# google-research/frame-interpolation

Hardware: AMD Instinct MI355X
Metric: interpolated frames/sec @1080p (higher is better)
Workload: dtype f32; 1 GPU; 1080p_2x2: 1920x1080 pair, align 64, block_shape [2, 2] -> 4 tile(s) of 960x576 in one batch, film_net published config, seeded synthetic weights, t=0.5; parallelism=1 independent GPU(s), weights RCCL-broadcast once, exec=direct launches, two lanes, lanes=1

## Files before the change

### frame-interpolation_amd/csrc/conv_igemm.hip

```cpp
#include "conv_buf_impl.h"
#include "conv_wino43_impl.h"
#include "conv_wino2d_impl.h"
#include "conv_fold4_impl.h"
#include "conv_c3_impl.h"
#ifdef FILM_EXTRA_FAMILIES
#include "conv_halo_impl.h"
#include "conv_split_impl.h"
#include "conv_wino_impl.h"
#include "conv_winox3_impl.h"
#include "conv_foldx3_impl.h"
#endif

template <int F>
static hipError_t launch_shape(const ConvParams& p, int shape, hipStream_t s) {
  switch (shape) {
    case TILE_128x128: return conv_buf_launch<128, 128, 2, 2, F>(p, s);
    case TILE_256x64: return conv_buf_launch<256, 64, 4, 1, F>(p, s);
    case TILE_256x32: return conv_buf_launch<256, 32, 4, 1, F>(p, s);
    case TILE_64x64: return conv_buf_launch<64, 64, 2, 2, F>(p, s);
    case TILE_128x32: return conv_buf_launch<128, 32, 4, 1, F>(p, s);
    case TILE_128x64: return conv_buf_launch<128, 64, 2, 2, F>(p, s);
    case TILE_256x128: return conv_buf_launch<256, 128, 4, 2, F>(p, s);
    default: return hipErrorInvalidValue;
  }
}

static hipError_t launch_c3(const ConvParams& p, int shape, hipStream_t s) {
  if (shape != TILE_C3_DIRECT) return hipErrorInvalidValue;
  return p.Cout % 64 == 0 ? conv_c3_launch<64>(p, s) : conv_c3_launch<32>(p, s);
}

#ifdef FILM_EXTRA_FAMILIES
template <int F>
static hipError_t launch_halo(const ConvParams& p, int shape, hipStream_t s) {
  switch (shape) {
    case HALO_8x128: return conv_halo_launch<8, 128, 4, 2, F>(p, s);
    case HALO_8x64: return conv_halo_launch<8, 64, 4, 1, F>(p, s);
    case HALO_8x32: return conv_halo_launch<8, 32, 4, 1, F>(p, s);
    case HALO_4x64: return conv_halo_launch<4, 64, 4, 1, F>(p, s);
    case HALO_4x128: return conv_halo_launch<4, 128, 2, 2, F>(p, s);
    case HALO_4x32: return conv_halo_launch<4, 32, 4, 1, F>(p, s);
    default: return hipErrorInvalidValue;
  }
}

template <int F, int NP>
static hipError_t launch_split(const ConvParams& p, int shape, hipStream_t s) {
  switch (shape) {
    case HALO_8x128: return conv_halo_split_launch<8, 128, 4, 2, NP, F>(p, s);
    case HALO_8x64: return conv_halo_split_launch<8, 64, 4, 1, NP, F>(p, s);
    case HALO_8x32: return conv_halo_split_launch<8, 32, 4, 1, NP, F>(p, s);
    case HALO_4x64: return conv_halo_split_launch<4, 64, 4, 1, NP, F>(p, s);
    case HALO_4x128: return conv_halo_split_launch<4, 128, 2, 2, NP, F>(p, s);
    case HALO_4x32: return conv_halo_split_launch<4, 32, 4, 1, NP, F>(p, s);
    default: return hipErrorInvalidValue;
  }
}

template <int F>
static hipError_t launch_wino(const ConvParams& p, int shape, hipStream_t s) {
  switch (shape) {
    case WINO_4x128: return conv_wino_launch<4, 128, 4, 2, F>(p, s);
    case WINO_4x64: return conv_wino_launch<4, 64, 4, 1, F>(p, s);
    case WINO_4x128_W16: return conv_wino_launch<4, 128, 4, 4, F>(p, s);
    case WINO_4x32: return conv_wino_launch<4, 32, 4, 1, F>(p, s);
    case WINO_8x64_W16: return conv_wino_launch<8, 64, 8, 2, F>(p, s);
    case WINO_8x32_W8: return conv_wino_launch<8, 32, 8, 1, F>(p, s);
    case WINO_2x64: return conv_wino_launch<2, 64, 2, 2, F>(p, s);
    case WINO_4x64_W8: return conv_wino_launch<4, 64, 4, 2, F>(p, s);
    default: return hipErrorInvalidValue;
  }
}

#endif

template <int F>
static hipError_t launch_wino43(const ConvParams& p, int shape, hipStream_t s) {
  switch (shape) {
    case W43_Q16_4x64_T21_P2: return conv_wino43_launch<4, 64, 2, 1, F | W43_F_PF2, 16>(p, s);
    case W43_Q16_4x32_T11_P2: return conv_wino43_launch<4, 32, 1, 1, F | W43_F_PF2, 16>(p, s);
    case W43_Q16_4x64_N1_P2: return conv_wino43_launch<4, 64, 1, 1, F | W43_F_PF2, 16, 1>(p, s);
    case W43_Q8_8x64_T21_P2: return conv_wino43_launch<8, 64, 2, 1, F | W43_F_PF2, 8>(p, s);
    case W43_Q8_8x64_N1_P2: return conv_wino43_launch<8, 64, 1, 1, F | W43_F_PF2, 8, 1>(p, s);
    case W43_Q8_8x32_T11_BG: return conv_wino43_launch<8, 32, 1, 1, F | W43_F_BG, 8>(p, s);
    case W43_Q8_8x32_T11_P2: return conv_wino43_launch<8, 32, 1, 1, F | W43_F_PF2, 8>(p, s);
#ifdef FILM_EXTRA_FAMILIES
    case W43_4x64_T21: return conv_wino43_launch<4, 64, 2, 1, F>(p, s);
    case W43_4x64_T12: return conv_wino43_launch<4, 64, 1, 2, F>(p, s);
    case W43_4x32_T11: return conv_wino43_launch<4, 32, 1, 1, F>(p, s);
    case W43_Q16_4x64_T21: return conv_wino43_launch<4, 64, 2, 1, F, 16>(p, s);
    case W43_Q16_4x64_T12: return conv_wino43_launch<4, 64, 1, 2, F, 16>(p, s);
    case W43_Q16_4x32_T11: return conv_wino43_launch<4, 32, 1, 1, F, 16>(p, s);
    case W43_Q16_4x64_N1: return conv_wino43_launch<4, 64, 1, 1, F, 16, 1>(p, s);
    case W43_Q16_4x64_T12_P2: return conv_wino43_launch<4, 64, 1, 2, F | W43_F_PF2, 16>(p, s);
    case W43_Q16_4x32_T11_BG: return conv_wino43_launch<4, 32, 1, 1, F | W43_F_BG, 16>(p, s);
    case W43_Q8_8x64_T12_P2: return conv_wino43_launch<8, 64, 1, 2, F | W43_F_PF2, 8>(p, s);
#endif
    default: return hipErrorInvalidValue;
  }
}

template <int F>
static hipError_t launch_wino2d(const ConvParams& p, int shape, hipStream_t s) {
  switch (shape) {
    case W2D_8x64: return conv_wino2d_launch_any<64, F>(p, s);
    case W2D_8x32: return conv_wino2d_launch_any<32, F>(p, s);
    case W2D_8x32_S2: return conv_wino2d_launch_any<32, F, 2>(p, s);
    case W2D_16x64: return conv_wino2d_launch_any<64, F | W2D_F_SQ>(p, s);
    case W2D_16x32: return conv_wino2d_launch_any<32, F | W2D_F_SQ>(p, s);
    case W2D_16x32_S2: return conv_wino2d_launch_any<32, F | W2D_F_SQ, 2>(p, s);
    default: return hipErrorInvalidValue;
  }
}

template <int F>
static hipError_t launch_fold4(const ConvParams& p, int shape, hipStream_t s) {
  switch (shape) {
    case F4_4x64: return conv_fold4_launch<2, F>(p, s);
    case F4_4x32: return conv_fold4_launch<1, F>(p, s);
    default: return hipErrorInvalidValue;
  }
}

#ifdef FILM_EXTRA_FAMILIES
template <int F>
static hipError_t launch_winox3(const ConvParams& p, int shape, hipStream_t s) {
  switch (shape) {
    case WX3_4x128_T22: return conv_winox3_launch<4, 128, 2, 2, F>(p, s);
    case WX3_4x64_T12: return conv_winox3_launch<4, 64, 1, 2, F>(p, s);
    case WX3_4x64_T21: return conv_winox3_launch<4, 64, 2, 1, F>(p, s);
    case WX3_4x32_T11: return conv_winox3_launch<4, 32, 1, 1, F>(p, s);
    default: return hipErrorInvalidValue;
  }
}

template <int F>
static hipError_t launch_foldx3(const ConvParams& p, int shape, hipStream_t s) {
  switch (shape) {
    case FX3_4x64: return conv_foldx3_launch<4, 64, 4, 1, F>(p, s);
    case FX3_8x64: return conv_foldx3_launch<8, 64, 8, 1, F>(p, s);
    case FX3_4x128: return conv_foldx3_launch<4, 128, 4, 2, F>(p, s);
    default: return hipErrorInvalidValue;
  }
}
#endif


__global__ __launch_bounds__(256) void conv_splitk_reduce_kernel(const float* __restrict__ part, const float* __restrict__ bias,
                                                                 float* __restrict__ out, int M, int Cout, int ostride,
                                                                 int S, int leaky) {
  const int G = Cout >> 2;
  const unsigned idx = blockIdx.x * 256u + threadIdx.x;
  if (idx >= (unsigned)M * (unsigned)G) return;
  const unsigned m = idx / (unsigned)G, g = idx - m * (unsigned)G;
  const size_t plane = (size_t)M * Cout;
  const float4* src = reinterpret_cast<const float4*>(part + (size_t)m * Cout + g * 4);
  float4 a = *reinterpret_cast<const float4*>(bias + g * 4);
  for (int sidx = 0; sidx < S; ++sidx) {
    const float4 v = src[(size_t)sidx * (plane >> 2)];
    a.x += v.x; a.y += v.y; a.z += v.z; a.w += v.w;
  }
  if (leaky) {
    a.x = a.x > 0.f ? a.x : 0.2f * a.x; a.y = a.y > 0.f ? a.y : 0.2f * a.y;
    a.z = a.z > 0.f ? a.z : 0.2f * a.z; a.w = a.w > 0.f ? a.w : 0.2f * a.w;
  }
  *reinterpret_cast<float4*>(out + (size_t)m * ostride + g * 4) = a;
}

static hipError_t film_launch_conv_main(const ConvParams& p, int fam, int tile, hipStream_t s) {
  const int shape = conv_tile_shape(tile);
  const bool xcd = tile & CONV_TILE_XCD;
  if ((p.pool_out != nullptr || p.pw_out != nullptr) && kConvFamily[fam].fused_shape < 0) return hipErrorInvalidValue;
  switch (fam) {
    case FAM_BUF: return xcd ? launch_shape<CONV_B_XCD_M>(p, shape, s) : launch_shape<0>(p, shape, s);
    case FAM_C3: return launch_c3(p, shape, s);
    case FAM_FOLD4: return xcd ? launch_fold4<CONV_B_XCD_M>(p, shape, s) : launch_fold4<0>(p, shape, s);
    case FAM_W2D:
      if (p.ksize != 3) return hipErrorInvalidValue;
      return xcd ? launch_wino2d<CONV_B_XCD_M>(p, shape, s) : launch_wino2d<0>(p, shape, s);
    case FAM_W43:
      if (p.ksize != 3) return hipErrorInvalidValue;
      if (p.pool_out != nullptr && shape < W43_Q16_4x64_T21) return hipErrorInvalidValue;
      if (p.pw_out != nullptr && ((shape != W43_Q16_4x64_N1 && shape != W43_Q16_4x64_N1_P2 && shape != W43_Q8_8x64_N1_P2) || p.Cout != 64 || p.ksplit > 1 ||
                                  p.pool_out != nullptr || p.pw_cout < 1 || p.pw_cout > 4))
        return hipErrorInvalidValue;
      return xcd ? launch_wino43<CONV_B_XCD_M>(p, shape, s) : launch_wino43<0>(p, shape, s);
#ifdef FILM_EXTRA_FAMILIES
    case FAM_HALO:
      if (p.ksize != 3) return hipErrorInvalidValue;
      return xcd ? launch_halo<CONV_B_XCD_M>(p, shape, s) : launch_halo<0>(p, shape, s);
    case FAM_SPLIT6:
      if (p.ksize != 3) return hipErrorInvalidValue;
      return xcd ? launch_split<CONV_B_XCD_M, 6>(p, shape, s) : launch_split<0, 6>(p, shape, s);
    case FAM_SPLIT3:
      if (p.ksize != 3) return hipErrorInvalidValue;
      return xcd ? launch_split<CONV_B_XCD_M, 3>(p, shape, s) : launch_split<0, 3>(p, shape, s);
    case FAM_WINO:
      if (p.ksize != 3) return hipErrorInvalidValue;
      return xcd ? launch_wino<CONV_B_XCD_M>(p, shape, s) : launch_wino<0>(p, shape, s);
    case FAM_WINOX3:
      if (p.ksize != 3) return hipErrorInvalidValue;
      return xcd ? launch_winox3<CONV_B_XCD_M>(p, shape, s) : launch_winox3<0>(p, shape, s);
    case FAM_FOLDX3:
      if (p.ksize != 2 || p.fold != 2) return hipErrorInvalidValue;
      return xcd ? launch_foldx3<CONV_B_XCD_M>(p, shape, s) : launch_foldx3<0>(p, shape, s);
#endif
    default: return hipErrorNotSupported;
  }
}

hipError_t film_launch_conv(const ConvParams& p, int tile, hipStream_t s) {
  const int fam = conv_family_of(tile);
  if (fam < 0 || (p.ksplit > 1 && !kConvFamily[fam].splitk)) return hipErrorInvalidValue;
  const hipError_t e = film_launch_conv_main(p, fam, tile, s);
  if (e != hipSuccess || p.ksplit <= 1) return e;
  const long long Mout = (long long)p.M * (p.fold == 3 ? 4 : 1);
  if (!p.part || (p.Cout & 3) || Mout * (p.Cout >> 2) >= (1ll << 32)) return hipErrorInvalidValue;
  const unsigned units = (unsigned)Mout * (unsigned)(p.Cout >> 2);
  hipLaunchKernelGGL(conv_splitk_reduce_kernel, dim3((units + 255) / 256), dim3(256), 0, s, p.part, p.bias, p.out, (int)Mout, p.Cout,
                     p.ostride, p.ksplit, p.leaky);
  return hipGetLastError();
}
```

### frame-interpolation_amd/csrc/conv_wino2d_impl.h

```cpp
#pragma once
#include "conv_common.h"

enum { W2D_F_SQ = 128,
       W2D_F_XEPI = 8,
       W2D_DBG_TIME = 8192 };


template <bool SQ> struct W2dSlotTable { unsigned v[24 * 64]; };
template <bool SQ> constexpr W2dSlotTable<SQ> w2d_make_slot_table() {
  constexpr int QW = SQ ? 4 : 8, TH = SQ ? 16 : 8, HR = TH + 2, PW = 4 * QW + 2;
  constexpr int CO4 = (PW + 3) / 4, MO4 = 4 * CO4, RP4 = 4 * MO4 + (SQ ? 2 : 4);
  W2dSlotTable<SQ> t{};
  for (int sl = 0; sl < 24 * 64; ++sl) {
    const int r = sl / RP4, rem = sl % RP4, m = rem / MO4, rr = rem % MO4, c = rr / CO4, k = rr % CO4, px = 4 * k + m;
    const bool ok = r < HR && rem < 4 * MO4 && px < PW;
    t.v[sl] = ok ? ((unsigned)r << 24 | (unsigned)px << 8 | (unsigned)c << 4) : 0xFFFFFFFFu;
  }
  return t;
}
template <bool SQ> __device__ const W2dSlotTable<SQ> w2d_slot_table = w2d_make_slot_table<SQ>();

template <int BN, int FLAGS, int NS_ = 3>
__global__ __launch_bounds__(4 * (BN / 32) * 64, (BN == 32) ? 2 : 1) void conv_wino2d_kernel(ConvParams p) {
  constexpr bool SQ = (FLAGS & W2D_F_SQ) != 0;
  constexpr int QW = SQ ? 4 : 8, TH = SQ ? 16 : 8, HR = TH + 2, PXW = 4 * QW, PW = PXW + 2;
  static_assert(QW * (TH / 2) == 32, "32 units per tile");
  constexpr int NG = BN / 32, NW = 4 * NG;
  constexpr int CO4 = (PW + 3) / 4, MO4 = 4 * CO4, RP4 = 4 * MO4 + (SQ ? 2 : 4);
  constexpr int NREQ = 24;
  constexpr int STAGE4 = NREQ * 64;
  constexpr int NS = NS_;
  static_assert(NS == 2 || NS == 3, "stages");
  constexpr int IPW = NREQ / NW;
  static_assert(NREQ % NW == 0, "requests per wave");
  static_assert(HR * RP4 <= STAGE4, "stage size");
  constexpr bool XE = (FLAGS & W2D_F_XEPI) != 0;
  constexpr unsigned OOB = 0xFFFFFFFFu;

  extern __shared__ __attribute__((aligned(1024))) float smem[];

  const int t = threadIdx.x;
  const int lane = t & 63;
  const int wv = __builtin_amdgcn_readfirstlane(t >> 6);
  const int l31 = lane & 31, half = lane >> 5;
  const int mu = wv & 3, ng = wv >> 2;

  unsigned long long tm0 = 0, tm1 = 0, tm2 = 0, tmA = 0, tmB = 0, tmC = 0, tmW = 0, tmE1 = 0, tmE2 = 0, tmE3 = 0;
  unsigned long long rt0 = 0;
  if constexpr ((FLAGS & W2D_DBG_TIME) != 0) { rt0 = __builtin_amdgcn_s_memrealtime(); tm0 = __builtin_readcyclecounter(); }

  int aH = p.H, aW = p.W, aNB = p.NB, aCtot = p.Ctot, aKsplit = p.ksplit, aNseg = p.nseg, aUnused = p.unused_chain;
  unsigned a_tpi = p.mg_tpi, a_ntx = p.mg_ntx, a_nby = p.mg_nby;
  int ntx_ = p.tl_ntx, tpi_ = p.tl_tpi;
  int aGx = (int)gridDim.x, aGy = (int)gridDim.y;
  const float* aS0ptr = p.seg[0].ptr;
  int aS0stride = p.seg[0].stride, aS0C = p.seg[0].C, aS0boff = p.seg[0].boff, aS0bmod = p.seg[0].bmod;
  const float* aWptr = p.w;
  unsigned rtab[(24 / (4 * (BN / 32)))];
#pragma unroll
  for (int n = 0; n < 24 / NW; ++n) rtab[n] = w2d_slot_table<SQ>.v[t + 64 * NW * n];
  {
    unsigned long long q0 = (unsigned long long)(uintptr_t)aS0ptr, q1 = (unsigned long long)(uintptr_t)aWptr;
    asm volatile("" : "+s"(aH), "+s"(aW), "+s"(aNB), "+s"(aCtot), "+s"(aKsplit), "+s"(aNseg), "+s"(aUnused), "+s"(a_tpi), "+s"(a_ntx), "+s"(a_nby), "+s"(ntx_), "+s"(tpi_),
                      "+s"(aGx), "+s"(aGy), "+s"(q0), "+s"(q1), "+s"(aS0stride), "+s"(aS0C), "+s"(aS0boff), "+s"(aS0bmod));
    aS0ptr = reinterpret_cast<const float*>((uintptr_t)q0);
    aWptr = reinterpret_cast<const float*>((uintptr_t)q1);
  }
  unsigned long long tmK = 0, tmT = 0;
  if constexpr ((FLAGS & W2D_DBG_TIME) != 0) tmK = __builtin_readcyclecounter();
  int bx = blockIdx.x, by = blockIdx.y;
  if constexpr ((FLAGS & CONV_B_XCD_M) != 0) {
    const int nbx = aGx, nby = aGy;
    const int nwg = nbx * nby;
    const int lin = by * nbx + bx;
    const int xcd = lin & 7, idx = lin >> 3;
    const int q = nwg >> 3, r = nwg & 7;
    const int base = xcd < r ? xcd * (q + 1) : r * (q + 1) + (xcd - r) * q;
    const int nl = base + idx;
    bx = (int)conv_udiv((unsigned)nl, a_nby);
    by = nl - bx * nby;
  }
  const int ntx = ntx_, tpi = tpi_;
  const int img = (int)conv_udiv((unsigned)bx, a_tpi);
  const int trow0 = (int)conv_udiv((unsigned)(bx - img * tpi), a_ntx);
  const int y0 = trow0 * TH, x0 = (bx - img * tpi - trow0 * ntx) * PXW;
  const int n0 = by * BN;

  unsigned rvoff[IPW];
  int rsg = 0, rc0 = 0, rsegC = 0;
  conv_rsrc_t rrsrc = conv_make_rsrc(conv_uniform_ptr(aS0ptr));
  const unsigned lds0 = (unsigned)(size_t)(__attribute__((address_space(3))) float*)smem;
  unsigned rpk[IPW];
  auto set_rpk = [&]() {
    const int H = aH, W = aW;
    const bool inside = y0 >= 1 && y0 + TH + 1 <= H && x0 >= 1 && x0 + PXW + 1 <= W;
    if (inside) {
#pragma unroll
      for (int n = 0; n < IPW; ++n) rpk[n] = rtab[n];
    } else {
#pragma unroll
      for (int n = 0; n < IPW; ++n) {
        const unsigned tv = rtab[n];
        const unsigned y = (unsigned)(y0 - 1) + (tv >> 24), x = (unsigned)(x0 - 1) + ((tv >> 8) & 255u);
        rpk[n] = ((y < (unsigned)H) & (x < (unsigned)W)) ? tv : OOB;
      }
    }
  };
  set_rpk();
#pragma unroll
  for (int n = 0; n < IPW; ++n) asm volatile("" : "+v"(rpk[n]));
  if constexpr ((FLAGS & W2D_DBG_TIME) != 0) tmT = __builtin_readcyclecounter();
  auto raw_setup_seg_of = [&](const float* sptr, int sstride, int sC, int sboff, int sbmod) {
    rsegC = __builtin_amdgcn_readfirstlane(sC);
    int be = img + sboff;
    if (sbmod && be >= sbmod) be -= sbmod;
    const int spix = (be * aH + (y0 - 1)) * aW + (x0 - 1);
    rrsrc = conv_make_rsrc(conv_uniform_ptr(sptr + (long long)spix * sstride));
    const unsigned st4 = (unsigned)sstride * 4u;
    const unsigned wst4 = (unsigned)aW * st4;
#pragma unroll
    for (int n = 0; n < IPW; ++n) {
      const unsigned tv = rpk[n];
      unsigned off, tmp;
      asm("v_and_b32 %0, 48, %2\n\tv_bfe_u32 %1, %2, 8, 8\n\tv_mad_u32_u24 %0, %1, %3, %0\n\tv_lshrrev_b32 %1, 24, %2\n\tv_mad_u32_u24 %0, %1, %4, %0"
          : "=&v"(off), "=&v"(tmp) : "v"(tv), "s"(st4), "s"(wst4));
      rvoff[n] = tv == OOB ? OOB : off;
    }
  };
  auto raw_setup_seg = [&]() {
    const ConvSeg& s = p.seg[rsg];
    raw_setup_seg_of(s.ptr, s.stride, s.C, s.boff, s.bmod);
  };
  auto dma_piece = [&](int n, int stage) {
    const unsigned so = (unsigned)rc0 * 4u;
    const unsigned base = lds0 + (unsigned)stage * (STAGE4 * 16u) + (unsigned)(wv + NW * n) * 1024u;
    asm volatile("s_mov_b32 m0, %0\n\ts_nop 0\n\tbuffer_load_dwordx4 %1, %2, %3 offen lds" ::"s"(base), "v"(rvoff[n]), "s"(rrsrc), "s"(so)
                 : "memory");
  };
  auto dma_advance = [&]() {
    rc0 += 16;
    if (rc0 >= rsegC) {
      if (rsg + 1 < aNseg) { rc0 = 0; ++rsg; raw_setup_seg(); }
    }
  };
  const int ksp = XE && aKsplit > 1 ? aKsplit : 1;
  const int nsc_all = aCtot >> 4;
  int sc0 = 0, sc1 = nsc_all;
  if (ksp > 1) {
    sc0 = (int)((unsigned)nsc_all * blockIdx.z / (unsigned)ksp);
    sc1 = (int)((unsigned)nsc_all * (blockIdx.z + 1u) / (unsigned)ksp);
    int c = sc0 * 16;
    while (rsg + 1 < aNseg && c >= p.seg[rsg].C) { c -= p.seg[rsg].C; ++rsg; }
    rc0 = c;
  }
  auto raw_issue = [&](int stage) {
#pragma unroll
    for (int n = 0; n < IPW; ++n) dma_piece(n, stage);
    dma_advance();
  };

  const int nkc = aCtot / 8, nsc = sc1 - sc0, kc0 = 2 * sc0, kc1 = 2 * sc1;
  const conv_rsrc_t brsrc = conv_make_rsrc(conv_uniform_ptr(aWptr));
  const unsigned bvoff = (unsigned)((half * 32 + l31) * 16);
  const int ct = n0 / 32 + ng;
  auto slab = [&](int kc) { return (unsigned)(((ct * nkc + (kc < nkc ? kc : nkc - 1)) * 4 + mu) * 6) * 1024u; };
  bf4 fbg[2][6];

  f32x16 acc[6];

  const bf4* const smem4 = reinterpret_cast<const bf4*>(smem);
  const int ur = l31 / QW, lq = l31 % QW;
  const int ra = mu == 0 ? 0 : mu == 2 ? 2 : 1, rb = mu == 0 ? 2 : mu == 1 ? 2 : mu == 2 ? 1 : 3;
  const float sgn = mu == 1 ? 1.f : -1.f;
  const int ix_a = (2 * ur + ra) * RP4 + half * CO4 + lq, ix_b = (2 * ur + rb) * RP4 + half * CO4 + lq;
  typedef float f2 __attribute__((ext_vector_type(2)));
  f2 A[2][6][2];
  bf4 d[6];
  bf4 d2[6];

  using C0 = std::integral_constant<int, 0>;
  using C1 = std::integral_constant<int, 1>;
  auto read_row = [&](bf4 (&dst)[6], int ix, int stage, auto h_c) {
    constexpr int IMM = decltype(h_c)::value * 2 * CO4;
    const int ixs = ix + stage * STAGE4;
#pragma unroll
    for (int j = 0; j < 6; ++j) dst[j] = smem4[ixs + IMM + (j & 3) * MO4 + (j >> 2)];
  };
  auto pair_of = [](const bf4& v, int q) -> f2 { return q ? f2{v[2], v[3]} : f2{v[0], v[1]}; };
  auto set_pair = [](bf4& v, int q, f2 x) { if (q) { v[2] = x[0]; v[3] = x[1]; } else { v[0] = x[0]; v[1] = x[1]; } };
  auto fma2 = [](float k, f2 x, f2 y) -> f2 {
    f2 r;
    const f2 kk = {k, k};
    asm("v_pk_fma_f32 %0, %1, %2, %3" : "=v"(r) : "s"(kk), "v"(x), "v"(y));
    return r;
  };
  auto add2 = [](f2 x, f2 y) -> f2 { f2 r; asm("v_pk_add_f32 %0, %1, %2" : "=v"(r) : "v"(x), "v"(y)); return r; };
  auto mul2 = [](float k, f2 x) -> f2 {
    f2 r;
    const f2 kk = {k, k};
    asm("v_pk_mul_f32 %0, %1, %2" : "=v"(r) : "s"(kk), "v"(x));
    return r;
  };
  auto max1 = [](float x, float y) -> float { float r; asm("v_max_f32 %0, %1, %2" : "=v"(r) : "v"(x), "v"(y)); return r; };
  auto sub2 = [](f2 x, f2 y) -> f2 { f2 r; asm("v_pk_add_f32 %0, %1, %2 neg_lo:[0,1] neg_hi:[0,1]" : "=v"(r) : "v"(x), "v"(y)); return r; };
  f2 xt[4];
  auto xf_t = [&](int q) {
    const f2 d1 = pair_of(d[1], q), d2v = pair_of(d[2], q), d3 = pair_of(d[3], q), d4 = pair_of(d[4], q);
    xt[0] = fma2(-4.f, d2v, d4);
    xt[1] = fma2(-4.f, d1, d3);
    xt[2] = sub2(d4, d2v);
    xt[3] = sub2(d3, d1);
  };
  auto xf_v = [&](int q, int nu) -> f2 {
    switch (nu) {
      case 0: return fma2(4.f, pair_of(d[0], q), fma2(-5.f, pair_of(d[2], q), pair_of(d[4], q)));
      case 1: return add2(xt[0], xt[1]);
      case 2: return sub2(xt[0], xt[1]);
      case 3: return fma2(2.f, xt[3], xt[2]);
      case 4: return fma2(-2.f, xt[3], xt[2]);
      default: return fma2(4.f, pair_of(d[1], q), fma2(-5.f, pair_of(d[3], q), pair_of(d[5], q)));
    }
  };
  auto pin = [](f2& v) { asm volatile("" : "+v"(v)); };
  auto prepare = [&](f2 (&An)[6][2], int stage, auto h_c) {
    read_row(d, ix_a, stage, h_c);
    read_row(d2, ix_b, stage, h_c);
#pragma unroll
    for (int j = 0; j < 6; ++j)
#pragma unroll
      for (int q = 0; q < 2; ++q) set_pair(d[j], q, fma2(sgn, pair_of(d2[j], q), pair_of(d[j], q)));
#pragma unroll
    for (int q = 0; q < 2; ++q) {
      xf_t(q);
#pragma unroll
      for (int nu = 0; nu < 6; ++nu) An[nu][q] = xf_v(q, nu);
    }
  };

  if (ksp > 1) raw_setup_seg();
  else raw_setup_seg_of(aS0ptr, aS0stride, aS0C, aS0boff, aS0bmod);
  raw_issue(0);
  if constexpr ((FLAGS & W2D_DBG_TIME) != 0) tmA = __builtin_readcyclecounter();
#pragma unroll
  for (int j = 0; j < 6; ++j) fbg[0][j] = conv_buf_load(brsrc, bvoff, slab(kc0) + (unsigned)j * 1024u);
  __builtin_amdgcn_sched_barrier(0);
  asm volatile("s_waitcnt vmcnt(6)" ::: "memory");
  if constexpr ((FLAGS & W2D_DBG_TIME) != 0) tmB = __builtin_readcyclecounter();
  __syncthreads();
  if constexpr ((FLAGS & W2D_DBG_TIME) != 0) tmC = __builtin_readcyclecounter();
#pragma unroll
  for (int j = 0; j < 6; ++j) fbg[1][j] = conv_buf_load(brsrc, bvoff, slab(kc0 + 1) + (unsigned)j * 1024u);
  __builtin_amdgcn_sched_barrier(0);
  if (nsc > 1) raw_issue(1);
  if constexpr (NS > 2) { if (nsc > 2) raw_issue(2); }
  prepare(A[0], 0, C0{});

  int st_s = 0, st_n = 1;
  int st_dma = 0;
  bool dma_on = false;
  int gs = 0;
  constexpr int P1 = NS == 2 ? IPW : (IPW + 1) / 2, P0 = IPW - P1;
  auto dma_slot = [](int g, int cnt) constexpr -> int {
    if (cnt <= 0) return -1;
    if (cnt == 6) return g == 2 ? 0 : (g >= 5 && (g - 5) % 4 == 0) ? 1 + (g - 5) / 4 : -1;
    const int step = 24 / cnt, at = cnt == 1 ? 13 : 5;
    return (g % step == at && g / step < cnt) ? g / step : -1;
  };
  auto chunk = [&](int kc, auto h_c, auto first_c, auto last_c) {
    constexpr int H = decltype(h_c)::value;
    constexpr bool FIRST = decltype(first_c)::value != 0;
    constexpr bool LAST = decltype(last_c)::value != 0;
    constexpr bool PREP = !(LAST && H == 1);
    using RH = std::integral_constant<int, 1 - H>;
    const int rs = H == 0 ? st_s : st_n;
    f2(&Ac)[6][2] = A[H];
    f2(&An)[6][2] = A[1 - H];
    if constexpr (H == 1 && !LAST) {
      unsigned long long tw0 = 0;
      if constexpr ((FLAGS & W2D_DBG_TIME) != 0) tw0 = __builtin_readcyclecounter();
      if (NS == 2 || gs == 0) asm volatile("s_waitcnt vmcnt(6)" ::: "memory");
      else asm volatile("s_waitcnt vmcnt(12)" ::: "memory");
      __syncthreads();
      if constexpr ((FLAGS & W2D_DBG_TIME) != 0) tmW += __builtin_readcyclecounter() - tw0;
      dma_on = (kc >> 1) + NS < sc1;
      st_dma = st_s;
    }
    const unsigned so2 = LAST ? 0u : slab(kc + 2);
    __builtin_amdgcn_sched_barrier(0);
    auto gap = [&](auto g_c) {
      constexpr int g = decltype(g_c)::value;
      constexpr int jp = g >> 3, i8 = g & 7, k = i8 >> 1, j = 2 * jp + (i8 & 1);
      if constexpr (FIRST && k == 0) {
        const f32x16 zero = {0.f, 0.f, 0.f, 0.f, 0.f, 0.f, 0.f, 0.f, 0.f, 0.f, 0.f, 0.f, 0.f, 0.f, 0.f, 0.f};
        acc[j] = __builtin_amdgcn_mfma_f32_32x32x2f32(fbg[H][j][k], Ac[j][k >> 1][k & 1], zero, 0, 0, 0);
      } else {
        acc[j] = __builtin_amdgcn_mfma_f32_32x32x2f32(fbg[H][j][k], Ac[j][k >> 1][k & 1], acc[j], 0, 0, 0);
      }
      if constexpr (!LAST) {
        if constexpr (k == 3) fbg[H][j] = conv_buf_load(brsrc, bvoff, so2 + (unsigned)j * 1024u);
      }
      if constexpr (PREP) {
        if constexpr (g == 0) read_row(d, ix_a, rs, RH{});
        if constexpr (g == 1) read_row(d2, ix_b, rs, RH{});
        if constexpr (g >= 4 && g < 10) {
          constexpr int jj = g - 4;
#pragma unroll
          for (int q = 0; q < 2; ++q) { f2 v = fma2(sgn, pair_of(d2[jj], q), pair_of(d[jj], q)); pin(v); set_pair(d[jj], q, v); }
        }
        if constexpr (g >= 10 && g < 16) {
          constexpr int q = (g - 10) / 3, part = (g - 10) % 3;
          if constexpr (part == 0) {
            xf_t(q);
            pin(xt[0]); pin(xt[1]); pin(xt[2]); pin(xt[3]);
          } else if constexpr (part == 1) {
            An[0][q] = xf_v(q, 0);
            An[5][q] = xf_v(q, 5);
            pin(An[0][q]); pin(An[5][q]);
          } else {
#pragma unroll
            for (int nu = 1; nu < 5; ++nu) { An[nu][q] = xf_v(q, nu); pin(An[nu][q]); }
          }
        }
      }
      if constexpr (!LAST) {
        constexpr int CNT = H == 1 ? P1 : P0, N0 = H == 1 ? 0 : P1;
        constexpr int idx = dma_slot(g, CNT);
        if constexpr (idx >= 0) {
          if (dma_on) {
            dma_piece(N0 + idx, st_dma);
            if constexpr (N0 + idx == IPW - 1) dma_advance();
          }
        }
      }
      __builtin_amdgcn_sched_barrier(0);
    };
    conv_for_each(gap, std::make_integer_sequence<int, 24>{});
    if constexpr (H == 1) {
      st_s = st_n;
      st_n = st_n + 1 == NS ? 0 : st_n + 1;
      ++gs;
    }
  };

  auto epilogue = [&]() {
    const int t = threadIdx.x, lane = t & 63, l31 = lane & 31, half = lane >> 5;
    __syncthreads();
    if constexpr ((FLAGS & W2D_DBG_TIME) != 0) tmE1 = __builtin_readcyclecounter();
    float o[4][16];
  #pragma unroll
    for (int r = 0; r < 16; ++r) {
      const float m0 = acc[0][r], m1 = acc[1][r], m2 = acc[2][r], m3 = acc[3][r], m4 = acc[4][r], m5 = acc[5][r];
      const float s34 = m3 + m4, d34 = m3 - m4, d12 = m1 - m2, s12 = m1 + m2;
      o[0][r] = ((m0 + m1) + m2) + s34;
      o[1][r] = __builtin_fmaf(2.f, d34, d12);
      o[2][r] = __builtin_fmaf(4.f, s34, s12);
      o[3][r] = d12 + __builtin_fmaf(8.f, d34, m5);
    }
    bf4* const xb = reinterpret_cast<bf4*>(smem);
    constexpr int XB4 = NG * 4 * 256;
    static_assert(2 * XB4 <= NS * STAGE4, "exchange buffers");
    const int widx = (ng * 4 + mu) * 256 + l31 * 8;
    const int rng = t >> 8, run = (t >> 3) & 31, rcg = t & 7;
    const int ridx = rng * 1024 + run * 8 + (rcg ^ (run & 7));
    const int nrd = n0 + rng * 32 + rcg * 4;
    const bool rawsum = XE && ksp > 1;
    const bool has_pw = XE && p.pw_out != nullptr;
    float b0 = 0.f, b1 = 0.f, b2 = 0.f, b3 = 0.f;
    if (!rawsum) { const float* const bp = p.bias + nrd; b0 = bp[0]; b1 = bp[1]; b2 = bp[2]; b3 = bp[3]; }
    const int oy = y0 + 2 * (run / QW), ox = x0 + 4 * (run % QW);
    const int ostr = rawsum ? p.Cout : p.ostride;
    const float slope = (p.leaky && !rawsum) ? 0.2f : 1.f;
    const int dyo = 2 * (run / QW), dxo = 4 * (run % QW), nth = rng * 32 + rcg * 4;
    const int cpix = (img * p.H + y0) * p.W + x0;
    float* obase = p.out;
    if (rawsum) { asm volatile(""); obase = p.part + (size_t)blockIdx.z * p.M * p.Cout; }
    float* const ocorner = obase + ((long long)cpix * ostr + n0);
    float* const orow = ocorner + (__umul24(__umul24(dyo, p.W) + dxo, ostr) + nth);
    float* pool_base = nullptr;
    if (XE && p.pool_out) {
      asm volatile("");
      const int ppix = (img * (p.H >> 1) + (y0 >> 1)) * (p.W >> 1) + (x0 >> 1);
      pool_base = p.pool_out + ((long long)ppix * p.pool_ostride + n0) + (__umul24(__umul24(dyo >> 1, p.W >> 1) + (dxo >> 1), p.pool_ostride) + nth);
    }
    constexpr int PWS = 68;
    float* const pwt = smem + 2 * XB4 * 4;
    float* const pww = pwt + TH * PXW * PWS;
    if (has_pw && t < 256) pww[t] = (t & 3) < p.pw_cout ? p.pw_w[(t >> 2) * p.pw_cout + (t & 3)] : 0.f;
    bf4 k0 = {0.f, 0.f, 0.f, 0.f}, k1 = {0.f, 0.f, 0.f, 0.f};
    auto write_round = [&](int jx, bf4* xw) {
  #pragma unroll
      for (int g = 0; g < 4; ++g) {
        bf4 v;
        v[0] = o[jx][4 * g]; v[1] = o[jx][4 * g + 1]; v[2] = o[jx][4 * g + 2]; v[3] = o[jx][4 * g + 3];
        xw[widx + ((2 * g + half) ^ (l31 & 7))] = v;
      }
    };
  #pragma unroll
    for (int jx = 0; jx < 4; ++jx) {
      bf4* const xw = xb + (jx & 1) * XB4;
      write_round(jx, xw);
      __syncthreads();
      if constexpr ((FLAGS & W2D_DBG_TIME) != 0) { if (jx == 0) tmE2 = __builtin_readcyclecounter(); if (jx == 3) tmE3 = __builtin_readcyclecounter(); }
      const bf4 m0 = xw[ridx], m1 = xw[ridx + 256], m2 = xw[ridx + 512], m3 = xw[ridx + 768];
      bf4 r0, r1;
  #pragma unroll
      for (int q = 0; q < 2; ++q) {
        const f2 bq = q ? f2{b2, b3} : f2{b0, b1};
        const f2 v0 = add2(add2(add2(pair_of(m0, q), pair_of(m1, q)), pair_of(m2, q)), bq);
        const f2 v1 = add2(sub2(sub2(pair_of(m1, q), pair_of(m2, q)), pair_of(m3, q)), bq);
        const f2 s0 = mul2(slope, v0), s1 = mul2(slope, v1);
        set_pair(r0, q, f2{max1(v0[0], s0[0]), max1(v0[1], s0[1])});
        set_pair(r1, q, f2{max1(v1[0], s1[0]), max1(v1[1], s1[1])});
      }
      if (!has_pw) {
        if (ox + jx < p.W) {
          float* const o0 = orow + (size_t)jx * ostr;
          if (oy < p.H) *reinterpret_cast<bf4*>(o0) = r0;
          if (oy + 1 < p.H) *reinterpret_cast<bf4*>(o0 + (size_t)p.W * ostr) = r1;
        }
        if (XE && pool_base != nullptr) {
          if (jx & 1) {
            bf4 pv;
  #pragma unroll
            for (int c = 0; c < 4; ++c) pv[c] = (((k0[c] + r0[c]) + k1[c]) + r1[c]) * 0.25f;
            if (oy < p.H && ox + jx < p.W) *reinterpret_cast<bf4*>(pool_base + (size_t)(jx >> 1) * p.pool_ostride) = pv;
          } else {
            k0 = r0; k1 = r1;
          }
        }
      } else {
        float* const tr = pwt + ((2 * (run / QW)) * PXW + 4 * (run % QW) + jx) * PWS + rng * 32 + rcg * 4;
        *reinterpret_cast<bf4*>(tr) = r0;
        *reinterpret_cast<bf4*>(tr + PXW * PWS) = r1;
      }
    }
    if (has_pw) {
      __syncthreads();
      if (t < TH * PXW) {
        const int y = y0 + t / PXW, x = x0 + (t % PXW);
        float a[4] = {0.f, 0.f, 0.f, 0.f};
        const bf4* row = reinterpret_cast<const bf4*>(pwt + t * PWS);
        const bf4* wq = reinterpret_cast<const bf4*>(pww);
  #pragma unroll 4
        for (int c4 = 0; c4 < 16; ++c4) {
          const bf4 v = row[c4];
  #pragma unroll
          for (int k = 0; k < 4; ++k) {
            const bf4 w = wq[c4 * 4 + k];
  #pragma unroll
            for (int j = 0; j < 4; ++j) a[j] = __builtin_fmaf(v[k], w[j], a[j]);
          }
        }
        if (y < p.H && x < p.W) {
          float* dd = p.pw_out + (((size_t)img * p.H + y) * p.W + x) * p.pw_ostride;
  #pragma unroll
          for (int j = 0; j < 4; ++j)
            if (j < p.pw_cout) dd[j] = a[j] + p.pw_bias[j];
        }
      }
    }
  };
  if constexpr ((FLAGS & W2D_DBG_TIME) != 0) tm1 = __builtin_readcyclecounter();
  for (int tile = 0; tile < 1; ++tile) {
    chunk(kc0, C0{}, C1{}, C0{});
    chunk(kc0 + 1, C1{}, C0{}, C0{});
    for (int kc = kc0 + 2; kc < kc1 - 2; kc += 2) {
      chunk(kc, C0{}, C0{}, C0{});
      chunk(kc + 1, C1{}, C0{}, C0{});
    }
    if (nsc > 1) {
      chunk(kc1 - 2, C0{}, C0{}, C1{});
      chunk(kc1 - 1, C1{}, C0{}, C1{});
    }
    if constexpr ((FLAGS & W2D_DBG_TIME) != 0) tm2 = __builtin_readcyclecounter();
    epilogue();
  }
  if constexpr ((FLAGS & W2D_DBG_TIME) != 0) {
    const unsigned long long tm3 = __builtin_readcyclecounter();
    if (t == 0) {
      unsigned long long* o8 = reinterpret_cast<unsigned long long*>(p.part) + (size_t)(blockIdx.y * gridDim.x + blockIdx.x) * 16;
      o8[0] = tm0; o8[1] = tm1; o8[2] = tm2; o8[3] = tm3; o8[4] = tmA; o8[5] = tmB; o8[6] = tmC; o8[7] = tmW;
      o8[8] = rt0; o8[9] = __builtin_amdgcn_s_memrealtime();
      o8[10] = (unsigned long long)__builtin_amdgcn_s_getreg((31 << 11) | 4) | ((unsigned long long)__builtin_amdgcn_s_getreg((31 << 11) | 20) << 32);
      o8[11] = tmE1; o8[12] = tmE2; o8[13] = tmE3; o8[14] = tmK; o8[15] = tmT;
    }
  }
}

template <int BN, int FLAGS, int NS = 3>
hipError_t conv_wino2d_launch(const ConvParams& p, hipStream_t s) {
  if (!(FLAGS & W2D_F_XEPI) && (p.ksplit > 1 || p.pool_out || p.pw_out)) return hipErrorInvalidValue;
  const size_t lds = p.pw_out ? (size_t)2 * (BN / 32) * 16 * 1024 + 256 * 68 * 4 + 1024 : (size_t)NS * 24 * 1024;
  constexpr int NT = 4 * (BN / 32) * 64;
  if (p.ksize != 3 || p.Ctot % 16 || p.Cout % BN) return hipErrorInvalidValue;
  if (p.ksplit > 1 && (!p.part || (reinterpret_cast<uintptr_t>(p.part) & 15) || p.Cout % 4 || p.pool_out || p.pw_out || p.ksplit > p.Ctot / 16)) return hipErrorInvalidValue;
  if (p.pw_out) {
    if (BN != 64 || p.Cout != 64 || p.pool_out || p.pw_cout < 1 || p.pw_cout > 4) return hipErrorInvalidValue;
  } else if (p.ostride % 4 || (reinterpret_cast<uintptr_t>(p.out) & 15)) return hipErrorInvalidValue;
  if (p.pool_out && ((p.H | p.W) & 1 || p.pool_ostride % 4 || (reinterpret_cast<uintptr_t>(p.pool_out) & 15))) return hipErrorInvalidValue;
  {
    long long nimg = p.NB;
    for (int i = 0; i < p.nseg; ++i) nimg = std::max<long long>(nimg, (long long)p.seg[i].bmod);
    if ((nimg + 1) * p.H * p.W >= (1ll << 31)) return hipErrorInvalidValue;
  }
  if (p.W <= 0 || p.H <= 0 || p.W >= (1 << 20) || p.ostride >= (1 << 22) || p.pool_ostride >= (1 << 22) || p.Cout >= (1 << 22) ||
      (long long)8 * p.W * (p.ostride > p.Cout ? p.ostride : p.Cout) >= (1ll << 31)) return hipErrorInvalidValue;
  for (int i = 0; i < p.nseg; ++i)
    if ((long long)p.W * p.seg[i].stride * 4 >= (1ll << 24) || p.seg[i].C % 16 || p.seg[i].stride % 4 || p.seg[i].stride <= 0 || p.seg[i].stride >= (1 << 22) || p.seg[i].up || (reinterpret_cast<uintptr_t>(p.seg[i].ptr) & 15)) return hipErrorInvalidValue;
  constexpr bool SQ = (FLAGS & W2D_F_SQ) != 0;
  const int ntx = SQ ? (p.W + 15) / 16 : (p.W + 31) / 32, nty = SQ ? (p.H + 15) / 16 : (p.H + 7) / 8;
  const int ntiles = p.NB * ntx * nty;
  dim3 grid((unsigned)ntiles, p.Cout / BN, (unsigned)(p.ksplit > 1 ? p.ksplit : 1));
  ConvParams q = p;
  bool exact = true;
  q.mg_nby = conv_magic(grid.y, (unsigned long long)grid.x * grid.y, exact);
  q.mg_tpi = conv_magic((unsigned long long)ntx * nty, (unsigned long long)ntiles + 1, exact);
  q.mg_ntx = conv_magic(ntx, (unsigned long long)ntx * nty, exact);
  q.tl_ntx = ntx; q.tl_tpi = ntx * nty;
  if (!exact) return hipErrorInvalidValue;
  return conv_launch<conv_wino2d_kernel<BN, FLAGS, NS>>(grid, dim3(NT), lds, s, q, 144 * 1024);
}

template <int BN, int FLAGS, int NS = 3>
hipError_t conv_wino2d_launch_any(const ConvParams& p, hipStream_t s) {
  if (p.ksplit > 1 || p.pool_out || p.pw_out) return conv_wino2d_launch<BN, FLAGS | W2D_F_XEPI, NS>(p, s);
  return conv_wino2d_launch<BN, FLAGS, NS>(p, s);
}
```

### frame-interpolation_amd/csrc/film_engine.cpp

```cpp
#include "film_internal.h"

namespace film_internal {

thread_local std::string g_create_error;

int fail(film_t* h, int code, const char* fmt, ...) {
  char buf[1024];
  va_list ap;
  va_start(ap, fmt);
  vsnprintf(buf, sizeof buf, fmt, ap);
  va_end(ap);
  if (h) h->err = buf; else g_create_error = buf;
  return code;
}

int copy_out_string(film_t* h, const std::string& s, char* buf, int64_t cap, int64_t* needed) {
  if (needed) *needed = (int64_t)s.size() + 1;
  if (!buf || cap < (int64_t)s.size() + 1) {
    if (!buf && needed) return FILM_OK;
    return fail(h, FILM_ERR_INVALID, "buffer too small: need %lld bytes", (long long)s.size() + 1);
  }
  memcpy(buf, s.c_str(), s.size() + 1);
  return FILM_OK;
}

}

using namespace film_internal;

namespace {

enum OptNorm { AS_IS, BOOL, NONNEG, LOW5 };
struct OptionRow {
  const char* key;
  int film_t::*field;
  OptNorm norm;
  bool drops_plans;
  int64_t lo = 0, hi = 0;
  const char* refusal = nullptr;
  ConvFamily family = FAM_BUF;
  int need_lo = 0, need_hi = 0;
  const char* family_refusal = nullptr;
};
constexpr OptionRow kOptions[] = {
    {"graph", &film_t::opt_graph, AS_IS, false, 0, 2, "graph: 0 (one stream, eager), 1 (hipGraph replay) or 2 (two lanes, eager: the default)"},
    {"profile", &film_t::opt_profile, BOOL, false},
    {"autotune", &film_t::opt_autotune, BOOL, false},
    {"max_batch", &film_t::opt_max_batch, NONNEG, false},
    {"host_overlap", &film_t::opt_host_overlap, BOOL, false},
    {"block_overlap_h", &film_t::opt_block_overlap_h, AS_IS, false, -1, 65535, "block_overlap_h: -1 (what the align padding of a tile holds) or 0 .. 65535 rows"},
    {"block_overlap_w", &film_t::opt_block_overlap_w, AS_IS, false, -1, 65535, "block_overlap_w: -1 (what the align padding of a tile holds) or 0 .. 65535 columns"},
    {"tune_ms", &film_t::opt_tune_ms, NONNEG, false},
    {"splitk", &film_t::opt_splitk, BOOL, true},
    {"pack_groups", nullptr, AS_IS, false, 1, 4, "pack_groups: 1 .. 4"},
    {"fuse", &film_t::opt_fuse, LOW5, true},
    {"fold2x2", &film_t::opt_fold2x2, AS_IS, true, 0, 2, "fold2x2: 0, 1 or 2"},
    {"planar", &film_t::opt_planar, BOOL, true},
    {"winograd", &film_t::opt_wino, AS_IS, true, 0, 3, "winograd: 0, 1, 2 or 3", FAM_WINO, 2, 2,
     "winograd = 2 (F(2,3) kernel on every level) needs a library built with FILM_EXTRA_FAMILIES=1"},
    {"halo_all", &film_t::opt_halo_all, BOOL, true, 0, 0, nullptr, FAM_HALO, 1, 1, "halo_all needs a library built with FILM_EXTRA_FAMILIES=1"},
    {"lanes", &film_t::opt_lanes, AS_IS, true, 0, 3, "lanes: 0, 1, 2 or 3"},
    {"wino2d", &film_t::opt_wino2d, AS_IS, true, 0, 2, "wino2d: 0, 1 or 2"},
    {"w2d_small_px", &film_t::opt_w2d_small_px, AS_IS, true, 0, 1 << 30, "w2d_small_px: pixels per image, 0 = never"},
    {"w2d_min_px", &film_t::opt_w2d_min_px, AS_IS, true, 1, 1 << 30, "w2d_min_px: pixels per image"},
    {"w2d_splitk", &film_t::opt_w2d_splitk, AS_IS, true, 0, 16, "w2d_splitk: 0 (off), 1 (default rule) or 2..16 (A/B: the cap on levels of <= 1024 pixels)"},
    {"w2d_shape", &film_t::opt_w2d_shape, AS_IS, true, -1, W2D_SHAPES - 1, "w2d_shape: -1 (autotuned) or a Wino2dTile shape index"},
    {"fold4_shape", &film_t::opt_fold4_shape, AS_IS, true, -1, F4_4x32, "fold4_shape: -1 (autotuned) or a Fold4Tile shape index"},
    {"w43_shape", &film_t::opt_w43_shape, AS_IS, true, -1, 31, "w43_shape: -1 (autotuned) or a Wino43Tile shape index"},
    {"precision", &film_t::opt_precision, AS_IS, true, 0, 2, "precision: 0 (f32), 1 (bf16x6) or 2 (bf16x3)", FAM_SPLIT6, 1, 2,
     "precision %d (bf16 split modes) needs a library built with FILM_EXTRA_FAMILIES=1; this build runs fp32 MFMA only"},
};
constexpr bool option_rows_complete() {
  for (const OptionRow& o : kOptions)
    if ((o.lo < o.hi) != (o.refusal != nullptr) || ((o.family != FAM_BUF) != (o.family_refusal != nullptr))) return false;
  return true;
}
static_assert(option_rows_complete(), "a row with a range (a family) carries its refusal message, a row without leaves lo = hi (family = FAM_BUF)");

int tile_geometry(film_t* h, int H, int W, int block_h, int block_w, int align, TileMapParams* tp) {
  const int bh = block_h > 0 ? block_h : 1, bw = block_w > 0 ? block_w : 1;
  if (H % bh) return fail(h, FILM_ERR_INVALID, "block_height=%d should evenly divide height=%d.", bh, H);
  if (W % bw) return fail(h, FILM_ERR_INVALID, "block_width=%d should evenly divide width=%d.", bw, W);
  tp->H = H; tp->W = W; tp->bh = bh; tp->bw = bw; tp->ph = H / bh; tp->pw = W / bw;
  struct Axis { const char* key; int nb, p, want; int *ov, *e, *T, *off; };
  const Axis axes[2] = {{"block_overlap_h", bh, tp->ph, h->opt_block_overlap_h, &tp->ovy, &tp->eh, &tp->TH, &tp->oy},
                        {"block_overlap_w", bw, tp->pw, h->opt_block_overlap_w, &tp->ovx, &tp->ew, &tp->TW, &tp->ox}};
  for (const Axis& a : axes) {
    const int pad0 = (align > 0 && a.p % align) ? align - a.p % align : 0;
    const int o = a.nb == 1 ? 0 : a.want < 0 ? std::min(pad0 / 2, a.p / 2) : a.want;
    if (2 * (int64_t)o > a.p)
      return fail(h, FILM_ERR_INVALID, "%s: twice the overlap (%d) must not exceed the patch size %d", a.key, o, a.p);
    const int e = a.p + 2 * o;
    const int pad = (align > 0 && e % align) ? align - e % align : 0;
    *a.ov = o; *a.e = e; *a.T = e + pad; *a.off = pad / 2;
  }
  return FILM_OK;
}
hipError_t cut_tiles(const TileMapParams& tp, hipStream_t s) {
  return (tp.ovy | tp.ovx) ? film_launch_frame_to_tiles_overlap(tp, s) : film_launch_frame_to_tiles(tp, s);
}
hipError_t join_tiles(const TileMapParams& tp, hipStream_t s) {
  return (tp.ovy | tp.ovx) ? film_launch_blend_tiles(tp, s) : film_launch_tiles_to_frame(tp, s);
}
hipError_t cut_tiles_pix(const TileMapParams& tp, int pix, hipStream_t s) {
  if (pix != FILM_PIX_U8) return cut_tiles(tp, s);
  const uint8_t* src = reinterpret_cast<const uint8_t*>(tp.src);
  return (tp.ovy | tp.ovx) ? film_launch_frame_to_tiles_overlap_u8(tp, src, s) : film_launch_frame_to_tiles_u8(tp, src, s);
}
int ensure_stage(film_t* h, size_t bytes, hipStream_t s) {
  if (h->stage_bytes >= bytes) return FILM_OK;
  if (h->stage) { HIPCHK(h, hipStreamSynchronize(s)); HIPCHK(h, hipFree(h->stage)); h->stage = nullptr; h->stage_bytes = 0; }
  hipError_t e = hipMalloc(&h->stage, bytes);
  if (e != hipSuccess) return fail(h, FILM_ERR_NOMEM, "frame staging hipMalloc of %.1f MB failed", bytes * 1e-6);
  h->stage_bytes = bytes;
  return FILM_OK;
}
int balanced_chunk(int n, int maxc) {
  if (n <= maxc) return n;
  for (int c = maxc; 2 * c > maxc; --c)
    if (n % c == 0) return c;
  return maxc;
}
void sequence_chunk(int n, int T, int cap, int* k, int* nt) {
  int bk = 0, bt = 1;
  for (int t = std::min(T, cap); t >= 1; --t) {
    const int kk = std::min(n, cap / t);
    if (kk > bk) { bk = kk; bt = t; }
  }
  *k = balanced_chunk(n, std::max(bk, 1));
  *nt = balanced_chunk(T, bt);
}
int need_device(film_t* h, const char* fn) {
  if (h->plan_only) return fail(h, FILM_ERR_NO_DEVICE, "plan-only handle: %s needs a HIP device (no CPU fallback)", fn);
  if (!h->finalized) return fail(h, FILM_ERR_STATE, "film_finalize has not been called");
  return FILM_OK;
}
bool halve_on_nomem(int rc, int* chunk) {
  if (rc != FILM_ERR_NOMEM || *chunk <= 1) return false;
  *chunk = (*chunk + 1) / 2;
  return true;
}
struct FrameStage {
  film_t* h; hipStream_t s; bool host;
  float* result; size_t out_floats;
  float* out = nullptr;
  size_t used = 0;
  int open(size_t in_floats) {
    out = result;
    if (!host) return FILM_OK;
    int rc = ensure_stage(h, (in_floats + out_floats) * sizeof(float), s);
    if (rc == FILM_OK) out = (float*)h->stage + in_floats;
    return rc;
  }
  int upload(const float* src, size_t floats, const float** dev) {
    *dev = src;
    if (!host) return FILM_OK;
    HIPCHK(h, hipMemcpyAsync((float*)h->stage + used, src, floats * sizeof(float), hipMemcpyHostToDevice, s));
    *dev = (float*)h->stage + used;
    used += floats;
    return FILM_OK;
  }
  int finish() {
    if (!host) return FILM_OK;
    HIPCHK(h, hipMemcpyAsync(result, out, out_floats * sizeof(float), hipMemcpyDeviceToHost, s));
    HIPCHK(h, hipStreamSynchronize(s));
    return FILM_OK;
  }
};
template <class T> struct TileCopy { T* frames; int tile0, ntiles; int64_t slot; };
using Cut = TileCopy<const float>;
using Join = TileCopy<float>;
int run_chunk(film_t* h, Plan* P, TileMapParams tp, const std::vector<Cut>& cuts, const std::vector<Join>& joins, hipStream_t s) {
  const int64_t tile_floats = (int64_t)tp.TH * tp.TW * 3;
  for (const Cut& c : cuts) {
    tp.tile0 = c.tile0; tp.ntiles = c.ntiles; tp.src = c.frames; tp.dst = P->at("img0") + c.slot * tile_floats;
    HIPCHK(h, cut_tiles(tp, s));
  }
  int rc = run_plan(h, P, s);
  if (rc) return rc;
  for (const Join& j : joins) {
    tp.tile0 = j.tile0; tp.ntiles = j.ntiles; tp.src = P->at("out") + j.slot * tile_floats; tp.dst = j.frames;
    HIPCHK(h, join_tiles(tp, s));
  }
  return FILM_OK;
}

hipStream_t pick_stream(film_t* h, int mem_kind, void* stream) {
  return stream ? (hipStream_t)stream : (mem_kind == FILM_MEM_DEVICE ? (hipStream_t) nullptr : h->stream);
}

int forward_chunk(film_t* h, const float* x0, const float* x1, int B, int H, int W, float* out, int mem_kind, void* stream) {
  HIPCHK(h, hipSetDevice(h->device));
  Plan* P = nullptr;
  int rc = get_plan(h, B, H, W, true, &P);
  if (rc) return rc;
  hipStream_t s = pick_stream(h, mem_kind, stream);
  const size_t in_bytes = (size_t)B * H * W * 3 * sizeof(float);
  const hipMemcpyKind kin = mem_kind == FILM_MEM_HOST ? hipMemcpyHostToDevice : hipMemcpyDeviceToDevice;
  const hipMemcpyKind kout = mem_kind == FILM_MEM_HOST ? hipMemcpyDeviceToHost : hipMemcpyDeviceToDevice;
  HIPCHK(h, hipMemcpyAsync(P->at("img0"), x0, in_bytes, kin, s));
  HIPCHK(h, hipMemcpyAsync(P->at("img0") + (int64_t)B * H * W * 3, x1, in_bytes, kin, s));
  rc = run_plan(h, P, s);
  if (rc) return rc;
  HIPCHK(h, hipMemcpyAsync(out, P->at("out"), in_bytes, kout, s));
  if (mem_kind == FILM_MEM_HOST) HIPCHK(h, hipStreamSynchronize(s));
  return FILM_OK;
}

int interpolate_host_pipeline(film_t* h, Plan* P, TileMapParams tp, const float* x0, const float* x1, float* out, float* st, size_t frame_bytes, hipStream_t s) {
  const int nt = P->B;
  const size_t nf = frame_bytes / sizeof(float);
  for (hipEvent_t& e : h->pipe_ev)
    if (!e) HIPCHK(h, hipEventCreateWithFlags(&e, hipEventDisableTiming));
  LanePipe lp;
  for (size_t i = 0; i < P->ops.size() && lp.head.size() < 2; ++i) {
    const OpDesc& op = P->ops[i];
    if (op.lane == 1) continue;
    if (!batch_splittable(op, 2) || !op.xdeps.empty() || op.NB != 2 * nt) break;
    lp.head.push_back(i);
  }
  const OpDesc& last = P->ops.back();
  lp.tail = tp.B == 1 && tp.bh % 2 == 0 && last.lane == 0 && last.pw_out.buf >= 0 && last.NB == nt && batch_splittable(last, 2) && P->ops.size() > lp.head.size() + 1 &&
            std::find(lp.head.begin(), lp.head.end(), P->ops.size() - 1) == lp.head.end();
  tp.tile0 = 0;
  lp.mid_tail = [&]() -> hipError_t {
    TileMapParams t2 = tp;
    t2.ntiles = nt / 2; t2.src = P->at("out"); t2.dst = st + 2 * nf;
    hipError_t e = film_launch_tiles_to_frame(t2, s);
    if (e == hipSuccess) e = hipEventRecord(h->pipe_ev[1], s);
    return e;
  };
  struct Drain {
    film_t* h; hipStream_t s; bool armed;
    ~Drain() { if (armed) { (void)hipStreamSynchronize(h->stream2); (void)hipStreamSynchronize(s); } }
  } drain{h, s, true};
  HIPCHK(h, hipMemcpyAsync(st, x0, frame_bytes, hipMemcpyHostToDevice, s));
  tp.ntiles = nt; tp.src = st; tp.dst = P->at("img0");
  HIPCHK(h, film_launch_frame_to_tiles(tp, s));
  HIPCHK(h, hipEventRecord(h->pipe_ev[0], s));
  HIPCHK(h, hipStreamWaitEvent(h->stream2, h->pipe_ev[0], 0));
  for (size_t i : lp.head) HIPCHK(h, launch_op(batch_part(P->ops[i], 0, 2), P->arena, h->packed_dev, s));
  HIPCHK(h, hipMemcpyAsync(st + nf, x1, frame_bytes, hipMemcpyHostToDevice, h->stream2));
  tp.src = st + nf; tp.dst = P->at("img0") + (int64_t)nt * tp.TH * tp.TW * 3;
  HIPCHK(h, film_launch_frame_to_tiles(tp, h->stream2));
  HIPCHK(h, hipEventRecord(h->pipe_ev[0], h->stream2));
  HIPCHK(h, hipStreamWaitEvent(s, h->pipe_ev[0], 0));
  const hipError_t le = issue_lanes(h, P, s, false, &lp);
  if (le != hipSuccess) return fail(h, FILM_ERR_HIP, "kernel launch failed: %s", hipGetErrorString(le));
  h->last_plan = P;
  const int64_t tile_floats = (int64_t)tp.TH * tp.TW * 3;
  if (lp.tail) {
    TileMapParams t2 = tp;
    t2.tile0 = nt / 2; t2.ntiles = nt - nt / 2; t2.src = P->at("out") + (int64_t)(nt / 2) * tile_floats; t2.dst = st + 2 * nf;
    HIPCHK(h, film_launch_tiles_to_frame(t2, s));
    const size_t half = frame_bytes / 2;
    HIPCHK(h, hipStreamWaitEvent(h->stream2, h->pipe_ev[1], 0));
    HIPCHK(h, hipMemcpyAsync(out, st + 2 * nf, half, hipMemcpyDeviceToHost, h->stream2));
    HIPCHK(h, hipMemcpyAsync((char*)out + half, (const char*)(st + 2 * nf) + half, frame_bytes - half, hipMemcpyDeviceToHost, s));
    HIPCHK(h, hipStreamSynchronize(h->stream2));
  } else {
    tp.tile0 = 0; tp.ntiles = nt; tp.src = P->at("out"); tp.dst = st + 2 * nf;
    HIPCHK(h, film_launch_tiles_to_frame(tp, s));
    HIPCHK(h, hipMemcpyAsync(out, st + 2 * nf, frame_bytes, hipMemcpyDeviceToHost, s));
  }
  HIPCHK(h, hipStreamSynchronize(s));
  drain.armed = false;
  return FILM_OK;
}

size_t pix_bytes(int pix) { return pix == FILM_PIX_U8 ? 1 : sizeof(float); }
void stream_free(film_t* h) {
  FilmStream& fs = h->fs;
  for (void* p : {fs.keep, (void*)fs.result, (void*)fs.result8})
    if (p) (void)hipFree(p);
  fs = FilmStream{};
}
bool same_geometry(const TileMapParams& a, const TileMapParams& b) {
  const int va[] = {a.H, a.W, a.bh, a.bw, a.ph, a.pw, a.TH, a.TW, a.oy, a.ox, a.ovy, a.ovx, a.eh, a.ew};
  const int vb[] = {b.H, b.W, b.bh, b.bw, b.ph, b.pw, b.TH, b.TW, b.oy, b.ox, b.ovy, b.ovx, b.eh, b.ew};
  return std::equal(std::begin(va), std::end(va), std::begin(vb));
}
hipError_t stream_cut(const FilmStream& fs, TileMapParams tp, const Plan* P, int slot, hipStream_t s) {
  tp.tile0 = 0; tp.ntiles = tp.bh * tp.bw;
  tp.src = (const float*)fs.keep;
  tp.dst = P->at("img0") + (int64_t)slot * tp.ntiles * tp.TH * tp.TW * 3;
  return cut_tiles_pix(tp, fs.pix, s);
}

int debug_plan(film_t* h, int B, int H, int W, int tiles, Plan** P) {
  if (h->plan_only) return fail(h, FILM_ERR_NO_DEVICE, "plan-only handle has no device");
  if (!h->finalized) return fail(h, FILM_ERR_STATE, "weights are not finalized");
  if (tiles < 0 || (tiles > 0 && B % tiles)) return fail(h, FILM_ERR_INVALID, "tiles must be 0 (pair plan) or divide B (sequence plan)");
  HIPCHK(h, hipSetDevice(h->device));
  return get_plan(h, B, H, W, true, P, tiles);
}

}

extern "C" {

int film_to_uint8(const float* src, unsigned char* dst, int64_t n, void* stream) {
  if (n < 0 || (n > 0 && (!src || !dst))) return FILM_ERR_INVALID;
  return film_launch_to_uint8(src, dst, n, (hipStream_t)stream) == hipSuccess ? FILM_OK : FILM_ERR_HIP;
}

#ifndef FILM_SRC_ID
#define FILM_SRC_ID "unknown"
#endif
#ifdef FILM_EXTRA_FAMILIES
#define FILM_FLAVOUR "+extra"
#else
#define FILM_FLAVOUR ""
#endif
const char* film_version(void) { return "gfx950;film_hip r6;src=" FILM_SRC_ID FILM_FLAVOUR; }

int film_default_config(film_config* cfg) {
  if (!cfg) return FILM_ERR_INVALID;
  memset(cfg, 0, sizeof *cfg);
  cfg->pyramid_levels = 7; cfg->fusion_pyramid_levels = 5; cfg->specialized_levels = 3; cfg->sub_levels = 4;
  cfg->filters = 64;
  const int fcv[4] = {3, 3, 3, 3}, ffl[4] = {32, 64, 128, 256};
  for (int i = 0; i < 4; ++i) { cfg->flow_convs[i] = fcv[i]; cfg->flow_filters[i] = ffl[i]; }
  return FILM_OK;
}

int film_create(film_t** out, int device, const film_config* cfg) {
  if (!out) return fail(nullptr, FILM_ERR_INVALID, "out is NULL");
  *out = nullptr;
  std::unique_ptr<film_handle> h(new film_handle);
  if (cfg) h->cfg = *cfg; else film_default_config(&h->cfg);
  int rc = validate_config(h.get(), h->cfg);
  if (rc) { g_create_error = h->err; return rc; }
  h->device = device;
  h->plan_only = device < 0;
  if (!h->plan_only) {
    int ndev = 0;
    hipError_t e = hipGetDeviceCount(&ndev);
    if (e != hipSuccess || ndev <= 0)
      return fail(nullptr, FILM_ERR_NO_DEVICE, "no HIP device available (%s); libfilm_hip has no CPU fallback",
                  e != hipSuccess ? hipGetErrorString(e) : "device count 0");
    if (device >= ndev) return fail(nullptr, FILM_ERR_INVALID, "device %d out of range (%d devices)", device, ndev);
    if (hipSetDevice(device) != hipSuccess) return fail(nullptr, FILM_ERR_HIP, "hipSetDevice(%d) failed", device);
    hipDeviceProp_t prop;
    if (hipGetDeviceProperties(&prop, device) == hipSuccess && strncmp(prop.gcnArchName, "gfx950", 6) != 0)
      return fail(nullptr, FILM_ERR_NO_DEVICE, "device %d is %s; this library is built for gfx950 only", device, prop.gcnArchName);
    if (hipStreamCreateWithFlags(&h->stream, hipStreamNonBlocking) != hipSuccess ||
        hipStreamCreateWithFlags(&h->stream2, hipStreamNonBlocking) != hipSuccess)
      return fail(nullptr, FILM_ERR_HIP, "hipStreamCreate failed");
  }
  build_layers(h.get());
  *out = h.release();
  return FILM_OK;
}

void film_destroy(film_t* h) {
  if (!h) return;
  drop_plans(h);
  stream_free(h);
  if (h->packed_dev) (void)hipFree(h->packed_dev);
  if (h->stage) (void)hipFree(h->stage);
  if (h->metrics_buf) (void)hipFree(h->metrics_buf);
  if (h->stream) (void)hipStreamDestroy(h->stream);
  for (hipEvent_t& e : h->pipe_ev) if (e) { (void)hipEventDestroy(e); e = nullptr; }
  if (h->stream2) (void)hipStreamDestroy(h->stream2);
  delete h;
}

const char* film_last_error(const film_t* h) { return h ? h->err.c_str() : g_create_error.c_str(); }

int film_set_option(film_t* h, const char* key, int64_t value) {
  if (!h || !key) return FILM_ERR_INVALID;
  for (const OptionRow& o : kOptions) {
    if (strcmp(key, o.key)) continue;
    if (o.refusal && (value < o.lo || value > o.hi)) return fail(h, FILM_ERR_INVALID, "%s", o.refusal);
    const int v = o.norm == BOOL ? value != 0 : o.norm == NONNEG ? (value > 0 ? (int)value : 0) : o.norm == LOW5 ? (int)(value & 31) : (int)value;
    if (o.family_refusal && v >= o.need_lo && v <= o.need_hi && !conv_family_built(o.family)) return fail(h, FILM_ERR_INVALID, o.family_refusal, v);
    if (!o.field) return h->finalized ? film_ensure_groups_(h, v) : FILM_OK;
    if (h->*o.field == v) return FILM_OK;
    if (o.drops_plans) drop_plans(h);
    h->*o.field = v;
    return FILM_OK;
  }
  return fail(h, FILM_ERR_NOTFOUND, "unknown option '%s'", key);
}

int film_plan_json(film_t* h, int B, int H, int W, char* buf, int64_t cap, int64_t* needed) {
  if (!h) return FILM_ERR_INVALID;
  Plan* P = nullptr;
  int rc = get_plan(h, B, H, W, false, &P);
  if (rc) return rc;
  return copy_out_string(h, plan_json(h, *P), buf, cap, needed);
}

int film_sequence_plan_json(film_t* h, int n_pairs, int tiles_per_frame, int H, int W, char* buf, int64_t cap, int64_t* needed) {
  if (!h) return FILM_ERR_INVALID;
  if (n_pairs < 1 || tiles_per_frame < 1) return fail(h, FILM_ERR_INVALID, "n_pairs and tiles_per_frame must be positive");
  if ((int64_t)n_pairs * tiles_per_frame >= (int64_t)1 << 30) return fail(h, FILM_ERR_INVALID, "batch too large (2*B*H*W must fit int32)");
  Plan* P = nullptr;
  int rc = get_plan(h, n_pairs * tiles_per_frame, H, W, false, &P, tiles_per_frame);
  if (rc) return rc;
  return copy_out_string(h, plan_json(h, *P), buf, cap, needed);
}

int film_profile_json(film_t* h, char* buf, int64_t cap, int64_t* needed) {
  if (!h) return FILM_ERR_INVALID;
  if (h->profile_json.empty()) return fail(h, FILM_ERR_STATE, "no profiled forward yet (film_set_option(\"profile\", 1))");
  return copy_out_string(h, h->profile_json, buf, cap, needed);
}

int film_forward(film_t* h, const float* x0, const float* x1, int B, int H, int W, float* out, int mem_kind, void* stream) {
  if (!h || !x0 || !x1 || !out) return fail(h, FILM_ERR_INVALID, "NULL argument");
  int rc = need_device(h, "film_forward");
  if (rc) return rc;
  if (mem_kind != FILM_MEM_HOST && mem_kind != FILM_MEM_DEVICE) return fail(h, FILM_ERR_INVALID, "bad mem_kind");
  if (B < 1) return fail(h, FILM_ERR_INVALID, "B, H, W must be positive");
  int bmax = 1;
  rc = max_units(h, H, W, "frame", "tile the frame (Interpolator block_shape)", &bmax);
  if (rc) return rc;
  const size_t frame = (size_t)H * W * 3;
  int chunk = balanced_chunk(B, bmax);
  for (int b0 = 0; b0 < B;) {
    chunk = std::min(chunk, B - b0);
    rc = forward_chunk(h, x0 + b0 * frame, x1 + b0 * frame, chunk, H, W, out + b0 * frame, mem_kind, stream);
    if (halve_on_nomem(rc, &chunk)) continue;
    if (rc) return rc;
    b0 += chunk;
  }
  return FILM_OK;
}

int film_interpolate(film_t* h, const float* x0, const float* x1, int B, int H, int W, int align, int block_h,
                     int block_w, float* out, int mem_kind, void* stream) {
  if (!h || !x0 || !x1 || !out) return fail(h, FILM_ERR_INVALID, "NULL argument");
  int rc = need_device(h, "film_interpolate");
  if (rc) return rc;
  if (mem_kind != FILM_MEM_HOST && mem_kind != FILM_MEM_DEVICE) return fail(h, FILM_ERR_INVALID, "bad mem_kind");
  if (B < 1 || H < 1 || W < 1) return fail(h, FILM_ERR_INVALID, "B, H, W must be positive");
  TileMapParams tp{};
  tp.B = B;
  rc = tile_geometry(h, H, W, block_h, block_w, align, &tp);
  if (rc) return rc;
  HIPCHK(h, hipSetDevice(h->device));
  int tmax = 1;
  rc = max_units(h, tp.TH, tp.TW, "tile", "use a finer block_shape", &tmax);
  if (rc) return rc;
  const int ntiles = B * tp.bh * tp.bw;
  hipStream_t s = pick_stream(h, mem_kind, stream);
  const size_t nf = (size_t)B * H * W * 3;
  FrameStage st{h, s, mem_kind == FILM_MEM_HOST, out, nf};
  rc = st.open(2 * nf);
  if (rc) return rc;
  if (st.host && h->opt_host_overlap && !(tp.ovy | tp.ovx) && !h->opt_profile && h->opt_graph == 2 && h->opt_lanes != 0 && ntiles <= tmax && h->stream2) {
    Plan* P = nullptr;
    rc = get_plan(h, ntiles, tp.TH, tp.TW, true, &P);
    if (rc == FILM_OK) return interpolate_host_pipeline(h, P, tp, x0, x1, out, (float*)h->stage, nf * sizeof(float), s);
    if (rc != FILM_ERR_NOMEM) return rc;
  }
  const float *d0 = nullptr, *d1 = nullptr;
  if ((rc = st.upload(x0, nf, &d0)) || (rc = st.upload(x1, nf, &d1))) return rc;
  int chunk = balanced_chunk(ntiles, tmax);
  for (int t0 = 0; t0 < ntiles;) {
    chunk = std::min(chunk, ntiles - t0);
    Plan* P = nullptr;
    rc = get_plan(h, chunk, tp.TH, tp.TW, true, &P);
    if (halve_on_nomem(rc, &chunk)) continue;
    if (rc == FILM_OK) rc = run_chunk(h, P, tp, {{d0, t0, chunk, 0}, {d1, t0, chunk, chunk}}, {{st.out, t0, chunk, 0}}, s);
    if (rc) return rc;
    t0 += chunk;
  }
  return st.finish();
}

int film_tiling_json(film_t* h, int H, int W, int align, int block_h, int block_w, char* buf, int64_t cap, int64_t* needed) {
  if (!h) return FILM_ERR_INVALID;
  if (H < 1 || W < 1) return fail(h, FILM_ERR_INVALID, "B, H, W must be positive");
  TileMapParams tp{};
  int rc = tile_geometry(h, H, W, block_h, block_w, align, &tp);
  if (rc) return rc;
  std::ostringstream o;
  o << "{\"overlap_h\":" << tp.ovy << ",\"overlap_w\":" << tp.ovx << ",\"tile_h\":" << tp.eh << ",\"tile_w\":" << tp.ew
    << ",\"padded_h\":" << tp.TH << ",\"padded_w\":" << tp.TW << ",\"pad_y\":" << tp.oy << ",\"pad_x\":" << tp.ox << ",\"origins_y\":[";
  for (int i = 0; i < tp.bh; ++i) o << (i ? "," : "") << film_tile_origin(i, tp.ph, tp.ovy, tp.H, tp.eh);
  o << "],\"origins_x\":[";
  for (int j = 0; j < tp.bw; ++j) o << (j ? "," : "") << film_tile_origin(j, tp.pw, tp.ovx, tp.W, tp.ew);
  o << "]}";
  return copy_out_string(h, o.str(), buf, cap, needed);
}

int film_interpolate_sequence(film_t* h, const float* frames, int F, int H, int W, int align, int block_h, int block_w, float* out,
                              int mem_kind, void* stream) {
  if (!h || !frames || !out) return fail(h, FILM_ERR_INVALID, "NULL argument");
  if (mem_kind != FILM_MEM_HOST && mem_kind != FILM_MEM_DEVICE) return fail(h, FILM_ERR_INVALID, "bad mem_kind");
  if (F < 2) return fail(h, FILM_ERR_INVALID, "a sequence needs at least 2 frames, got %d", F);
  if (H < 1 || W < 1) return fail(h, FILM_ERR_INVALID, "B, H, W must be positive");
  TileMapParams tp{};
  tp.B = 1;
  int rc = tile_geometry(h, H, W, block_h, block_w, align, &tp);
  if (rc == FILM_OK) rc = need_device(h, "film_interpolate_sequence");
  if (rc) return rc;
  HIPCHK(h, hipSetDevice(h->device));
  int tmax = 1;
  rc = max_units(h, tp.TH, tp.TW, "tile", "use a finer block_shape", &tmax);
  if (rc) return rc;
  const int n = F - 1, T = tp.bh * tp.bw;
  int k = 1, nt = 1;
  sequence_chunk(n, T, tmax, &k, &nt);
  hipStream_t s = pick_stream(h, mem_kind, stream);
  const size_t frame = (size_t)H * W * 3;
  FrameStage st{h, s, mem_kind == FILM_MEM_HOST, out, n * frame};
  const float* dfr = nullptr;
  if ((rc = st.open(F * frame)) || (rc = st.upload(frames, F * frame, &dfr))) return rc;
  for (int j0 = 0; j0 < n; j0 += k) {
    k = std::min(k, n - j0);
    for (int t0 = 0; t0 < T;) {
      const int nn = std::min(nt, T - t0);
      Plan* P = nullptr;
      rc = get_plan(h, k * nn, tp.TH, tp.TW, true, &P, nn);
      if (k * nn > 1 && (halve_on_nomem(rc, &k) || halve_on_nomem(rc, &nt))) { t0 = 0; continue; }
      if (rc) return rc;
      std::vector<Cut> cuts;
      std::vector<Join> joins;
      if (nn == T) {
        cuts = {{dfr + j0 * frame, 0, (k + 1) * T, 0}};
        joins = {{st.out + j0 * frame, 0, k * T, 0}};
      } else {
        for (int f = 0; f <= k; ++f) cuts.push_back({dfr + (j0 + f) * frame, t0, nn, (int64_t)f * nn});
        for (int j = 0; j < k; ++j) joins.push_back({st.out + (j0 + j) * frame, t0, nn, (int64_t)j * nn});
      }
      rc = run_chunk(h, P, tp, cuts, joins, s);
      if (rc) return rc;
      t0 += nn;
    }
  }
  return st.finish();
}

int film_stream_plan_json(film_t* h, int tiles, int H, int W, int slot, char* buf, int64_t cap, int64_t* needed) {
  if (!h) return FILM_ERR_INVALID;
  if (tiles < 1) return fail(h, FILM_ERR_INVALID, "tiles must be positive");
  if (slot != 0 && slot != 1) return fail(h, FILM_ERR_INVALID, "slot must be 0 or 1 (the half of the frame buffers the pushed frame fills)");
  if (tiles >= 1 << 30) return fail(h, FILM_ERR_INVALID, "batch too large (2*B*H*W must fit int32)");
  Plan* P = nullptr;
  int rc = get_plan(h, tiles, H, W, false, &P, tiles, true);
  if (rc) return rc;
  return copy_out_string(h, plan_json(h, *P->orientation(slot)), buf, cap, needed);
}

int film_stream_open(film_t* h, int H, int W, int align, int block_h, int block_w, int pix) {
  if (!h) return FILM_ERR_INVALID;
  if (h->fs.open) return fail(h, FILM_ERR_STATE, "a stream is already open on this handle (one per handle: close it, or create another handle)");
  if (pix != FILM_PIX_F32 && pix != FILM_PIX_U8) return fail(h, FILM_ERR_INVALID, "bad pix: FILM_PIX_F32 (0) or FILM_PIX_U8 (1)");
  if (H < 1 || W < 1) return fail(h, FILM_ERR_INVALID, "B, H, W must be positive");
  TileMapParams tp{};
  tp.B = 1;
  int rc = tile_geometry(h, H, W, block_h, block_w, align, &tp);
  if (rc == FILM_OK) rc = need_device(h, "film_stream_open");
  if (rc) return rc;
  HIPCHK(h, hipSetDevice(h->device));
  int tmax = 1;
  rc = max_units(h, tp.TH, tp.TW, "tile", "use a finer block_shape", &tmax);
  if (rc) return rc;
  const int T = tp.bh * tp.bw;
  if (T > tmax)
    return fail(h, FILM_ERR_INVALID, "a stream runs the whole frame in one model invocation: its %d tiles of %d x %d exceed the %d tiles one invocation "
                "may take (64 GiB / 60 %% of the free HBM of workspace, 4 GiB per 32-bit addressed buffer, \"max_batch\") - use a finer block_shape", T, tp.TH, tp.TW, tmax);
  Plan* P = nullptr;
  rc = get_plan(h, T, tp.TH, tp.TW, true, &P, T, true);
  if (rc) return rc;
  FilmStream& fs = h->fs;
  const size_t nv = (size_t)H * W * 3;
  hipError_t e = hipMalloc(&fs.keep, (nv * pix_bytes(pix) + 3) & ~(size_t)3);
  if (e == hipSuccess) e = hipMalloc((void**)&fs.result, nv * sizeof(float));
  if (e == hipSuccess && pix == FILM_PIX_U8) e = hipMalloc((void**)&fs.result8, nv);
  if (e != hipSuccess) {
    (void)hipGetLastError();
    stream_free(h);
    return fail(h, FILM_ERR_NOMEM, "hipMalloc of the stream's frame buffers (%.1f MB) failed", nv * (pix_bytes(pix) + 5) * 1e-6);
  }
  fs.open = true;
  fs.H = H; fs.W = W; fs.align = align; fs.block_h = block_h; fs.block_w = block_w; fs.pix = pix;
  return FILM_OK;
}

int film_stream_reset(film_t* h) {
  if (!h) return FILM_ERR_INVALID;
  if (!h->fs.open) return fail(h, FILM_ERR_STATE, "no open stream (film_stream_open)");
  h->fs.primed = false;
  return FILM_OK;
}

int film_stream_close(film_t* h) {
  if (!h) return FILM_ERR_INVALID;
  if (!h->fs.open) return fail(h, FILM_ERR_STATE, "no open stream (film_stream_open)");
  (void)hipSetDevice(h->device);
  (void)hipDeviceSynchronize();
  stream_free(h);
  return FILM_OK;
}

int film_stream_push(film_t* h, const void* frame, void* mid, int* produced, int mem_kind, void* stream) {
  if (!h) return FILM_ERR_INVALID;
  FilmStream& fs = h->fs;
  if (!fs.open) return fail(h, FILM_ERR_STATE, "no open stream (film_stream_open)");
  hipStream_t s = pick_stream(h, mem_kind == FILM_MEM_DEVICE ? FILM_MEM_DEVICE : FILM_MEM_HOST, stream);
  struct Unprime {
    film_t* h; hipStream_t s; bool armed;
    ~Unprime() {
      if (!armed) return;
      h->fs.primed = false;
      (void)hipStreamSynchronize(h->stream2);
      (void)hipStreamSynchronize(s);
    }
  } unprime{h, s, true};
  if (produced) *produced = 0;
  if (!frame || !produced || (fs.primed && !mid)) return fail(h, FILM_ERR_INVALID, "NULL argument");
  if (mem_kind != FILM_MEM_HOST && mem_kind != FILM_MEM_DEVICE) return fail(h, FILM_ERR_INVALID, "bad mem_kind");
  HIPCHK(h, hipSetDevice(h->device));
  TileMapParams tp{};
  tp.B = 1;
  int rc = tile_geometry(h, fs.H, fs.W, fs.block_h, fs.block_w, fs.align, &tp);
  if (rc) return rc;
  const int T = tp.bh * tp.bw;
  Plan* P0 = nullptr;
  rc = get_plan(h, T, tp.TH, tp.TW, true, &P0, T, true);
  if (rc) return rc;
  const bool host = mem_kind == FILM_MEM_HOST;
  const size_t nv = (size_t)fs.H * fs.W * 3;
  if (fs.primed && (fs.plan_id != P0->id || !same_geometry(fs.geo, tp))) {
    Plan* R = P0->orientation(fs.slot);
    HIPCHK(h, stream_cut(fs, tp, R, fs.slot, s));
    if ((rc = run_plan(h, R, s, R->n_extract))) return rc;
  }
  const int slot = fs.primed ? 1 - fs.slot : 0;
  Plan* P = P0->orientation(slot);
  HIPCHK(h, hipMemcpyAsync(fs.keep, frame, nv * pix_bytes(fs.pix), host ? hipMemcpyHostToDevice : hipMemcpyDeviceToDevice, s));
  HIPCHK(h, stream_cut(fs, tp, P, slot, s));
  if (!fs.primed) {
    if ((rc = run_plan(h, P, s, P->n_extract))) return rc;
  } else {
    if ((rc = run_plan(h, P, s))) return rc;
    float* joined = (fs.pix == FILM_PIX_F32 && !host) ? (float*)mid : fs.result;
    TileMapParams j = tp;
    j.tile0 = 0; j.ntiles = T; j.src = P->at("out"); j.dst = joined;
    HIPCHK(h, join_tiles(j, s));
    if (fs.pix == FILM_PIX_U8) {
      uint8_t* q = host ? fs.result8 : (uint8_t*)mid;
      HIPCHK(h, film_launch_to_uint8(joined, q, (int64_t)nv, s));
      if (host) HIPCHK(h, hipMemcpyAsync(mid, q, nv, hipMemcpyDeviceToHost, s));
    } else if (host) {
      HIPCHK(h, hipMemcpyAsync(mid, joined, nv * sizeof(float), hipMemcpyDeviceToHost, s));
    }
  }
  if (host) HIPCHK(h, hipStreamSynchronize(s));
  *produced = fs.primed ? 1 : 0;
  fs.primed = true; fs.slot = slot; fs.plan_id = P0->id; fs.geo = tp;
  unprime.armed = false;
  return FILM_OK;
}

int film_get_tap(film_t* h, const char* name, float* dst, int64_t cap, int64_t dims[4]) {
  if (!h || !name) return FILM_ERR_INVALID;
  if (h->plan_only) return fail(h, FILM_ERR_NO_DEVICE, "plan-only handle has no device");
  Plan* P = h->last_plan;
  if (!P || !P->arena) return fail(h, FILM_ERR_STATE, "no forward has run yet");
  const int bi = P->find(name);
  if (bi < 0) return fail(h, FILM_ERR_NOTFOUND, "unknown tap '%s'", name);
  const Buffer& b = P->bufs[bi];
  for (const OpDesc& op : P->ops)
    if (op.kind == OP_CONV && op.pw_out.buf >= 0 && op.out.buf == bi)
      return fail(h, FILM_ERR_STATE, "tap '%s' is not materialised: the RGB head is fused into the layer that produces it "
                  "(film_set_option \"fuse\" without bit 16 keeps it)", name);
  if (dims) { dims[0] = b.N; dims[1] = b.H; dims[2] = b.W; dims[3] = b.C; }
  if (!dst) return FILM_OK;
  if (cap < b.size()) return fail(h, FILM_ERR_INVALID, "capacity %lld < %lld floats", (long long)cap, (long long)b.size());
  HIPCHK(h, hipSetDevice(h->device));
  HIPCHK(h, hipDeviceSynchronize());
  if (!b.planar) {
    HIPCHK(h, hipMemcpy(dst, P->arena + b.off, (size_t)b.size() * sizeof(float), hipMemcpyDeviceToHost));
    return FILM_OK;
  }
  std::vector<float> raw((size_t)b.size());
  HIPCHK(h, hipMemcpy(raw.data(), P->arena + b.off, raw.size() * sizeof(float), hipMemcpyDeviceToHost));
  const int64_t npix = (int64_t)b.N * b.H * b.W;
  const int pc[3] = {b.planar, b.planar, b.C - 2 * b.planar};
  int64_t base = 0;
  int coff = 0;
  for (int part = 0; part < 3; ++part) {
    for (int64_t i = 0; i < npix; ++i) std::memcpy(dst + i * b.C + coff, raw.data() + base + i * pc[part], (size_t)pc[part] * sizeof(float));
    base += npix * pc[part];
    coff += pc[part];
  }
  return FILM_OK;
}

int film_debug_arena(film_t* h, int B, int H, int W, int tiles, int64_t offset, int64_t count, float* data, int write) {
  if (!h) return FILM_ERR_INVALID;
  if (!data || offset < 0 || count < 0) return fail(h, FILM_ERR_INVALID, "film_debug_arena: NULL data or a negative range");
  Plan* P = nullptr;
  int rc = debug_plan(h, B, H, W, tiles, &P);
  if (rc) return rc;
  if (offset > P->arena_floats || count > P->arena_floats - offset)
    return fail(h, FILM_ERR_INVALID, "film_debug_arena: floats %lld .. %lld leave the workspace of %lld floats", (long long)offset,
                (long long)(offset + count), (long long)P->arena_floats);
  HIPCHK(h, hipStreamSynchronize(h->stream));
  if (count > 0) {
    if (write) HIPCHK(h, hipMemcpy(P->arena + offset, data, (size_t)count * sizeof(float), hipMemcpyHostToDevice));
    else HIPCHK(h, hipMemcpy(data, P->arena + offset, (size_t)count * sizeof(float), hipMemcpyDeviceToHost));
  }
  h->last_plan = P;
  return FILM_OK;
}

int film_debug_run_op(film_t* h, int B, int H, int W, int tiles, int index, int candidate, int* n_candidates) {
  if (!h) return FILM_ERR_INVALID;
  Plan* P = nullptr;
  int rc = debug_plan(h, B, H, W, tiles, &P);
  if (rc) return rc;
  if (index < 0 || (size_t)index >= P->ops.size())
    return fail(h, FILM_ERR_INVALID, "film_debug_run_op: op %d of a plan of %zu ops", index, P->ops.size());
  OpDesc op = P->ops[(size_t)index];
  std::vector<int> cands;
  if (op.kind == OP_CONV) cands = conv_candidates(op);
  if (n_candidates) *n_candidates = (int)cands.size();
  if (candidate < -1 || candidate >= (int)cands.size())
    return fail(h, FILM_ERR_INVALID, "film_debug_run_op: candidate %d of op %d ('%s'), which has %zu", candidate, index, op.tag.c_str(), cands.size());
  if (candidate >= 0) op.tile = cands[(size_t)candidate];
  HIPCHK(h, launch_op(op, P->arena, h->packed_dev, h->stream));
  HIPCHK(h, hipStreamSynchronize(h->stream));
  h->last_plan = P;
  return FILM_OK;
}

int film_debug_tile_map(film_t* h, int mode, int pix, void* frames_dev, float* tiles_dev, int B, int H, int W, int align, int block_h,
                        int block_w, int tile0, int ntiles, void* stream) {
  if (!h) return FILM_ERR_INVALID;
  if (!frames_dev || !tiles_dev) return fail(h, FILM_ERR_INVALID, "film_debug_tile_map: NULL argument");
  if (mode != 0 && mode != 1) return fail(h, FILM_ERR_INVALID, "film_debug_tile_map: bad mode %d: 0 (cut) or 1 (join)", mode);
  if (pix != FILM_PIX_F32 && pix != FILM_PIX_U8) return fail(h, FILM_ERR_INVALID, "bad pix: FILM_PIX_F32 (0) or FILM_PIX_U8 (1)");
  if (mode == 1 && pix == FILM_PIX_U8) return fail(h, FILM_ERR_INVALID, "film_debug_tile_map: a join writes float32 frames (FILM_PIX_U8 is for the cut only)");
  if (B < 1 || H < 1 || W < 1) return fail(h, FILM_ERR_INVALID, "B, H, W must be positive");
  TileMapParams tp{};
  tp.B = B;
  int rc = tile_geometry(h, H, W, block_h, block_w, align, &tp);
  if (rc) return rc;
  const int64_t total = (int64_t)B * tp.bh * tp.bw;
  if (ntiles < 1 || tile0 < 0 || (int64_t)tile0 + ntiles > total)
    return fail(h, FILM_ERR_INVALID, "film_debug_tile_map: tiles [%d, %lld) are no range of the %lld tiles of the batch", tile0,
                (long long)tile0 + ntiles, (long long)total);
  if (h->plan_only) return fail(h, FILM_ERR_NO_DEVICE, "plan-only handle: film_debug_tile_map needs a HIP device (no CPU fallback)");
  HIPCHK(h, hipSetDevice(h->device));
  tp.tile0 = tile0; tp.ntiles = ntiles;
  if (mode == 0) {
    tp.src = static_cast<const float*>(frames_dev); tp.dst = tiles_dev;
    HIPCHK(h, cut_tiles_pix(tp, pix, (hipStream_t)stream));
  } else {
    tp.src = tiles_dev; tp.dst = static_cast<float*>(frames_dev);
    HIPCHK(h, join_tiles(tp, (hipStream_t)stream));
  }
  return FILM_OK;
}

}
```

### frame-interpolation_amd/csrc/film_exec.cpp

```cpp
#include "film_internal.h"

namespace film_internal {
namespace {
inline const float* cptr(const float* base, const View& v) { return base + v.off; }
inline float* mptr(float* base, const View& v) { return base + v.off; }
}

hipError_t launch_op(const OpDesc& op, float* arena, const float* wts, hipStream_t s) {
  switch (op.kind) {
    case OP_CONV: {
      ConvParams p{};
      p.nseg = op.nseg;
      for (int i = 0; i < op.nseg; ++i) {
        p.seg[i].ptr = cptr(arena, op.seg[i].v);
        p.seg[i].stride = op.seg[i].v.stride;
        p.seg[i].C = op.seg[i].v.C;
        p.seg[i].boff = op.seg[i].boff; p.seg[i].bmod = op.seg[i].bmod; p.seg[i].up = op.seg[i].up;
      }
      p.ksize = op.ksize;
      p.w = wts + op.*kConvFamily[op.family].weights;
      p.bias = wts + op.b_off;
      p.out = mptr(arena, op.out); p.ostride = op.out.stride;
      p.NB = op.NB; p.H = op.H; p.W = op.W; p.Cout = op.Cout; p.Ctot = op.Ctot; p.leaky = op.leaky;
      p.M = op.NB * op.H * op.W;
      p.fold = op.fold; p.py = op.py; p.px = op.px; p.ftaps = op.ftaps;
      p.ksplit = op.ksplit; p.part = op.ksplit > 1 ? arena + op.part_off : nullptr;
      if (op.out2.buf >= 0) { p.pool_out = mptr(arena, op.out2); p.pool_ostride = op.out2.stride; }
      if (op.pw_out.buf >= 0) {
        p.pw_w = wts + op.w2_off; p.pw_bias = wts + op.b2_off; p.pw_out = mptr(arena, op.pw_out); p.pw_ostride = op.pw_out.stride; p.pw_cout = op.pw_cout;
      }
      for (int q = 0; q < 4; ++q) { p.tdy[q] = (signed char)op.tdy[q]; p.tdx[q] = (signed char)op.tdx[q]; p.fold_woff[q] = op.fold_woff[q]; }
      return film_launch_conv(p, op.tile, s);
    }
    case OP_FLOW_HEAD: {
      FlowHeadParams p{};
      p.in = cptr(arena, op.in); p.istride = op.in.stride; p.Cin = op.Ctot;
      p.w3 = wts + op.w_off; p.b3 = wts + op.b_off; p.w4 = wts + op.w2_off; p.b4 = wts + op.b2_off;
      p.out = mptr(arena, op.out); p.M = (int)op.n;
      if (op.out2.buf >= 0) { p.add = cptr(arena, op.in2); p.sum = mptr(arena, op.out2); }
      return film_launch_flow_head(p, s);
    }
    case OP_CONV_PW: {
      ConvPwParams p{};
      p.in = cptr(arena, op.in); p.istride = op.in.stride; p.Cin = op.Ctot;
      p.w = wts + op.w_off; p.bias = wts + op.b_off;
      p.out = mptr(arena, op.out); p.ostride = op.out.stride; p.Cout = op.Cout; p.leaky = op.leaky;
      p.M = (int)op.n;
      if (op.out2.buf >= 0) { p.add = cptr(arena, op.in2); p.sum = mptr(arena, op.out2); }
      return film_launch_conv_pw(p, s);
    }
    case OP_POOL: {
      PoolParams p{};
      p.in = cptr(arena, op.in); p.istride = op.in.stride; p.out = mptr(arena, op.out); p.ostride = op.out.stride;
      p.C = op.in.C; p.NB = op.NB; p.H = op.H; p.W = op.W;
      return film_launch_pool(p, s);
    }
    case OP_FLOW_UP: {
      FlowUpParams p{};
      p.in = cptr(arena, op.in); p.out = mptr(arena, op.out); p.NB = op.NB; p.h = op.H; p.w = op.W;
      return film_launch_flow_up(p, s);
    }
    case OP_FLOW_ADD: {
      FlowAddParams p{};
      p.a = cptr(arena, op.in); p.b = cptr(arena, op.in2); p.out = mptr(arena, op.out); p.n = op.n;
      return film_launch_flow_add(p, s);
    }
    case OP_WARP: {
      WarpParams p{};
      p.src = cptr(arena, op.in); p.sstride = op.in.stride; p.C = op.in.C;
      p.flow = op.in2.buf >= 0 ? cptr(arena, op.in2) : nullptr; p.fscale = op.fscale;
      p.dst = mptr(arena, op.out); p.dstride = op.out.stride;
      p.NB = op.NB; p.H = op.H; p.W = op.W;
      p.src_brot = op.src_brot; p.flow_brot = op.flow_brot; p.misc_nb = op.misc_nb;
      if (op.in3.buf >= 0) { p.coarse = cptr(arena, op.in3); p.flow_out = mptr(arena, op.out2); }
      if (op.img_out.buf >= 0) {
        p.src3 = cptr(arena, op.img_in); p.s3stride = op.img_in.stride;
        p.src3b = p.src3 + (int64_t)(op.misc_nb > 0 ? op.misc_nb : op.NB) * op.H * op.W * op.img_in.stride;
        p.dst3 = mptr(arena, op.img_out); p.d3stride = op.img_out.stride;
        p.pack_b = cptr(arena, op.pack_b); p.pack_f = cptr(arena, op.pack_f);
      }
      return film_launch_warp(p, s);
    }
    case OP_PACK_FLOW: {
      PackFlowParams p{};
      p.bflow = cptr(arena, op.in); p.fflow = cptr(arena, op.in2);
      p.dst = mptr(arena, op.out); p.dstride = op.out.stride; p.npix = op.n;
      return film_launch_pack_flow(p, s);
    }
  }
  return hipErrorInvalidValue;
}

bool batch_splittable(const OpDesc& op, int nparts) {
  return op.kind == OP_CONV && op.nseg == 1 && op.seg[0].bmod == 0 && op.seg[0].boff == 0 && op.seg[0].up == 0 && op.ksplit <= 1 && op.fold == 0 &&
         op.NB >= nparts && op.NB % nparts == 0 && (op.out2.buf < 0 || (!(op.H & 1) && !(op.W & 1)));
}
OpDesc batch_part(const OpDesc& op, int part, int nparts) {
  OpDesc q = op;
  q.NB = op.NB / nparts;
  const int64_t px = (int64_t)part * q.NB * op.H * op.W;
  q.seg[0].v.off += px * op.seg[0].v.stride;
  q.out.off += px * op.out.stride;
  if (op.out2.buf >= 0) q.out2.off += (int64_t)part * q.NB * (op.H / 2) * (op.W / 2) * op.out2.stride;
  if (op.pw_out.buf >= 0) q.pw_out.off += px * op.pw_out.stride;
  return q;
}

hipError_t issue_lanes(film_t* h, Plan* P, hipStream_t main, bool capturing, const LanePipe* lp) {
  const size_t nops = P->ops.size();
  if (P->lane_ev.size() < nops + 2) P->lane_ev.resize(nops + 2, nullptr);
  hipError_t ev_err = hipSuccess;
  auto event_of = [&](size_t i) -> hipEvent_t {
    if (!P->lane_ev[i]) {
      hipError_t e = hipEventCreateWithFlags(&P->lane_ev[i], hipEventDisableTiming);
      if (e != hipSuccess) { ev_err = e; P->lane_ev[i] = nullptr; }
    }
    return P->lane_ev[i];
  };
  const bool two_lanes = h->opt_lanes != 0;
  hipError_t le = hipSuccess;
  if (two_lanes) {
    le = hipEventRecord(event_of(nops), main);
    if (le == hipSuccess) le = hipStreamWaitEvent(h->stream2, event_of(nops), 0);
  }
  for (size_t i = 0; i < nops && le == hipSuccess; ++i) {
    const OpDesc& op = P->ops[i];
    const int lane = (two_lanes && op.lane == 1) ? 1 : 0;
    hipStream_t ls = lane ? h->stream2 : main;
    if (two_lanes)
      for (int d : op.xdeps) {
        le = hipStreamWaitEvent(ls, event_of((size_t)d), 0);
        if (le != hipSuccess) break;
      }
    if (le != hipSuccess) break;
    if (lp && std::find(lp->head.begin(), lp->head.end(), i) != lp->head.end()) le = launch_op(batch_part(op, 1, 2), P->arena, h->packed_dev, ls);
    else if (lp && lp->tail && i + 1 == nops) {
      le = launch_op(batch_part(op, 0, 2), P->arena, h->packed_dev, ls);
      if (le == hipSuccess) le = lp->mid_tail();
      if (le == hipSuccess) le = launch_op(batch_part(op, 1, 2), P->arena, h->packed_dev, ls);
    } else le = launch_op(op, P->arena, h->packed_dev, ls);
    if (le == hipSuccess && two_lanes && op.signal) le = hipEventRecord(event_of(i), ls);
  }
  if (two_lanes && le == hipSuccess) {
    le = hipEventRecord(event_of(nops + 1), h->stream2);
    if (le == hipSuccess) le = hipStreamWaitEvent(main, event_of(nops + 1), 0);
  } else if (two_lanes && !capturing) {
    (void)hipStreamSynchronize(h->stream2);
  }
  return le == hipSuccess ? ev_err : le;
}

int run_plan(film_t* h, Plan* P, hipStream_t s, size_t n_ops) {
  const int B = P->B, H = P->H, W = P->W;
  const bool prefix = n_ops < P->ops.size();
  if (h->opt_profile) {
    const size_t n = std::min(n_ops, P->ops.size());
    while (P->ev.size() < n + 1) { hipEvent_t e; HIPCHK(h, hipEventCreate(&e)); P->ev.push_back(e); }
    HIPCHK(h, hipEventRecord(P->ev[0], s));
    for (size_t i = 0; i < n; ++i) {
      HIPCHK(h, launch_op(P->ops[i], P->arena, h->packed_dev, s));
      HIPCHK(h, hipEventRecord(P->ev[i + 1], s));
    }
    HIPCHK(h, hipStreamSynchronize(s));
    struct Acc { int launches = 0; double ms = 0, flops = 0, bytes = 0; };
    std::map<std::string, Acc> cls;
    std::ostringstream ops;
    for (size_t i = 0; i < n; ++i) {
      float ms = 0;
      HIPCHK(h, hipEventElapsedTime(&ms, P->ev[i], P->ev[i + 1]));
      Acc& a = cls[kKindName[P->ops[i].kind]];
      a.launches++; a.ms += ms; a.flops += P->ops[i].flops; a.bytes += P->ops[i].bytes;
      ops << (i ? "," : "") << "{\"tag\":\"" << P->ops[i].tag << "\",\"kind\":\"" << kKindName[P->ops[i].kind] << "\",\"ms\":" << ms
          << ",\"flops\":" << P->ops[i].flops << ",\"bytes\":" << P->ops[i].bytes << ",\"tile\":" << P->ops[i].tile << "}";
    }
    std::ostringstream o;
    o << "{\"B\":" << B << ",\"H\":" << H << ",\"W\":" << W << ",\"classes\":{";
    bool first = true;
    for (auto& kv : cls) {
      o << (first ? "" : ",") << "\"" << kv.first << "\":{\"launches\":" << kv.second.launches << ",\"ms\":" << kv.second.ms
        << ",\"flops\":" << kv.second.flops << ",\"bytes\":" << kv.second.bytes << "}";
      first = false;
    }
    o << "},\"ops\":[" << ops.str() << "]}";
    h->profile_json = o.str();
  } else if (prefix) {
    for (size_t i = 0; i < n_ops; ++i) HIPCHK(h, launch_op(P->ops[i], P->arena, h->packed_dev, s));
  } else if (h->opt_graph == 1) {
    if (!P->graph_exec) {
      HIPCHK(h, hipStreamSynchronize(s));
      HIPCHK(h, hipStreamBeginCapture(h->stream, hipStreamCaptureModeThreadLocal));
      const hipError_t le = issue_lanes(h, P, h->stream, true);
      hipError_t ce = hipStreamEndCapture(h->stream, &P->graph);
      if (le != hipSuccess) return fail(h, FILM_ERR_HIP, "kernel launch failed during capture: %s", hipGetErrorString(le));
      HIPCHK(h, ce);
      HIPCHK(h, hipGraphInstantiate(&P->graph_exec, P->graph, nullptr, nullptr, 0));
    }
    HIPCHK(h, hipGraphLaunch(P->graph_exec, s));
  } else if (h->opt_graph == 2 && h->opt_lanes != 0) {
    const hipError_t le = issue_lanes(h, P, s, false);
    if (le != hipSuccess) return fail(h, FILM_ERR_HIP, "kernel launch failed: %s", hipGetErrorString(le));
  } else {
    for (const OpDesc& op : P->ops) HIPCHK(h, launch_op(op, P->arena, h->packed_dev, s));
  }
  h->last_plan = P;
  return FILM_OK;
}

}
```

### frame-interpolation_amd/csrc/film_internal.h

```cpp
#pragma once
#include <hip/hip_runtime.h>

#include <algorithm>
#include <atomic>
#include <cmath>
#include <cstdarg>
#include <cstdint>
#include <cstdio>
#include <cstdlib>
#include <cstring>
#include <functional>
#include <map>
#include <memory>
#include <sstream>
#include <string>
#include <thread>
#include <vector>

#include "../../include/film_hip.h"
#include "film_kernels.h"

namespace film_internal {


extern thread_local std::string g_create_error;

enum OpKind { OP_CONV = 0, OP_FLOW_HEAD, OP_CONV_PW, OP_POOL, OP_FLOW_UP, OP_FLOW_ADD, OP_WARP, OP_PACK_FLOW, OP_KINDS };
extern const char* const kKindName[OP_KINDS];

struct Buffer {
  std::string name;
  int64_t off;
  int N, H, W, C;
  int64_t floats;
  int planar = 0;
  int64_t size() const { return floats; }
};

struct View {
  int buf = -1;
  int64_t off = 0;
  int stride = 0;
  int C = 0;
};

struct SegDesc {
  View v;
  int boff = 0, bmod = 0, up = 0;
};

struct OpDesc : ConvWeights {
  int kind = 0;
  std::string tag;
  SegDesc seg[FILM_MAX_SEG];
  int nseg = 0;
  int ksize = 1, leaky = 0, Cout = 0, Ctot = 0, tile = 0;
  ConvFamily family = FAM_BUF;
  int64_t b_off = 0;
  int64_t w2_off = 0, b2_off = 0;
  int ksplit = 1;
  int64_t part_off = 0;
  int fold = 0, py = 0, px = 0;
  int ftaps = 0; int tdy[4] = {0, 0, 0, 0}, tdx[4] = {0, 0, 0, 0};
  int64_t fold_woff[4] = {0, 0, 0, 0};
  int lane = 0;
  std::vector<int> xdeps;
  bool signal = false;
  View in, in2, out;
  View pack_b, pack_f;
  View img_in, img_out;
  View pw_out; int pw_cout = 0;
  View in3, out2;
  int NB = 0, H = 0, W = 0;
  float fscale = 1.f;
  int src_brot = 0, flow_brot = 0, misc_nb = 0;
  int64_t n = 0;
  double flops = 0;
  double bytes = 0;
};

struct LayerPack : ConvWeights {
  std::string name;
  int kh, kw, cin, cout;
  std::vector<int> perm;
  bool c3 = false;
  bool kmajor() const { return !c3 && cout % 32 == 0; }
  int64_t b_off = 0;
  int64_t wf_off = -1;
  bool has_halo() const { return kmajor() && kh == 3 && kw == 3; }
  bool has_fold() const { return kmajor() && kh == 2 && kw == 2; }
  bool has_fold4() const { return has_fold() && ctot() % 16 == 0 && cout % 32 == 0; }
  bool has_w2d() const { return has_halo() && ctot() % 16 == 0 && cout % 32 == 0; }
  int ctot() const { return (int)perm.size(); }
  int64_t packed_rows() const { return c3 ? 48 : (int64_t)kh * kw * ctot(); }
};

struct HostTensor {
  std::vector<int64_t> dims;
  std::vector<float> data;
};

struct Plan {
  int B = 0, H = 0, W = 0;
  int tiles = 0;
  int slot = -1;
  size_t n_extract = 0;
  std::unique_ptr<Plan> twin;
  Plan* orientation(int s) { return s == slot ? this : twin.get(); }
  uint64_t id = 0;
  std::vector<Buffer> bufs;
  std::vector<OpDesc> ops;
  int64_t arena_floats = 0;
  float* arena = nullptr;
  hipGraphExec_t graph_exec = nullptr;
  hipGraph_t graph = nullptr;
  std::vector<hipEvent_t> ev;
  std::vector<hipEvent_t> lane_ev;
  uint64_t last_use = 0;
  int find(const std::string& n) const {
    for (size_t i = 0; i < bufs.size(); ++i)
      if (bufs[i].name == n) return (int)i;
    return -1;
  }
  float* at(const char* name) const { return arena + bufs[find(name)].off; }
};

enum FuseBit {
  FUSE_FLOW_UP = 1,
  FUSE_FLOW_ADD = 2,
  FUSE_MISC16 = 4,
  FUSE_POOL = 8,
  FUSE_RGB_HEAD = 16,
};

}

struct FilmStream {
  bool open = false;
  int H = 0, W = 0, align = 0, block_h = 0, block_w = 0, pix = 0;
  void* keep = nullptr;
  float* result = nullptr;
  unsigned char* result8 = nullptr;
  bool primed = false;
  int slot = 0;
  uint64_t plan_id = 0;
  TileMapParams geo{};
};

struct film_handle {
  FilmStream fs;
  uint64_t plan_ids = 0;
  void* stage = nullptr;
  size_t stage_bytes = 0;
  void* metrics_buf = nullptr;
  size_t metrics_bytes = 0;
  int device = -1;
  bool plan_only = true;
  film_config cfg{};
  hipStream_t stream = nullptr;
  std::string err;
  std::map<std::string, film_internal::HostTensor> host_w;
  std::vector<film_internal::LayerPack> layers;
  std::map<std::string, int> layer_idx;
  int64_t packed_floats = 0;
  int64_t group_end[4] = {0, 0, 0, 0};
  int groups_packed = 0;
  std::vector<float> packed_host;
  float* packed_dev = nullptr;
  bool finalized = false;
  std::vector<std::unique_ptr<film_internal::Plan>> plans;
  film_internal::Plan* last_plan = nullptr;
  uint64_t tick = 0;
  int opt_graph = 2;
  int opt_profile = 0, opt_autotune = 1;
  int opt_max_batch = 0;
  int opt_block_overlap_h = 0, opt_block_overlap_w = 0;
  int opt_host_overlap = 1;
  hipEvent_t pipe_ev[2] = {nullptr, nullptr};
  int opt_splitk = 1;
  int opt_fuse = 31;
  int opt_planar = 1;
  int opt_fold2x2 = 1;
  int opt_wino = 1;
  int opt_halo_all = 0;
  int opt_tune_ms = 0;
  int opt_lanes = 1;
  hipStream_t stream2 = nullptr;
  int opt_precision = 0;
  int opt_wino2d = 1;
  int opt_w2d_min_px = 1536;
  int opt_w2d_small_px = 256;
  int opt_w2d_splitk = 1;
  int opt_w2d_shape = -1;
  int opt_fold4_shape = -1;
  int opt_w43_shape = -1;
  std::string profile_json;
  std::map<std::string, int> tune_cache;
  std::map<std::string, int> tune_import;
};

extern "C" int film_ensure_groups_(film_t* h, int n);

namespace film_internal {

int fail(film_t* h, int code, const char* fmt, ...);

#define HIPCHK(h, expr)                                                                     \
  do {                                                                                      \
    hipError_t e_ = (expr);                                                                 \
    if (e_ != hipSuccess)                                                                   \
      return fail(h, FILM_ERR_HIP, "%s failed: %s (%s:%d)", #expr, hipGetErrorString(e_), __FILE__, __LINE__); \
  } while (0)


std::vector<int> feature_channels(const film_config& c);
int slot_offset(const film_config& c, int j);
std::vector<int> fusion_filters(const film_config& c);
std::string predictor_prefix(const film_config& c, int level);
int predictor_index(const film_config& c, int level);
int validate_config(film_t* h, const film_config& c);
void build_layers(film_t* h);
int layout_groups(int64_t ConvWeights::* copy);

struct FamilyCodes { int c3 = 0, halo = 0, split = 0, wino = 0; };
inline FamilyCodes family_codes(ConvFamily f) {
  FamilyCodes c;
  switch (f) {
    case FAM_C3: c.c3 = 1; break;
    case FAM_HALO: c.halo = 1; break;
    case FAM_SPLIT6: c.split = 1; break;
    case FAM_SPLIT3: case FAM_FOLDX3: c.split = 2; break;
    case FAM_WINO: c.wino = 1; break;
    case FAM_WINOX3: c.wino = 2; break;
    case FAM_W43: c.wino = 3; break;
    case FAM_W2D: c.wino = 4; break;
    default: break;
  }
  return c;
}

int copy_out_string(film_t* h, const std::string& s, char* buf, int64_t cap, int64_t* needed);

hipError_t launch_op(const OpDesc& op, float* arena, const float* wts, hipStream_t s);
bool batch_splittable(const OpDesc& op, int nparts);
OpDesc batch_part(const OpDesc& op, int part, int nparts);
struct LanePipe {
  std::vector<size_t> head;
  bool tail = false;
  std::function<hipError_t()> mid_tail;
};
hipError_t issue_lanes(film_t* h, Plan* P, hipStream_t main, bool capturing, const LanePipe* lp = nullptr);
int run_plan(film_t* h, Plan* P, hipStream_t s, size_t n_ops = SIZE_MAX);

std::vector<int> conv_candidates(const OpDesc& op);
int autotune_plan(film_t* h, Plan* P);

int get_plan(film_t* h, int B, int H, int W, bool need_device, Plan** out, int tiles = 0, bool stream = false);
void drop_plans(film_t* h);
int max_units(film_t* h, int H, int W, const char* what, const char* advice, int* units);

int plan_build(film_t* h, Plan* P, int B, int H, int W, int tiles = 0, int slot = -1);
int64_t limited_buffer_bytes(const Plan* P);
std::string plan_json(film_t* h, const Plan& P);

}
```

### frame-interpolation_amd/csrc/film_kernels.h

```cpp
#pragma once
#include <hip/hip_runtime.h>
#include <stdint.h>

#include <vector>

#define FILM_MAX_SEG 4
#define FILM_BK 16

struct ConvSeg {
  const float* ptr;
  int stride;
  int C;
  int boff, bmod;
  int up;
};

struct ConvParams {
  ConvSeg seg[FILM_MAX_SEG];
  int nseg;
  int ksize;
  const float* w;
  const float* bias;
  float* out;
  int ostride;
  int NB, H, W;
  int Cout, Ctot;
  int leaky;
  int M;
  int fold, py, px, ftaps;
  signed char tdy[4], tdx[4];
  long long fold_woff[4];
  int ksplit;
  float* part;
  int unused_chain;
  unsigned mg_tpi, mg_ntx, mg_nby;
  int tl_ntx, tl_tpi;
  float* pool_out;
  int pool_ostride;
  const float* pw_w;
  const float* pw_bias;
  float* pw_out;
  int pw_ostride, pw_cout;
};

struct FlowHeadParams {
  const float* in;
  int istride;
  int Cin;
  const float* w3;
  const float* b3;
  const float* w4;
  const float* b4;
  float* out;
  int M;
  const float* add;
  float* sum;
};

struct ConvPwParams {
  const float* in;
  int istride;
  int Cin;
  const float* w;
  const float* bias;
  float* out;
  int ostride;
  int Cout;
  int leaky;
  int M;
  const float* add;
  float* sum;
};

struct PoolParams {
  const float* in;
  int istride;
  float* out;
  int ostride;
  int C;
  int NB, H, W;
};

struct FlowUpParams {
  const float* in;
  float* out;
  int NB, h, w;
};

struct FlowAddParams {
  const float* a;
  const float* b;
  float* out;
  int64_t n;
};

struct WarpParams {
  const float* src;
  int sstride;
  int C;
  const float* flow;
  float fscale;
  float* dst;
  int dstride;
  int NB, H, W;
  const float* coarse;
  float* flow_out;
  const float* src3;
  const float* src3b;
  int s3stride;
  float* dst3;
  int d3stride;
  const float* pack_b;
  const float* pack_f;
  int src_brot = 0, flow_brot = 0, misc_nb = 0;
};

struct PackFlowParams {
  const float* bflow;
  const float* fflow;
  float* dst;
  int dstride;
  int64_t npix;
};

struct TileMapParams {
  const float* src;
  float* dst;
  int B, H, W;
  int bh, bw;
  int ph, pw;
  int TH, TW;
  int oy, ox;
  int tile0, ntiles;
  int ovy, ovx;
  int eh, ew;
};
__host__ __device__ inline int film_tile_origin(int i, int p, int o, int n, int e) {
  const int s = i * p - o;
  return s < 0 ? 0 : (s > n - e ? n - e : s);
}

enum ConvTile { TILE_128x128 = 0, TILE_256x64 = 1, TILE_256x32 = 2, TILE_64x64 = 3, TILE_128x32 = 4,
                TILE_128x64 = 5, TILE_256x128 = 6 , TILE_SHAPES = 7,
                TILE_C3_DIRECT = 7 , CONV_TILE_XCD = 16,
                CONV_TILE_C3 = 32 ,
                CONV_TILE_HALO = 64 ,
                CONV_TILE_WINO = 256 ,
                CONV_TILE_SPLIT = 128 ,
                CONV_TILE_X3 = 512 ,
                CONV_TILE_F43 = 2048 ,
                CONV_TILE_W2D = 8192 ,
                CONV_TILE_EXT = 4096 ,
                CONV_TILE_FOLD4 = 16384 ,
                CONV_TILE_FOLDX3 = 1024  };
enum Wino43Tile { W43_4x64_T21 = 0, W43_4x64_T12 = 1, W43_4x32_T11 = 2, W43_Q16_4x64_T21 = 3, W43_Q16_4x64_T12 = 4, W43_Q16_4x32_T11 = 5,
                  W43_Q16_4x64_N1 = 6 ,
                  W43_Q16_4x64_T21_P2 = 7, W43_Q16_4x64_T12_P2 = 8, W43_Q16_4x32_T11_P2 = 9, W43_Q16_4x64_N1_P2 = 10,
                  W43_Q16_4x32_T11_BG = 11,
                  W43_Q8_8x64_T21_P2 = 12, W43_Q8_8x64_N1_P2 = 13, W43_Q8_8x32_T11_BG = 14, W43_Q8_8x64_T12_P2 = 15,
                  W43_Q8_8x32_T11_P2 = 16 };
#ifdef FILM_EXTRA_FAMILIES
constexpr bool kExtraFamilies = true;
#else
constexpr bool kExtraFamilies = false;
#endif
static inline bool film_w43_shape_built(int sh) {
  if (kExtraFamilies) return sh >= 0 && sh <= W43_Q8_8x32_T11_P2;
  return sh == W43_Q16_4x64_T21_P2 || sh == W43_Q16_4x32_T11_P2 || sh == W43_Q16_4x64_N1_P2 || sh == W43_Q8_8x64_T21_P2 || sh == W43_Q8_8x64_N1_P2 ||
         sh == W43_Q8_8x32_T11_BG || sh == W43_Q8_8x32_T11_P2;
}
enum Wino2dTile { W2D_8x64 = 0, W2D_8x32 = 1, W2D_8x32_S2 = 2, W2D_16x64 = 3, W2D_16x32 = 4, W2D_16x32_S2 = 5, W2D_SHAPES = 6 };
inline bool film_w2d_square(int shape) { return shape >= W2D_16x64 && shape <= W2D_16x32_S2; }
inline bool film_w2d_64(int shape) { return shape == W2D_8x64 || shape == W2D_16x64; }
enum Fold4Tile { F4_4x64 = 0, F4_4x32 = 1 };
enum FoldX3Tile { FX3_4x64 = 0 , FX3_8x64 = 1 , FX3_4x128 = 2  };
enum WinoX3Tile { WX3_4x128_T22 = 0, WX3_4x64_T12 = 1, WX3_4x64_T21 = 3, WX3_4x32_T11 = 4 };
enum WinoTile { WINO_4x128 = 0 , WINO_4x64 = 1 , WINO_4x128_W16 = 2 ,
                WINO_4x64_W8 = 3 , WINO_4x32 = 4 , WINO_8x64_W16 = 5 ,
                WINO_8x32_W8 = 6 , WINO_2x64 = 7 , WINO_SHAPES = 8 };
enum HaloTile { HALO_8x128 = 0 , HALO_8x64 = 1 , HALO_8x32 = 2 , HALO_4x64 = 3 ,
                HALO_4x128 = 4 , HALO_4x32 = 5 , HALO_SHAPES = 6 };

struct TileShape { int bm, bn; };
static inline TileShape film_tile_shape(int tile) {
  switch (tile & (CONV_TILE_XCD - 1)) {
    case TILE_128x128: return {128, 128};
    case TILE_256x64: return {256, 64};
    case TILE_256x32: return {256, 32};
    case TILE_64x64: return {64, 64};
    case TILE_128x64: return {128, 64};
    case TILE_256x128: return {256, 128};
    default: return {128, 32};
  }
}

enum ConvFamily { FAM_BUF , FAM_C3, FAM_W2D, FAM_W43, FAM_FOLD4 ,
                  FAM_HALO, FAM_SPLIT6, FAM_SPLIT3, FAM_WINO, FAM_WINOX3, FAM_FOLDX3 ,
                  CONV_FAMILIES };
constexpr int CONV_TILE_FAMILY = CONV_TILE_C3 | CONV_TILE_HALO | CONV_TILE_SPLIT | CONV_TILE_WINO | CONV_TILE_X3 | CONV_TILE_FOLDX3 |
                                 CONV_TILE_F43 | CONV_TILE_W2D | CONV_TILE_FOLD4;

struct ConvWeights {
  int64_t w_off = 0;
  int64_t wh_off = -1;
  int64_t ws_off = -1;
  int64_t ww_off = -1;
  int64_t wx_off = -1;
  int64_t w43_off = -1;
  int64_t w2d_off = -1;
  int64_t wfx_off = -1;
  int64_t wf4_off = -1;
};

namespace film_internal {
struct OpDesc;
std::vector<int> tile_candidates(const OpDesc&), c3_candidates(const OpDesc&), wino2d_candidates(const OpDesc&), wino43_candidates(const OpDesc&),
    fold4_candidates(const OpDesc&), halo_candidates(const OpDesc&), wino_candidates(const OpDesc&), winox3_candidates(const OpDesc&),
    foldx3_candidates(const OpDesc&);
}
struct ConvFamilyRow {
  int flags;
  int64_t ConvWeights::* weights;
  bool splitk;
  bool in_default;
  int fused_shape;
  std::vector<int> (*candidates)(const film_internal::OpDesc&);
  int (*default_shape)(int Cout, int64_t M);
};

constexpr int conv_buf_shape(int Cout, int64_t M) {
  auto blocks = [&](int bm, int bn) { return ((M + bm - 1) / bm) * (Cout / bn); };
  if (Cout % 128 == 0) return blocks(128, 128) >= 768 ? TILE_128x128 : TILE_64x64;
  if (Cout % 64 == 0) return blocks(256, 64) >= 768 ? TILE_256x64 : TILE_64x64;
  return blocks(256, 32) >= 768 ? TILE_256x32 : TILE_128x32;
}
constexpr int film_split_shape(int Cout, int64_t) { return Cout % 128 == 0 ? HALO_8x128 : Cout % 64 == 0 ? HALO_4x64 : HALO_8x32; }

inline constexpr ConvFamilyRow kConvFamily[CONV_FAMILIES] = {
   {0, &ConvWeights::w_off, true, true, -1, film_internal::tile_candidates, conv_buf_shape},
   {CONV_TILE_C3, &ConvWeights::w_off, false, true, -1, film_internal::c3_candidates, [](int, int64_t) -> int { return TILE_C3_DIRECT; }},
   {CONV_TILE_W2D, &ConvWeights::w2d_off, true, true, W2D_8x64, film_internal::wino2d_candidates, [](int c, int64_t) -> int { return c % 64 == 0 ? W2D_8x64 : W2D_8x32; }},
   {CONV_TILE_WINO | CONV_TILE_F43, &ConvWeights::w43_off, true, true, W43_Q16_4x64_N1_P2, film_internal::wino43_candidates, [](int c, int64_t) -> int { return c % 64 == 0 ? W43_Q16_4x64_T21_P2 : W43_Q16_4x32_T11_P2; }},
   {CONV_TILE_FOLD4, &ConvWeights::wf4_off, true, true, -1, film_internal::fold4_candidates, [](int c, int64_t) -> int { return c % 64 == 0 ? F4_4x64 : F4_4x32; }},
   {CONV_TILE_HALO, &ConvWeights::wh_off, false, false, -1, film_internal::halo_candidates, [](int c, int64_t) -> int { return c % 64 == 0 ? HALO_4x64 : HALO_8x32; }},
   {CONV_TILE_SPLIT, &ConvWeights::ws_off, false, false, -1, film_internal::halo_candidates, film_split_shape},
   {CONV_TILE_SPLIT | CONV_TILE_X3, &ConvWeights::ws_off, false, false, -1, film_internal::halo_candidates, film_split_shape},
   {CONV_TILE_WINO, &ConvWeights::ww_off, false, false, -1, film_internal::wino_candidates, [](int c, int64_t) -> int { return c % 64 == 0 ? WINO_4x64_W8 : WINO_4x32; }},
   {CONV_TILE_WINO | CONV_TILE_X3, &ConvWeights::wx_off, false, false, -1, film_internal::winox3_candidates, [](int c, int64_t) -> int { return c % 128 == 0 ? WX3_4x128_T22 : c % 64 == 0 ? WX3_4x64_T12 : WX3_4x32_T11; }},
   {CONV_TILE_FOLDX3, &ConvWeights::wfx_off, false, false, -1, film_internal::foldx3_candidates, [](int, int64_t) -> int { return FX3_4x64; }},
};

constexpr bool conv_family_built(int f) { return kConvFamily[f].in_default || kExtraFamilies; }
constexpr int conv_family_of(int tile) {
  for (int f = 0; f < CONV_FAMILIES; ++f) if ((tile & CONV_TILE_FAMILY) == kConvFamily[f].flags) return f;
  return -1;
}
constexpr int conv_tile(int f, int shape, bool xcd) { return kConvFamily[f].flags | (shape & 15) | (shape >= 16 ? CONV_TILE_EXT : 0) | (xcd ? CONV_TILE_XCD : 0); }
constexpr int conv_tile_shape(int tile) { return (tile & 15) + ((tile & CONV_TILE_EXT) ? 16 : 0); }
constexpr int conv_default_tile(int f, int Cout, int64_t M) { return conv_tile(f, kConvFamily[f].default_shape(Cout, M), true); }

hipError_t film_launch_conv(const ConvParams& p, int tile, hipStream_t s);
hipError_t film_launch_conv_pw(const ConvPwParams& p, hipStream_t s);
hipError_t film_launch_flow_head(const FlowHeadParams& p, hipStream_t s);
hipError_t film_launch_pool(const PoolParams& p, hipStream_t s);
hipError_t film_launch_flow_up(const FlowUpParams& p, hipStream_t s);
hipError_t film_launch_flow_add(const FlowAddParams& p, hipStream_t s);
hipError_t film_launch_warp(const WarpParams& p, hipStream_t s);
hipError_t film_launch_pack_flow(const PackFlowParams& p, hipStream_t s);
hipError_t film_launch_frame_to_tiles(const TileMapParams& p, hipStream_t s);
hipError_t film_launch_tiles_to_frame(const TileMapParams& p, hipStream_t s);
hipError_t film_launch_frame_to_tiles_overlap(const TileMapParams& p, hipStream_t s);
hipError_t film_launch_frame_to_tiles_u8(const TileMapParams& p, const uint8_t* src, hipStream_t s);
hipError_t film_launch_frame_to_tiles_overlap_u8(const TileMapParams& p, const uint8_t* src, hipStream_t s);
hipError_t film_launch_blend_tiles(const TileMapParams& p, hipStream_t s);
hipError_t film_launch_to_uint8(const float* src, uint8_t* dst, int64_t n, hipStream_t s);
hipError_t film_launch_fill_random(float* dst, int64_t n, uint32_t seed, hipStream_t s);

#define FILM_SSIM_TAPS 11
struct MetricsParams {
  const float* pred;
  const float* ref;
  int B, H, W, C;
  int flags;
  double g[FILM_SSIM_TAPS];
  double c1, c2;
  int sum_blocks, ssim_tiles_x, ssim_tiles_y;
  int64_t part_per_image;
  double* part;
  double* out;
};
void film_metrics_layout(MetricsParams& p);
hipError_t film_launch_image_metrics(const MetricsParams& p, hipStream_t s);
```

### frame-interpolation_amd/csrc/film_planner.cpp

```cpp
#include "film_internal.h"

namespace film_internal {

const char* const kKindName[OP_KINDS] = {"conv_mfma", "flow_head", "conv_pw", "pool", "flow_up", "flow_add", "warp", "pack_flow"};

namespace {
struct ConvSite {
  const LayerPack* L;
  int H, W;
  int ctot;
  bool folded;
  bool any_up;
  bool out_16b;
  bool segs_16b;
  bool segs_c16;
  bool halo_row_24bit;
  bool fold4_rows_32bit;
  int64_t px() const { return (int64_t)H * W; }
};

ConvSite conv_site(const LayerPack& L, const std::vector<SegDesc>& segs, const View& out, int H, int W, bool folded) {
  ConvSite s{&L, H, W, 0, folded, false, out.off % 4 == 0 && out.stride % 4 == 0, true, true, true,
             (int64_t)16 * W * std::max(out.stride, L.cout) < (1ll << 31)};
  for (const SegDesc& g : segs) {
    s.ctot += g.v.C;
    s.any_up |= g.up != 0;
    s.segs_16b &= g.v.off % 4 == 0 && g.v.stride % 4 == 0;
    s.segs_c16 &= g.v.C % 16 == 0;
    s.halo_row_24bit &= (int64_t)W * g.v.stride * 4 < (1ll << 24);
  }
  return s;
}

ConvFamily plain_conv_family(const ConvSite& s, const film_t& o) {
  const LayerPack& L = *s.L;
  const int W = s.W, ctot = s.ctot;
  const int64_t px = s.px();
  const bool w2d_layout = ctot % 16 == 0 && s.out_16b && s.segs_c16 && s.segs_16b && s.halo_row_24bit;
  const int64_t w2d_tile_px = (int64_t)((s.H + 7) / 8) * 8 * ((W + 31) / 32) * 32;
  const bool w2d_level = px >= o.opt_w2d_min_px || (o.opt_w2d_small_px > 0 && px >= o.opt_w2d_small_px && px * 100 >= 65 * w2d_tile_px);
  if (L.w2d_off >= 0 && w2d_layout && !s.any_up && o.opt_precision == 0 &&
      (o.opt_wino2d == 2 || (o.opt_wino2d == 1 && o.opt_wino == 1 && w2d_level)))
    return FAM_W2D;
  const bool split = o.opt_precision != 0 && L.has_halo() && !s.any_up && (px >= 2048 || o.opt_halo_all);
  if (split && o.opt_precision == 1) return FAM_SPLIT6;
  const bool w43_width = L.w43_off >= 0 && (o.opt_wino == 3 || 64 * ((W + 63) / 64) * 100 <= 115 * W ||
                                            (px < 2048 && 32 * ((W + 31) / 32) * 100 <= 115 * W));
  const bool deep_small = L.cout % 128 == 0 && px >= 1024 && px < 8192 && ctot > 1024 && w43_width && o.opt_splitk &&
                          o.opt_wino == 1 && o.opt_precision == 0;
  if (L.ww_off >= 0 && !s.any_up && o.opt_wino != 0 &&
      ((L.cout % 128 == 0 && (px >= 8192 || (px >= 2048 && ctot <= 1024))) || (L.cout % 64 == 0 && px >= 30000) ||
       px >= 100000 || o.opt_wino >= 2 || deep_small)) {
    if (o.opt_precision == 2 && (split || o.opt_wino >= 2)) {
      if (L.cout % 128 == 0 || o.opt_wino >= 2) return FAM_WINOX3;
    } else {
      return o.opt_wino != 2 && w43_width ? FAM_W43 : FAM_WINO;
    }
  }
  if (split) return FAM_SPLIT3;
  if (L.has_halo() && !s.any_up && (o.opt_halo_all || (px >= 8192 && (ctot >= 768 || (ctot >= 512 && px >= 100000) || L.cout == 32))))
    return FAM_HALO;
  return FAM_BUF;
}

ConvFamily folded_conv_family(const ConvSite& s, const film_t& o) {
  const LayerPack& L = *s.L;
  if (o.opt_precision == 2 && L.wfx_off >= 0 && L.cout % 64 == 0 && (s.px() >= 2048 || o.opt_halo_all)) return FAM_FOLDX3;
  if (o.opt_fold2x2 == 1 && o.opt_precision == 0 && L.wf4_off >= 0 && s.segs_16b && s.out_16b && L.cout % 32 == 0 && s.fold4_rows_32bit)
    return FAM_FOLD4;
  return FAM_BUF;
}

int conv_ksplit(ConvFamily fam, const ConvSite& s, const film_t& o) {
  const LayerPack& L = *s.L;
  const int ctot = s.ctot;
  const int64_t px = s.px();
  if (!o.opt_splitk || L.cout % 4 != 0) return 1;
  switch (fam) {
    case FAM_BUF: {
      if (s.folded || !L.kmajor() || px > 4096) return 1;
      const int nsteps = L.kh * L.kw * ctot / 16;
      int S = nsteps < 128 ? 1 : px <= 64 ? 16 : px <= 256 ? 8 : px <= 1024 ? 4 : nsteps >= 256 ? 2 : 1;
      while (S > 1 && nsteps / S < 32) S >>= 1;
      return S;
    }
    case FAM_W43:
      if (px <= 4096 && ctot >= 512) return std::min(8, ctot / 128);
      if (px <= 16384 && ctot >= 1024) return 2;
      return 1;
    case FAM_W2D: {
      if (!o.opt_w2d_splitk) return 1;
      int S = 1;
      if (px <= 4096 && ctot >= 768) S = std::min(4, ctot / 384);
      if (o.opt_w2d_splitk > 1 && px <= 1024 && ctot >= 384) S = std::min(o.opt_w2d_splitk, ctot / 192);
      return S;
    }
    case FAM_FOLD4:
      return px <= 1024 && ctot >= 768 ? 4 : 1;
    default:
      return 1;
  }
}

struct Planner {
  film_t* h;
  Plan* P;
  int64_t cursor = 0;
  bool bad = false;
  std::string bad_msg;
  void refuse(const std::string& msg) { bad = true; bad_msg = msg; }

  int B = 0, T = 0, H0 = 0, W0 = 0;
  int NL = 0, FL = 0;
  int N2 = 0, NI = 0;
  int i0 = 0, i1 = 0;
  int NE = 0, e0 = 0;
  bool seq = false;
  std::vector<int> fc, ff;
  int HL(int l) const { return H0 >> l; }
  int WL(int l) const { return W0 >> l; }
  std::vector<int> img, feat, fx_a, fx_p, res, v, vup, warped, aligned, fu_u, fu_a, fu_b;
  int fp[3] = {-1, -1, -1}, out_buf = -1;
  View net;

  int push(const Buffer& b) {
    cursor += (b.floats + 63) & ~int64_t(63);
    P->bufs.push_back(b);
    return (int)P->bufs.size() - 1;
  }
  int add_buffer(const std::string& name, int N, int H, int W, int C) { return push(Buffer{name, cursor, N, H, W, C, (int64_t)N * H * W * C}); }
  int add_scratch(const std::string& name, int64_t floats) { return push(Buffer{name, cursor, 0, 0, 0, 0, std::max<int64_t>(floats, 64)}); }
  View view(int buf, int batch0, int coff, int C) const {
    const Buffer& b = P->bufs[buf];
    return View{buf, b.off + (int64_t)batch0 * b.H * b.W * b.C + coff, b.C, C};
  }
  View aligned_part(int buf, int part, int C) const {
    const Buffer& b = P->bufs[buf];
    const int Cp = part < 2 ? C : 16;
    return b.planar ? View{buf, b.off + (int64_t)part * b.N * b.H * b.W * C, Cp, Cp} : view(buf, 0, part * C, Cp);
  }
  static View sub(View v, int coff, int C) { v.off += coff; v.C = C; return v; }
  View scratch(int buf, int C) const { return View{buf, P->bufs[buf].off, C, C}; }
  View fx_scratch(int buf, int C, int64_t per_image) const { View v = scratch(buf, C); v.off += e0 * per_image; return v; }
  static SegDesc seg(View v, int up = 0) { SegDesc s; s.v = v; s.up = up; return s; }
  const LayerPack& layer(const std::string& name) const { return h->layers[h->layer_idx.at(name)]; }
  void to_lane(size_t first_op, int lane) { for (size_t q = first_op; q < P->ops.size(); ++q) P->ops[q].lane = lane; }

  void need_groups(int n) {
    if (!h->finalized || n <= h->groups_packed) return;
    if (film_ensure_groups_(h, n) != FILM_OK) refuse(h->err);
  }

  void set_family(OpDesc& op, ConvFamily fam, int64_t M) {
    if (!conv_family_built(fam)) fam = FAM_BUF;
    op.family = fam;
    need_groups(layout_groups(kConvFamily[fam].weights));
    op.tile = conv_default_tile(fam, op.Cout, M);
  }

  void split_k(OpDesc& op, int S) {
    op.ksplit = S;
    const int64_t out_px = (int64_t)op.NB * op.H * op.W * (op.fold ? 4 : 1);
    op.part_off = P->bufs[add_scratch("splitk:" + op.tag, S * out_px * op.Cout)].off;
  }

  void conv(const std::string& tag, const std::string& name, std::vector<SegDesc> segs, View out, int NB, int H, int W, bool leaky) {
    const LayerPack& L = layer(name);
    const bool folded = h->opt_fold2x2 != 0 && L.wf_off >= 0 && segs.size() == 1 && segs[0].up && !(H & 1) && !(W & 1);
    const ConvSite s = conv_site(L, segs, out, folded ? H / 2 : H, folded ? W / 2 : W, folded);
    OpDesc op;
    op.kind = OP_CONV;
    op.tag = tag + ":" + name + (folded ? ":phases" : "");
    op.nseg = (int)segs.size();
    for (int i = 0; i < op.nseg && i < FILM_MAX_SEG; ++i) op.seg[i] = segs[i];
    op.ksize = L.kh; op.leaky = leaky; op.Cout = L.cout; op.Ctot = s.ctot;
    op.out = out; op.NB = NB; op.H = s.H; op.W = s.W;
    static_cast<ConvWeights&>(op) = L;
    op.b_off = L.b_off;
    if (s.ctot != L.ctot() || out.C != L.cout || op.nseg > FILM_MAX_SEG || !L.kmajor()) refuse("planner: channel mismatch at " + tag + ":" + name);
    if (!folded && (!s.out_16b || L.cout % 32 != 0))
      refuse("planner: " + op.tag + " writes " + std::to_string(L.cout) + " channels at float offset " + std::to_string(out.off) + " of a " +
                std::to_string(out.stride) + "-float pixel: the convolution kernels need Cout % 32 == 0 and 16-byte aligned output slices");
    set_family(op, folded ? folded_conv_family(s, *h) : plain_conv_family(s, *h), (int64_t)NB * s.H * s.W * (folded ? 2 : 1));
    if (folded) {
      op.seg[0].up = 0;
      op.fold = op.family == FAM_FOLD4 ? 3 : 2;
      op.w_off = op.fold == 3 ? L.wf4_off : L.wf_off;
      int64_t rel = 0;
      for (int q = 0; q < 4 && op.fold == 2; ++q) { op.fold_woff[q] = rel; rel += (int64_t)((q >> 1) + 1) * ((q & 1) + 1) * s.ctot * L.cout; }
    }
    const int S = conv_ksplit(op.family, s, *h);
    if (S > 1) split_k(op, S);
    const double out_px = (double)NB * H * W;
    op.flops = 2.0 * out_px * L.cout * L.kh * L.kw * L.cin;
    op.bytes = 4.0 * out_px * ((folded ? L.cin / 4.0 : L.cin) + L.cout);
    P->ops.push_back(op);
  }
  void conv_c3(const std::string& tag, const std::string& name, View in, View out, int NB, int H, int W) {
    const LayerPack& L = layer(name);
    OpDesc op;
    op.kind = OP_CONV; op.family = FAM_C3; op.tag = tag + ":" + name;
    op.nseg = 1; op.seg[0].v = in;
    op.ksize = 3; op.leaky = 1; op.Cout = out.C; op.Ctot = 3;
    op.w_off = L.w_off; op.b_off = L.b_off;
    op.out = out; op.NB = NB; op.H = H; op.W = W;
    op.tile = conv_default_tile(FAM_C3, out.C, 0);
    op.flops = 2.0 * NB * H * W * out.C * 27; op.bytes = 4.0 * NB * H * W * (3 + out.C);
    P->ops.push_back(op);
  }
  void conv_pw(const std::string& tag, const std::string& name, View in, View out, int64_t M, bool leaky) {
    const LayerPack& L = layer(name);
    OpDesc op;
    op.kind = OP_CONV_PW; op.tag = tag + ":" + name;
    op.in = in; op.out = out; op.n = M; op.leaky = leaky; op.Cout = L.cout; op.Ctot = L.cin;
    op.w_off = L.w_off; op.b_off = L.b_off;
    op.flops = 2.0 * M * L.cout * L.cin; op.bytes = 4.0 * M * (L.cin + L.cout);
    P->ops.push_back(op);
  }
  void pool(const std::string& tag, View in, View out, int NB, int H, int W) {
    OpDesc op;
    op.kind = OP_POOL; op.tag = tag; op.in = in; op.out = out; op.NB = NB; op.H = H; op.W = W;
    op.bytes = 4.0 * NB * H * W * in.C * 1.25;
    P->ops.push_back(op);
  }
  void warp(const std::string& tag, View src, View flow, View dst, int NB, int H, int W, float fscale,
            bool count_flow = true) {
    OpDesc op;
    op.kind = OP_WARP; op.tag = tag; op.in = src; op.in2 = flow; op.out = dst;
    op.NB = NB; op.H = H; op.W = W; op.fscale = fscale;
    op.bytes = 4.0 * NB * H * W * (2.0 * src.C + (count_flow ? 2 : 0));
    P->ops.push_back(op);
  }

  void add_buffers() {
    const film_config& c = h->cfg;
    for (int l = 0; l < NL; ++l) img.push_back(add_buffer("img" + std::to_string(l), NI, HL(l), WL(l), 3));
    for (int l = 0; l < NL; ++l) feat.push_back(add_buffer("feat" + std::to_string(l), NI, HL(l), WL(l), fc[l]));
    for (int i = 0; i < NL; ++i) {
      const bool pooled = std::min(NL - i, c.sub_levels) > 1;
      fx_a.push_back(add_scratch("scratch_fx_a" + std::to_string(i), (int64_t)NI * HL(i) * WL(i) * c.filters));
      fx_p.push_back(add_scratch("scratch_fx_p" + std::to_string(i), pooled ? (int64_t)NI * HL(i + 1) * WL(i + 1) * c.filters : 0));
    }
    int64_t fp_sz = 0;
    for (int l = 0; l < NL; ++l) fp_sz = std::max<int64_t>(fp_sz, (int64_t)N2 * HL(l) * WL(l) * c.flow_filters[predictor_index(c, l)]);
    for (int k = 0; k < 3; ++k) fp[k] = add_scratch("scratch_fp_" + std::to_string(k), fp_sz);
    for (int l = 0; l < NL; ++l) res.push_back(add_buffer("res" + std::to_string(l), N2, HL(l), WL(l), 2));
    for (int l = 0; l < NL - 1; ++l) {
      vup.push_back(add_buffer("vup" + std::to_string(l), N2, HL(l), WL(l), 2));
      v.push_back(add_buffer("v" + std::to_string(l), N2, HL(l), WL(l), 2));
      warped.push_back(add_buffer("warped" + std::to_string(l), N2, HL(l), WL(l), fc[l]));
    }
    v.push_back(res[NL - 1]);
    for (int l = 0; l < FL; ++l) {
      aligned.push_back(add_buffer("aligned" + std::to_string(l), B, HL(l), WL(l), 2 * fc[l] + 16));
      if (h->opt_planar && l < FL - 1 && fc[l] % 16 == 0) P->bufs[aligned[l]].planar = fc[l];
    }
    for (int i = 0; i < FL - 1; ++i) {
      fu_u.push_back(add_buffer("fusion_up" + std::to_string(i), B, HL(i), WL(i), ff[i]));
      fu_a.push_back(add_buffer("fusion_a" + std::to_string(i), B, HL(i), WL(i), ff[i]));
      fu_b.push_back(add_buffer("fusion_b" + std::to_string(i), B, HL(i), WL(i), ff[i]));
    }
    out_buf = add_buffer("out", B, H0, W0, 3);
  }

  void emit_image_pyramids() {
    for (int l = 0; l + 1 < NL; ++l) {
      pool("image_pyramid_l" + std::to_string(l + 1), view(img[l], e0, 0, 3), view(img[l + 1], e0, 0, 3), NE, HL(l), WL(l));
      P->ops.back().lane = 1;
    }
  }

  void emit_extractor(int i) {
    const film_config& c = h->cfg;
    const int n = std::min(NL - i, c.sub_levels);
    const size_t first_op = P->ops.size();
    const int64_t a_img = (int64_t)HL(i) * WL(i) * c.filters, p_img = (int64_t)HL(i + 1) * WL(i + 1) * c.filters;
    for (int j = 0; j < n; ++j) {
      const int lv = i + j, k = c.filters << j;
      const std::string tg = "feat_s" + std::to_string(i) + "_" + std::to_string(j);
      const std::string w0 = "feat_net/sub_extractor/cfeat_conv_" + std::to_string(2 * j);
      const std::string w1 = "feat_net/sub_extractor/cfeat_conv_" + std::to_string(2 * j + 1);
      View tmp = fx_scratch(fx_a[i], k, a_img);
      if (j == 0) conv_c3(tg, w0, view(img[i], e0, 0, 3), tmp, NE, HL(lv), WL(lv));
      else conv(tg, w0, {seg(fx_scratch(fx_p[i], k >> 1, p_img))}, tmp, NE, HL(lv), WL(lv), true);
      View dst = view(feat[lv], e0, slot_offset(c, j), k);
      conv(tg, w1, {seg(tmp)}, dst, NE, HL(lv), WL(lv), true);
      if (j == n - 1) continue;
      OpDesc& cv = P->ops.back();
      if ((h->opt_fuse & FUSE_POOL) && cv.kind == OP_CONV && kConvFamily[cv.family].fused_shape >= 0 && cv.ksplit <= 1 && !(HL(lv) & 1) && !(WL(lv) & 1)) {
        cv.tag += "+pool";
        cv.out2 = fx_scratch(fx_p[i], k, p_img);
      } else
        pool(tg + ":pool", dst, fx_scratch(fx_p[i], k, p_img), NE, HL(lv), WL(lv));
    }
    const int side_from = (int64_t)H0 * W0 <= 512 * 512 ? 3 : 1;
    if (i >= side_from) to_lane(first_op, 1);
  }

  void emit_flow(int l) {
    const film_config& c = h->cfg;
    const size_t first_op = P->ops.size();
    const std::string tg = "flow_l" + std::to_string(l);
    const int pi = predictor_index(c, l);
    const int nf = c.flow_filters[pi], nconv = c.flow_convs[pi];
    const std::string prefix = predictor_prefix(c, l);
    const int Hl = HL(l), Wl = WL(l);
    const bool coarsest = l == NL - 1;
    if (!coarsest) {
      const bool fuse_up = (h->opt_fuse & FUSE_FLOW_UP) && (int64_t)Hl * Wl < 100000;
      if (!fuse_up) {
        OpDesc up;
        up.kind = OP_FLOW_UP; up.tag = tg + ":resize2x";
        up.in = view(v[l + 1], 0, 0, 2); up.out = view(vup[l], 0, 0, 2);
        up.NB = N2; up.H = HL(l + 1); up.W = WL(l + 1);
        up.bytes = 4.0 * N2 * Hl * Wl * 2 * 1.25;
        P->ops.push_back(up);
      }
      for (int d = 0; d < (seq ? 2 : 1); ++d) {
        if (seq)
          warp(tg + ":warp_d" + std::to_string(d), view(feat[l], d ? i0 : i1, 0, fc[l]), view(vup[l], d * B, 0, 2),
               view(warped[l], d * B, 0, fc[l]), B, Hl, Wl, 1.f);
        else {
          warp(tg + ":warp_d01", view(feat[l], 0, 0, fc[l]), view(vup[l], 0, 0, 2), view(warped[l], 0, 0, fc[l]), N2, Hl, Wl, 1.f);
          P->ops.back().src_brot = B;
        }
        if (fuse_up) {
          OpDesc& w = P->ops.back();
          w.tag += "+resize2x";
          w.in2 = View();
          w.in3 = view(v[l + 1], d * B, 0, 2);
          w.out2 = view(vup[l], d * B, 0, 2);
        }
      }
    }
    View cur = scratch(fp[0], nf);
    if (!seq) {
      SegDesc sa = seg(view(feat[l], 0, 0, fc[l])), sb = seg(view(coarsest ? feat[l] : warped[l], 0, 0, fc[l]));
      if (coarsest) { sb.boff = B; sb.bmod = N2; }
      conv(tg, prefix + "/conv_0", {sa, sb}, cur, N2, Hl, Wl, true);
    } else {
      for (int d = 0; d < 2; ++d) {
        SegDesc a = seg(view(feat[l], d ? i1 : i0, 0, fc[l]));
        SegDesc b = seg(coarsest ? view(feat[l], d ? i0 : i1, 0, fc[l]) : view(warped[l], d * B, 0, fc[l]));
        View o = cur;
        o.off += (int64_t)d * B * Hl * Wl * nf;
        conv(tg + ":d" + std::to_string(d), prefix + "/conv_0", {a, b}, o, B, Hl, Wl, true);
      }
    }
    int which = 0;
    for (int j = 1; j < nconv; ++j) {
      View nxt = scratch(fp[which ^ 1], nf);
      conv(tg, prefix + "/conv_" + std::to_string(j), {seg(cur)}, nxt, N2, Hl, Wl, true);
      cur = nxt; which ^= 1;
    }
    const int64_t M = (int64_t)N2 * Hl * Wl;
    const std::string l3 = prefix + "/conv_" + std::to_string(nconv), l4 = prefix + "/conv_" + std::to_string(nconv + 1);
    if ((nf / 2) % 32 == 0) {
      View hid = scratch(fp[2], nf / 2);
      conv(tg, l3, {seg(cur)}, hid, N2, Hl, Wl, true);
      conv_pw(tg, l4, hid, view(res[l], 0, 0, 2), M, false);
    } else {
      const LayerPack &L3 = layer(l3), &L4 = layer(l4);
      OpDesc op;
      op.kind = OP_FLOW_HEAD; op.tag = tg + ":" + l3 + "+conv_" + std::to_string(nconv + 1);
      op.in = cur; op.out = view(res[l], 0, 0, 2); op.n = M; op.Ctot = nf;
      op.w_off = L3.w_off; op.b_off = L3.b_off; op.w2_off = L4.w_off; op.b2_off = L4.b_off;
      op.flops = 2.0 * op.n * (nf * 16 + 16 * 2); op.bytes = 4.0 * op.n * (nf + 2);
      P->ops.push_back(op);
    }
    if (!coarsest && (h->opt_fuse & FUSE_FLOW_ADD)) {
      OpDesc& head = P->ops.back();
      head.tag += "+v=res+up";
      head.in2 = view(vup[l], 0, 0, 2); head.out2 = view(v[l], 0, 0, 2);
    } else if (!coarsest) {
      OpDesc ad;
      ad.kind = OP_FLOW_ADD; ad.tag = tg + ":v=res+up";
      ad.in = view(res[l], 0, 0, 2); ad.in2 = view(vup[l], 0, 0, 2); ad.out = view(v[l], 0, 0, 2);
      ad.n = M * 2; ad.bytes = 4.0 * ad.n * 3;
      P->ops.push_back(ad);
    }
    if (l >= 4) to_lane(first_op, 1);
  }

  void emit_align(int l) {
    const size_t first_op = P->ops.size();
    const std::string tg = "align_l" + std::to_string(l);
    const bool pair = P->bufs[aligned[l]].planar > 0 && !seq;
    const bool misc16 = (h->opt_fuse & FUSE_MISC16) && !seq;
    if (pair) {
      warp(tg + ":warp_feat01", view(feat[l], 0, 0, fc[l]), view(v[l], 0, 0, 2), aligned_part(aligned[l], 0, fc[l]), N2, HL(l), WL(l), 0.5f);
      P->ops.back().flow_brot = B;
    }
    for (int s = 0; s < 2; ++s) {
      View fl = view(v[l], (1 - s) * B, 0, 2);
      if (!pair)
        warp(tg + ":warp_feat" + std::to_string(s), view(feat[l], s ? i1 : i0, 0, fc[l]), fl,
             aligned_part(aligned[l], s, fc[l]), B, HL(l), WL(l), 0.5f);
      if (!misc16)
        warp(tg + ":warp_img" + std::to_string(s), view(img[l], s ? i1 : i0, 0, 3), fl,
             sub(aligned_part(aligned[l], 2, fc[l]), 3 * s, 3), B, HL(l), WL(l), 0.5f, false);
    }
    if (misc16) {
      OpDesc& w = P->ops.back();
      w.tag += "+misc16";
      if (pair) w.misc_nb = B;
      w.img_in = view(img[l], 0, 0, 3);
      w.img_out = aligned_part(aligned[l], 2, fc[l]);
      w.pack_b = view(v[l], B, 0, 2);
      w.pack_f = view(v[l], 0, 0, 2);
      w.bytes += 4.0 * B * HL(l) * WL(l) * 12.0;
    } else {
      OpDesc pk;
      pk.kind = OP_PACK_FLOW; pk.tag = tg + ":flows";
      pk.in = view(v[l], B, 0, 2);
      pk.in2 = view(v[l], 0, 0, 2);
      pk.out = sub(aligned_part(aligned[l], 2, fc[l]), 6, 10);
      pk.n = (int64_t)B * HL(l) * WL(l); pk.bytes = 4.0 * pk.n * 14;
      P->ops.push_back(pk);
    }
    to_lane(first_op, 1);
  }

  void emit_fusion(int i, int lane) {
    const size_t first_op = P->ops.size();
    const std::string tg = "fusion_l" + std::to_string(i);
    const std::string base = "fusion/convs_" + std::to_string(i);
    conv(tg, base + "_0", {seg(net, 1)}, view(fu_u[i], 0, 0, ff[i]), B, HL(i), WL(i), false);
    const SegDesc up = seg(view(fu_u[i], 0, 0, ff[i]));
    if (P->bufs[aligned[i]].planar)
      conv(tg, base + "_1", {seg(aligned_part(aligned[i], 0, fc[i])), seg(aligned_part(aligned[i], 1, fc[i])), seg(aligned_part(aligned[i], 2, fc[i])), up},
           view(fu_a[i], 0, 0, ff[i]), B, HL(i), WL(i), true);
    else
      conv(tg, base + "_1", {seg(view(aligned[i], 0, 0, 2 * fc[i] + 16)), up}, view(fu_a[i], 0, 0, ff[i]), B, HL(i), WL(i), true);
    conv(tg, base + "_2", {seg(view(fu_a[i], 0, 0, ff[i]))}, view(fu_b[i], 0, 0, ff[i]), B, HL(i), WL(i), true);
    net = view(fu_b[i], 0, 0, ff[i]);
    to_lane(first_op, lane);
  }

  void emit_rgb_head() {
    OpDesc& last = P->ops.back();
    const LayerPack& LO = layer("fusion/output_conv");
    if ((h->opt_fuse & FUSE_RGB_HEAD) && last.kind == OP_CONV && kConvFamily[last.family].fused_shape >= 0 && last.Cout == 64 && last.ksplit <= 1 &&
        last.out2.buf < 0 && LO.cout <= 4 && LO.cin == 64) {
      last.tag += "+output_conv";
      last.pw_out = view(out_buf, 0, 0, 3); last.pw_cout = LO.cout;
      last.w2_off = LO.w_off; last.b2_off = LO.b_off;
      last.tile = conv_tile(last.family, kConvFamily[last.family].fused_shape, true);
      last.flops += 2.0 * (double)B * H0 * W0 * LO.cout * LO.cin;
      last.bytes = 4.0 * (double)B * H0 * W0 * (64 + LO.cout);
    } else {
      conv_pw("fusion_out", "fusion/output_conv", net, view(out_buf, 0, 0, 3), (int64_t)B * H0 * W0, false);
    }
  }

  int build(int B_, int H_, int W_, int T_, int slot) {
    const film_config& c = h->cfg;
    B = B_; H0 = H_; W0 = W_; T = T_;
    NL = c.pyramid_levels; FL = c.fusion_pyramid_levels;
    seq = T > 0;
    N2 = 2 * B;
    NI = seq ? B + T : N2;
    i0 = 0; i1 = seq ? T : B;
    NE = NI; e0 = 0;
    if (slot >= 0) {
      if (slot > 1 || B != T) return fail(h, FILM_ERR_INVALID, "a stream plan has slot 0 or 1 and one pair of its tiles");
      i0 = (1 - slot) * T; i1 = slot * T;
      NE = T; e0 = i1;
    }
    fc = feature_channels(c);
    ff = fusion_filters(c);
    P->B = B; P->H = H0; P->W = W0; P->tiles = T; P->slot = slot;
    add_buffers();
    emit_image_pyramids();
    for (int i = 0; i < NL; ++i) emit_extractor(i);
    P->n_extract = P->ops.size();
    for (int l = NL - 1; l >= 0; --l) emit_flow(l);
    const bool early_fusion = h->opt_lanes >= 2 && ((int64_t)H0 * W0 > 512 * 512 || h->opt_lanes >= 3) && FL >= 4;
    net = view(aligned[FL - 1], 0, 0, 2 * fc[FL - 1] + 16);
    emit_align(FL - 1);
    if (early_fusion) {
      for (int i = FL - 2; i >= 0; --i) {
        emit_align(i);
        if (i >= 2) emit_fusion(i, 1);
      }
      for (int i = std::min(FL - 2, 1); i >= 0; --i) emit_fusion(i, 0);
    } else {
      for (int i = FL - 2; i >= 0; --i) emit_align(i);
      for (int i = FL - 2; i >= 0; --i) emit_fusion(i, 0);
    }
    emit_rgb_head();
    if (bad) return fail(h, FILM_ERR_INVALID, "%s", bad_msg.c_str());
    P->arena_floats = cursor;
    analyze_lanes();
    return FILM_OK;
  }

  struct Access { int buf; int c0, c1; };
  Access access(const View& v) const {
    const Buffer& b = P->bufs[v.buf];
    if (b.C == 0 || v.stride != b.C) return {v.buf, 0, 1 << 30};
    const int c0 = (int)((v.off - b.off) % b.C);
    return {v.buf, c0, c0 + v.C};
  }
  static bool overlap(const Access& a, const Access& b) { return a.buf == b.buf && a.c0 < b.c1 && b.c0 < a.c1; }
  void accesses(const OpDesc& op, std::vector<Access>& rd, std::vector<Access>& wr) const {
    rd.clear(); wr.clear();
    if (op.kind == OP_CONV) { for (int i = 0; i < op.nseg; ++i) rd.push_back(access(op.seg[i].v)); }
    else { if (op.in.buf >= 0) rd.push_back(access(op.in)); if (op.in2.buf >= 0) rd.push_back(access(op.in2)); }
    if (op.in3.buf >= 0) rd.push_back(access(op.in3));
    if (op.img_in.buf >= 0) rd.push_back(access(op.img_in));
    if (op.pack_b.buf >= 0) { rd.push_back(access(op.pack_b)); rd.push_back(access(op.pack_f)); }
    if (op.out.buf >= 0 && op.pw_out.buf < 0) wr.push_back(access(op.out));
    if (op.pw_out.buf >= 0) wr.push_back(access(op.pw_out));
    if (op.out2.buf >= 0) wr.push_back(access(op.out2));
    if (op.img_out.buf >= 0) wr.push_back(access(op.img_out));
  }
  void analyze_lanes() {
    const size_t n = P->ops.size();
    std::vector<std::vector<Access>> rd(n), wr(n);
    for (size_t i = 0; i < n; ++i) accesses(P->ops[i], rd[i], wr[i]);
    long waited[2] = {-1, -1};
    for (size_t j = 0; j < n; ++j) {
      OpDesc& oj = P->ops[j];
      const int lj = oj.lane ? 1 : 0;
      for (size_t ii = j; ii-- > 0;) {
        const OpDesc& oi = P->ops[ii];
        if ((oi.lane ? 1 : 0) == lj) continue;
        if ((long)ii <= waited[lj]) break;
        bool hit = false;
        for (const Access& w : wr[ii]) {
          for (const Access& r : rd[j]) hit |= overlap(w, r);
          for (const Access& w2 : wr[j]) hit |= overlap(w, w2);
        }
        for (const Access& r : rd[ii])
          for (const Access& w2 : wr[j]) hit |= overlap(r, w2);
        if (hit) { oj.xdeps.push_back((int)ii); P->ops[ii].signal = true; waited[lj] = (long)ii; break; }
      }
    }
  }
};

}

int plan_build(film_t* h, Plan* P, int B, int H, int W, int tiles, int slot) {
  Planner pl{h, P};
  return pl.build(B, H, W, tiles, slot);
}

int64_t limited_buffer_bytes(const Plan* P) {
  int64_t mx = 1;
  for (const OpDesc& op : P->ops) {
    if (op.kind != OP_CONV || op.family == FAM_W43 || op.family == FAM_W2D) continue;
    for (int i = 0; i < op.nseg; ++i) mx = std::max(mx, P->bufs[op.seg[i].v.buf].floats * (int64_t)sizeof(float));
  }
  return mx;
}

namespace {
struct JsonObject {
  std::ostringstream& o;
  const char* sep = "{";
  std::ostringstream& key(const char* k) { o << sep << "\"" << k << "\":"; sep = ","; return o; }
  template <class T> void num(const char* k, const T& v) { key(k) << v; }
  void str(const char* k, const std::string& v) { key(k) << "\"" << v << "\""; }
  template <class T, class F> void list(const char* k, const T* a, size_t n, F each) {
    key(k) << "[";
    for (size_t i = 0; i < n; ++i) { o << (i ? "," : ""); each(a[i]); }
    o << "]";
  }
  template <class T> void ints(const char* k, const T* a, size_t n) { list(k, a, n, [&](const T& v) { o << v; }); }
  template <class T, class F> void objects(const char* k, const T* a, size_t n, F fill) {
    list(k, a, n, [&](const T& v) { JsonObject e{o}; fill(e, v); o << "}"; });
  }
  void view(const char* k, const View& v, const Plan& P) {
    JsonObject j{key(k)};
    j.str("buf", v.buf >= 0 ? P.bufs[v.buf].name : std::string(""));
    j.num("off", v.off); j.num("stride", v.stride); j.num("C", v.C);
    o << "}";
  }
};

void json_op(JsonObject& j, const OpDesc& op, const Plan& P) {
  const FamilyCodes fc = family_codes(op.family);
  j.str("kind", kKindName[op.kind]); j.str("tag", op.tag); j.num("NB", op.NB); j.num("H", op.H); j.num("W", op.W);
  j.num("ksize", op.ksize); j.num("leaky", op.leaky); j.num("Cout", op.Cout); j.num("Ctot", op.Ctot); j.num("tile", op.tile);
  j.num("w_off", op.w_off); j.num("b_off", op.b_off); j.num("wf4_off", op.wf4_off);
  j.num("wh_off", op.wh_off); j.num("halo", fc.halo); j.num("ws_off", op.ws_off); j.num("split", fc.split);
  j.num("ww_off", op.ww_off); j.num("wx_off", op.wx_off); j.num("wfx_off", op.wfx_off); j.num("w43_off", op.w43_off); j.num("w2d_off", op.w2d_off);
  j.num("wino", fc.wino); j.num("fold", op.fold); j.num("ksplit", op.ksplit);
  j.num("py", op.py); j.num("px", op.px); j.num("ftaps", op.ftaps); j.ints("tdy", op.tdy, 4); j.ints("tdx", op.tdx, 4);
  j.ints("fold_woff", op.fold_woff, 4); j.num("lane", op.lane); j.ints("xdeps", op.xdeps.data(), op.xdeps.size());
  j.num("w2_off", op.w2_off); j.num("b2_off", op.b2_off); j.num("c3", fc.c3);
  j.num("fscale", op.fscale); j.num("src_brot", op.src_brot); j.num("flow_brot", op.flow_brot); j.num("misc_nb", op.misc_nb); j.num("n", op.n);
  j.num("flops", op.flops); j.num("bytes", op.bytes);
  j.view("in", op.in, P); j.view("in2", op.in2, P); j.view("in3", op.in3, P); j.view("out2", op.out2, P); j.view("pw_out", op.pw_out, P); j.num("pw_cout", op.pw_cout);
  j.view("img_in", op.img_in, P); j.view("img_out", op.img_out, P); j.view("pack_b", op.pack_b, P); j.view("pack_f", op.pack_f, P); j.view("out", op.out, P);
  j.objects("segs", op.seg, op.nseg, [&](JsonObject& s, const SegDesc& g) {
    s.view("v", g.v, P); s.num("boff", g.boff); s.num("bmod", g.bmod); s.num("up", g.up);
  });
}
}

std::string plan_json(film_t* h, const Plan& P) {
  std::ostringstream o;
  JsonObject j{o};
  j.num("B", P.B); j.num("H", P.H); j.num("W", P.W);
  if (P.slot >= 0) { j.str("kind", "stream"); j.num("tiles", P.tiles); j.num("slot", P.slot); j.num("n_extract", P.n_extract); }
  else if (P.tiles > 0) { j.str("kind", "sequence"); j.num("n_pairs", P.B / P.tiles); j.num("tiles", P.tiles); }
  j.num("arena_floats", P.arena_floats); j.num("offset32_buffer_bytes", limited_buffer_bytes(&P)); j.num("packed_floats", h->packed_floats);
  j.objects("buffers", P.bufs.data(), P.bufs.size(), [](JsonObject& e, const Buffer& b) {
    e.str("name", b.name); e.num("off", b.off); e.num("N", b.N); e.num("H", b.H); e.num("W", b.W); e.num("C", b.C); e.num("floats", b.floats); e.num("planar", b.planar);
  });
  j.objects("layers", h->layers.data(), h->layers.size(), [](JsonObject& e, const LayerPack& L) {
    e.str("name", L.name); e.num("kh", L.kh); e.num("kw", L.kw); e.num("cin", L.cin); e.num("cout", L.cout); e.num("ctot", L.ctot());
    e.num("w_off", L.w_off); e.num("b_off", L.b_off); e.num("wh_off", L.wh_off); e.num("ws_off", L.ws_off); e.num("ww_off", L.ww_off); e.num("wx_off", L.wx_off);
  });
  j.objects("ops", P.ops.data(), P.ops.size(), [&](JsonObject& e, const OpDesc& op) { json_op(e, op, P); });
  o << "}";
  return o.str();
}

}
```

### frame-interpolation_amd/csrc/film_plans.cpp

```cpp
#include "film_internal.h"

namespace film_internal {
namespace {
void free_plan(Plan* p) {
  if (p->twin) { p->twin->arena = nullptr; free_plan(p->twin.get()); }
  if (p->graph_exec) (void)hipGraphExecDestroy(p->graph_exec);
  if (p->graph) (void)hipGraphDestroy(p->graph);
  for (auto e : p->ev) (void)hipEventDestroy(e);
  for (auto e : p->lane_ev) if (e) (void)hipEventDestroy(e);
  if (p->arena) (void)hipFree(p->arena);
}

void forget_plan(film_t* h, size_t index) {
  if (h->last_plan == h->plans[index].get() || (h->last_plan && h->last_plan == h->plans[index]->twin.get())) h->last_plan = nullptr;
  free_plan(h->plans[index].get());
  h->plans.erase(h->plans.begin() + index);
}

constexpr int64_t kMaxBufferBytes = 0xFFF00000ll;
constexpr int64_t kMaxArenaBytes = 64ll << 30;
int64_t arena_budget_bytes(film_t* h) {
  int64_t cap = kMaxArenaBytes;
  if (!h->plan_only) {
    size_t fr = 0, tot = 0;
    if (hipSetDevice(h->device) == hipSuccess && hipMemGetInfo(&fr, &tot) == hipSuccess) {
      int64_t held = 0;
      for (auto& p : h->plans) if (p->arena) held += p->arena_floats * (int64_t)sizeof(float);
      cap = std::min<int64_t>(cap, ((int64_t)fr + held) / 10 * 6);
    } else {
      (void)hipGetLastError();
    }
  }
  return std::max<int64_t>(cap, 1);
}
}

void drop_plans(film_t* h) {
  if (!h->plan_only) { (void)hipSetDevice(h->device); (void)hipDeviceSynchronize(); }
  while (!h->plans.empty()) forget_plan(h, h->plans.size() - 1);
}

int get_plan(film_t* h, int B, int H, int W, bool need_device, Plan** out, int tiles, bool stream) {
  const auto same = [&](const Plan& p) { return p.B == B && p.H == H && p.W == W && p.tiles == tiles && (p.slot >= 0) == stream; };
  const int div = 1 << (h->cfg.pyramid_levels - 1);
  if (B < 1 || H < 1 || W < 1) return fail(h, FILM_ERR_INVALID, "B, H, W must be positive");
  if (H % div || W % div)
    return fail(h, FILM_ERR_INVALID, "input height and width (%d x %d) must be divisible by %d = 2^(pyramid_levels-1); "
                "pad first (Interpolator align)", H, W, div);
  const int wl = std::max(h->cfg.pyramid_levels - 2, h->cfg.fusion_pyramid_levels - 1);
  if ((H >> wl) < 2 || (W >> wl) < 2)
    return fail(h, FILM_ERR_INVALID, "input %d x %d too small: warped pyramid level %d would be smaller than 2x2", H, W, wl);
  if ((int64_t)2 * B * H * W >= (int64_t)1 << 31) return fail(h, FILM_ERR_INVALID, "batch too large (2*B*H*W must fit int32)");
  for (auto& p : h->plans)
    if (same(*p) && (!need_device || p->arena)) { *out = p.get(); p->last_use = ++h->tick; return FILM_OK; }
  if (need_device)
    for (size_t i = 0; i < h->plans.size(); ++i)
      if (same(*h->plans[i])) { forget_plan(h, i); break; }
  std::unique_ptr<Plan> P(new Plan);
  int rc = plan_build(h, P.get(), B, H, W, tiles, stream ? 0 : -1);
  if (rc) return rc;
  P->id = ++h->plan_ids;
  if (stream) {
    P->twin.reset(new Plan);
    Plan& Q = *P->twin;
    if ((rc = plan_build(h, &Q, B, H, W, tiles, 1))) return rc;
    bool alike = Q.arena_floats == P->arena_floats && Q.bufs.size() == P->bufs.size() && Q.n_extract == P->n_extract;
    for (size_t i = 0; alike && i < Q.bufs.size(); ++i) alike = Q.bufs[i].name == P->bufs[i].name && Q.bufs[i].off == P->bufs[i].off && Q.bufs[i].floats == P->bufs[i].floats;
    if (!alike) return fail(h, FILM_ERR_INVALID, "planner: the two orientations of a stream plan lay out different workspaces");
    Q.id = P->id;
  }
  if (need_device) {
    size_t alive = 0;
    for (auto& p : h->plans) alive += p->arena != nullptr;
    while (alive >= 3) {
      size_t victim = h->plans.size();
      for (size_t i = 0; i < h->plans.size(); ++i)
        if (h->plans[i]->arena && (victim == h->plans.size() || h->plans[i]->last_use < h->plans[victim]->last_use)) victim = i;
      if (victim == h->plans.size()) break;
      (void)hipSetDevice(h->device);
      (void)hipDeviceSynchronize();
      forget_plan(h, victim);
      --alive;
    }
    hipError_t e = hipMalloc(&P->arena, (size_t)P->arena_floats * sizeof(float));
    if (e != hipSuccess && alive > 0) {
      (void)hipGetLastError();
      (void)hipDeviceSynchronize();
      for (size_t i = h->plans.size(); i-- > 0;)
        if (h->plans[i]->arena) forget_plan(h, i);
      e = hipMalloc(&P->arena, (size_t)P->arena_floats * sizeof(float));
    }
    if (e != hipSuccess) {
      P->arena = nullptr;
      return fail(h, FILM_ERR_NOMEM, "workspace hipMalloc of %.1f MB failed: %s", P->arena_floats * 4e-6, hipGetErrorString(e));
    }
    HIPCHK(h, hipMemsetAsync(P->arena, 0, (size_t)P->arena_floats * sizeof(float), h->stream));
    HIPCHK(h, hipStreamSynchronize(h->stream));
    if (P->twin) P->twin->arena = P->arena;
    if (h->opt_autotune && h->finalized) {
      int trc = autotune_plan(h, P.get());
      if (trc == FILM_OK && P->twin) trc = autotune_plan(h, P->twin.get());
      if (trc) { free_plan(P.get()); return trc; }
    }
  }
  const std::pair<ConvFamily, int> forced[] = {{FAM_W43, h->opt_w43_shape}, {FAM_W2D, h->opt_w2d_shape}, {FAM_FOLD4, h->opt_fold4_shape}};
  for (const auto& [fam, shape] : forced) {
    if (shape < 0) continue;
    for (Plan* R : {P.get(), P->twin.get()}) {
      if (!R) continue;
      for (OpDesc& op : R->ops) {
        if (op.kind != OP_CONV || op.family != fam) continue;
        const std::vector<int> cands = conv_candidates(op);
        const int want = conv_tile(fam, shape, true);
        if (std::find(cands.begin(), cands.end(), want) != cands.end()) op.tile = want;
      }
    }
  }
  P->last_use = ++h->tick;
  *out = P.get();
  h->plans.push_back(std::move(P));
  return FILM_OK;
}

int max_units(film_t* h, int H, int W, const char* what, const char* advice, int* units) {
  Plan* P1 = nullptr;
  int rc = get_plan(h, 1, H, W, false, &P1);
  if (rc) return rc;
  const int64_t lim = limited_buffer_bytes(P1);
  const int64_t arena = std::max<int64_t>(1, P1->arena_floats * (int64_t)sizeof(float));
  *units = (int)std::max<int64_t>(1, std::min<int64_t>(kMaxBufferBytes / lim, arena_budget_bytes(h) / arena));
  if (lim > kMaxBufferBytes)
    return fail(h, FILM_ERR_INVALID, "a %d x %d %s needs a %.1f GB activation buffer in front of a kernel that addresses 4 GiB per "
                "buffer - %s", H, W, what, lim * 1e-9, advice);
  if (h->opt_max_batch) *units = std::min(*units, h->opt_max_batch);
  return FILM_OK;
}

}
```

### frame-interpolation_amd/csrc/film_tune.cpp

```cpp
#include "film_internal.h"

namespace film_internal {
namespace {
std::vector<int> both_maps(ConvFamily f, const std::vector<int>& shapes) {
  std::vector<int> out;
  for (int sh : shapes) { out.push_back(conv_tile(f, sh, false)); out.push_back(conv_tile(f, sh, true)); }
  return out;
}

std::string conv_signature(const OpDesc& op) {
  std::ostringstream o;
  const FamilyCodes fc = family_codes(op.family);
  o << op.NB << 'x' << op.H << 'x' << op.W << ':' << op.Cout << ':' << op.ksize << ':' << op.out.stride << ':' << fc.c3 << ':' << fc.halo << ':' << fc.split << ':' << fc.wino << ':' << op.fold << ':' << op.ksplit << ':' << (op.out2.buf >= 0) << ':' << op.pw_cout;
  for (int i = 0; i < op.nseg; ++i)
    o << '|' << op.seg[i].v.C << ',' << op.seg[i].v.stride << ',' << op.seg[i].up << ',' << op.seg[i].bmod;
  return o.str();
}
}

std::vector<int> tile_candidates(const OpDesc& op) {
  if (op.Cout % 128 == 0) return both_maps(FAM_BUF, {TILE_128x128, TILE_256x128, TILE_256x64, TILE_128x64, TILE_64x64});
  if (op.Cout % 64 == 0) return both_maps(FAM_BUF, {TILE_256x64, TILE_128x64, TILE_64x64, TILE_256x32, TILE_128x32});
  return both_maps(FAM_BUF, {TILE_256x32, TILE_128x32});
}

std::vector<int> c3_candidates(const OpDesc&) { return {conv_tile(FAM_C3, TILE_C3_DIRECT, false)}; }

std::vector<int> halo_candidates(const OpDesc& op) {
  if (op.Cout % 128 == 0) return both_maps(op.family, {HALO_4x64, HALO_4x128, HALO_8x64, HALO_8x128});
  if (op.Cout % 64 == 0) return both_maps(op.family, {HALO_4x64, HALO_8x64, HALO_4x32, HALO_8x32});
  return both_maps(op.family, {HALO_8x32, HALO_4x32});
}

std::vector<int> wino_candidates(const OpDesc& op) {
  if (op.Cout % 128 == 0) return both_maps(FAM_WINO, {WINO_4x64_W8, WINO_8x64_W16, WINO_2x64, WINO_4x128_W16, WINO_4x128});
  if (op.Cout % 64 == 0) return both_maps(FAM_WINO, {WINO_4x64_W8, WINO_8x64_W16, WINO_2x64, WINO_4x32});
  return both_maps(FAM_WINO, {WINO_4x32, WINO_8x32_W8});
}

std::vector<int> wino43_candidates(const OpDesc& op) {
  const bool pool = op.out2.buf >= 0, pw = op.pw_out.buf >= 0;
  std::vector<int> shapes;
  if (pw)
    shapes = {W43_Q16_4x64_N1, W43_Q16_4x64_N1_P2, W43_Q8_8x64_N1_P2};
  else if (op.Cout % 64 == 0)
    shapes = {W43_4x64_T21, W43_Q16_4x64_T21, W43_Q16_4x64_T12, W43_Q16_4x32_T11, W43_Q16_4x64_N1,
              W43_Q16_4x64_T21_P2, W43_Q16_4x64_T12_P2, W43_Q16_4x32_T11_P2, W43_Q16_4x64_N1_P2, W43_Q16_4x32_T11_BG,
              W43_Q8_8x64_T21_P2, W43_Q8_8x64_T12_P2, W43_Q8_8x64_N1_P2, W43_Q8_8x32_T11_BG, W43_Q8_8x32_T11_P2};
  else
    shapes = {W43_4x32_T11, W43_Q16_4x32_T11, W43_Q16_4x32_T11_P2, W43_Q16_4x32_T11_BG, W43_Q8_8x32_T11_BG, W43_Q8_8x32_T11_P2};
  std::vector<int> keep;
  for (int sh : shapes) {
    if (!film_w43_shape_built(sh)) continue;
    if (pool && (sh == W43_4x64_T21 || sh == W43_4x64_T12 || sh == W43_4x32_T11)) continue;
    keep.push_back(sh);
  }
  return both_maps(FAM_W43, keep);
}

std::vector<int> wino2d_candidates(const OpDesc& op) {
  const int H = op.H, W = op.W;
  const bool pw = op.pw_out.buf >= 0;
  const int64_t pad_r = (int64_t)((W + 31) / 32) * ((H + 7) / 8), pad_s = (int64_t)((W + 15) / 16) * ((H + 15) / 16);
  const bool sq = pad_s <= pad_r;
  std::vector<int> shapes;
  if (pw || op.Cout % 64 == 0) { shapes.push_back(W2D_8x64); if (sq) shapes.push_back(W2D_16x64); }
  if (!pw) {
    shapes.push_back(W2D_8x32); shapes.push_back(W2D_8x32_S2);
    if (sq) { shapes.push_back(W2D_16x32); shapes.push_back(W2D_16x32_S2); }
  }
  return both_maps(FAM_W2D, shapes);
}

std::vector<int> fold4_candidates(const OpDesc& op) {
  return both_maps(FAM_FOLD4, op.Cout % 64 == 0 ? std::vector<int>{F4_4x64, F4_4x32} : std::vector<int>{F4_4x32});
}

std::vector<int> foldx3_candidates(const OpDesc& op) {
  return both_maps(FAM_FOLDX3, op.Cout % 128 == 0 ? std::vector<int>{FX3_4x64, FX3_8x64, FX3_4x128} : std::vector<int>{FX3_4x64, FX3_8x64});
}

std::vector<int> winox3_candidates(const OpDesc& op) {
  if (op.Cout % 128 == 0) return both_maps(FAM_WINOX3, {WX3_4x128_T22, WX3_4x64_T12, WX3_4x64_T21});
  if (op.Cout % 64 == 0) return both_maps(FAM_WINOX3, {WX3_4x64_T12, WX3_4x64_T21, WX3_4x32_T11});
  return both_maps(FAM_WINOX3, {WX3_4x32_T11});
}

std::vector<int> conv_candidates(const OpDesc& op) { return kConvFamily[op.family].candidates(op); }

int autotune_plan(film_t* h, Plan* P) {
  bool need = false;
  for (const OpDesc& op : P->ops) {
    if (op.kind != OP_CONV) continue;
    const std::string sig = conv_signature(op);
    if (h->tune_cache.count(sig)) continue;
    auto it = h->tune_import.find(sig);
    if (it != h->tune_import.end()) {
      const std::vector<int> cands = conv_candidates(op);
      if (std::find(cands.begin(), cands.end(), it->second) != cands.end()) { h->tune_cache[sig] = it->second; continue; }
    }
    need = true;
  }
  if (need) {
    HIPCHK(h, film_launch_fill_random(P->arena, P->arena_floats, 0x9e3779b9u, h->stream));
    hipEvent_t e0, e1;
    HIPCHK(h, hipEventCreate(&e0));
    HIPCHK(h, hipEventCreate(&e1));
    for (OpDesc& op : P->ops) {
      if (op.kind != OP_CONV) continue;
      const std::string sig = conv_signature(op);
      if (h->tune_cache.count(sig)) continue;
      int best = op.tile;
      float best_ms = 1e30f;
      const std::vector<int> cands = conv_candidates(op);
      auto launch_tile = [&](int tile) -> hipError_t {
        OpDesc trial = op;
        trial.tile = tile;
        return launch_op(trial, P->arena, h->packed_dev, h->stream);
      };
      auto time_once = [&](int tile, float* ms) -> int {
        HIPCHK(h, hipEventRecord(e0, h->stream));
        HIPCHK(h, launch_tile(tile));
        HIPCHK(h, hipEventRecord(e1, h->stream));
        HIPCHK(h, hipEventSynchronize(e1));
        HIPCHK(h, hipEventElapsedTime(ms, e0, e1));
        return FILM_OK;
      };
      std::vector<std::pair<float, int>> timed;
      for (int tile : cands) {
        HIPCHK(h, launch_tile(tile));
        float ms_min = 1e30f, ms_sum = 0.f;
        for (int rep = 0; rep < 2 || (ms_sum < (float)h->opt_tune_ms && rep < 64); ++rep) {
          float ms = 0;
          int trc = time_once(tile, &ms);
          if (trc) return trc;
          ms_min = std::min(ms_min, ms);
          ms_sum += ms;
        }
        timed.push_back({ms_min, tile});
      }
      std::sort(timed.begin(), timed.end());
      size_t nfin = 0;
      while (nfin < timed.size() && nfin < 4 && timed[nfin].first <= timed[0].first * 1.06f) ++nfin;
      if (nfin > 1)
        for (int round = 0; round < 4; ++round)
          for (size_t c = 0; c < nfin; ++c) {
            float ms = 0;
            int trc = time_once(timed[c].second, &ms);
            if (trc) return trc;
            timed[c].first = std::min(timed[c].first, ms);
          }
      for (size_t c = 0; c < std::max<size_t>(nfin, 1) && c < timed.size(); ++c)
        if (timed[c].first < best_ms) { best_ms = timed[c].first; best = timed[c].second; }
      if (op.family == FAM_W2D && !film_w2d_64(best & 15)) {
        float ms64 = 1e30f;
        int t64 = -1;
        for (size_t c = 0; c < std::max<size_t>(nfin, 1) && c < timed.size(); ++c)
          if (film_w2d_64(timed[c].second & 15) && timed[c].first < ms64) { ms64 = timed[c].first; t64 = timed[c].second; }
        if (t64 >= 0 && ms64 <= best_ms * 1.02f) best = t64;
      }
      h->tune_cache[sig] = best;
    }
    (void)hipEventDestroy(e0);
    (void)hipEventDestroy(e1);
    HIPCHK(h, hipMemsetAsync(P->arena, 0, (size_t)P->arena_floats * sizeof(float), h->stream));
    HIPCHK(h, hipStreamSynchronize(h->stream));
  }
  for (OpDesc& op : P->ops)
    if (op.kind == OP_CONV) op.tile = h->tune_cache.at(conv_signature(op));
  return FILM_OK;
}

}

using namespace film_internal;

extern "C" {

int film_export_tune(film_t* h, char* buf, int64_t cap, int64_t* needed) {
  if (!h) return FILM_ERR_INVALID;
  std::ostringstream o;
  o << "# film_hip tune cache v1 " << film_version() << "\n";
  std::map<std::string, int> all = h->tune_import;
  for (const auto& kv : h->tune_cache) all[kv.first] = kv.second;
  for (const auto& kv : all) o << kv.first << '\t' << kv.second << '\n';
  return copy_out_string(h, o.str(), buf, cap, needed);
}

int film_import_tune(film_t* h, const char* text) {
  if (!h || !text) return fail(h, FILM_ERR_INVALID, "NULL argument");
  std::istringstream in(text);
  std::string line;
  if (!std::getline(in, line)) return FILM_OK;
  const std::string want = std::string("# film_hip tune cache v1 ") + film_version();
  if (line != want) return FILM_OK;
  std::map<std::string, int> got;
  while (std::getline(in, line)) {
    if (line.empty() || line[0] == '#') continue;
    const size_t tab = line.rfind('\t');
    if (tab == std::string::npos || tab == 0 || tab + 1 >= line.size()) return fail(h, FILM_ERR_INVALID, "tune cache: malformed line '%s'", line.c_str());
    char* end = nullptr;
    const long tile = strtol(line.c_str() + tab + 1, &end, 10);
    if (*end != 0 || tile < 0 || tile > (1 << 20)) return fail(h, FILM_ERR_INVALID, "tune cache: malformed line '%s'", line.c_str());
    got[line.substr(0, tab)] = (int)tile;
  }
  for (const auto& kv : got) h->tune_import[kv.first] = kv.second;
  return FILM_OK;
}

}
```

Before: 29.61 frames/s.

## Chain several 32-channel output blocks per Winograd-2D workgroup with prefetch

Result: no change. 29.62 frames/s (median of 3 runs) (+0.0%).

```diff
diff --git a/frame-interpolation_amd/csrc/conv_igemm.hip b/frame-interpolation_amd/csrc/conv_igemm.hip
--- a/frame-interpolation_amd/csrc/conv_igemm.hip
+++ b/frame-interpolation_amd/csrc/conv_igemm.hip
@@ -109,6 +109,8 @@
     case W2D_16x64: return conv_wino2d_launch_any<64, F | W2D_F_SQ>(p, s);
     case W2D_16x32: return conv_wino2d_launch_any<32, F | W2D_F_SQ>(p, s);
     case W2D_16x32_S2: return conv_wino2d_launch_any<32, F | W2D_F_SQ, 2>(p, s);
+    case W2D_8x32_S2_C: return conv_wino2d_launch_any<32, F | W2D_F_CHAIN, 2>(p, s);
+    case W2D_16x32_S2_C: return conv_wino2d_launch_any<32, F | W2D_F_SQ | W2D_F_CHAIN, 2>(p, s);
     default: return hipErrorInvalidValue;
   }
 }
diff --git a/frame-interpolation_amd/csrc/conv_wino2d_impl.h b/frame-interpolation_amd/csrc/conv_wino2d_impl.h
--- a/frame-interpolation_amd/csrc/conv_wino2d_impl.h
+++ b/frame-interpolation_amd/csrc/conv_wino2d_impl.h
@@ -3,6 +3,7 @@
 
 enum { W2D_F_SQ = 128,
        W2D_F_XEPI = 8,
+       W2D_F_CHAIN = 256,
        W2D_DBG_TIME = 8192 };
 
 
@@ -35,6 +36,8 @@
   static_assert(NREQ % NW == 0, "requests per wave");
   static_assert(HR * RP4 <= STAGE4, "stage size");
   constexpr bool XE = (FLAGS & W2D_F_XEPI) != 0;
+  constexpr bool CH = (FLAGS & W2D_F_CHAIN) != 0;
+  static_assert(!CH || BN == 32, "chained blocks: the 32-channel tiles");
   constexpr unsigned OOB = 0xFFFFFFFFu;
 
   extern __shared__ __attribute__((aligned(1024))) float smem[];
@@ -49,7 +52,7 @@
   unsigned long long rt0 = 0;
   if constexpr ((FLAGS & W2D_DBG_TIME) != 0) { rt0 = __builtin_amdgcn_s_memrealtime(); tm0 = __builtin_readcyclecounter(); }
 
-  int aH = p.H, aW = p.W, aNB = p.NB, aCtot = p.Ctot, aKsplit = p.ksplit, aNseg = p.nseg, aUnused = p.unused_chain;
+  int aH = p.H, aW = p.W, aNB = p.NB, aCtot = p.Ctot, aKsplit = p.ksplit, aNseg = p.nseg, aChain = p.chain;
   unsigned a_tpi = p.mg_tpi, a_ntx = p.mg_ntx, a_nby = p.mg_nby;
   int ntx_ = p.tl_ntx, tpi_ = p.tl_tpi;
   int aGx = (int)gridDim.x, aGy = (int)gridDim.y;
@@ -61,7 +64,7 @@
   for (int n = 0; n < 24 / NW; ++n) rtab[n] = w2d_slot_table<SQ>.v[t + 64 * NW * n];
   {
     unsigned long long q0 = (unsigned long long)(uintptr_t)aS0ptr, q1 = (unsigned long long)(uintptr_t)aWptr;
-    asm volatile("" : "+s"(aH), "+s"(aW), "+s"(aNB), "+s"(aCtot), "+s"(aKsplit), "+s"(aNseg), "+s"(aUnused), "+s"(a_tpi), "+s"(a_ntx), "+s"(a_nby), "+s"(ntx_), "+s"(tpi_),
+    asm volatile("" : "+s"(aH), "+s"(aW), "+s"(aNB), "+s"(aCtot), "+s"(aKsplit), "+s"(aNseg), "+s"(aChain), "+s"(a_tpi), "+s"(a_ntx), "+s"(a_nby), "+s"(ntx_), "+s"(tpi_),
                       "+s"(aGx), "+s"(aGy), "+s"(q0), "+s"(q1), "+s"(aS0stride), "+s"(aS0C), "+s"(aS0boff), "+s"(aS0bmod));
     aS0ptr = reinterpret_cast<const float*>((uintptr_t)q0);
     aWptr = reinterpret_cast<const float*>((uintptr_t)q1);
@@ -84,7 +87,8 @@
   const int img = (int)conv_udiv((unsigned)bx, a_tpi);
   const int trow0 = (int)conv_udiv((unsigned)(bx - img * tpi), a_ntx);
   const int y0 = trow0 * TH, x0 = (bx - img * tpi - trow0 * ntx) * PXW;
-  const int n0 = by * BN;
+  int n0 = by * BN;
+  if constexpr (CH) n0 *= aChain;
 
   unsigned rvoff[IPW];
   int rsg = 0, rc0 = 0, rsegC = 0;
@@ -143,7 +147,7 @@
       if (rsg + 1 < aNseg) { rc0 = 0; ++rsg; raw_setup_seg(); }
     }
   };
-  const int ksp = XE && aKsplit > 1 ? aKsplit : 1;
+  const int ksp = XE && !CH && aKsplit > 1 ? aKsplit : 1;
   const int nsc_all = aCtot >> 4;
   int sc0 = 0, sc1 = nsc_all;
   if (ksp > 1) {
@@ -162,7 +166,7 @@
   const int nkc = aCtot / 8, nsc = sc1 - sc0, kc0 = 2 * sc0, kc1 = 2 * sc1;
   const conv_rsrc_t brsrc = conv_make_rsrc(conv_uniform_ptr(aWptr));
   const unsigned bvoff = (unsigned)((half * 32 + l31) * 16);
-  const int ct = n0 / 32 + ng;
+  int ct = n0 / 32 + ng;
   auto slab = [&](int kc) { return (unsigned)(((ct * nkc + (kc < nkc ? kc : nkc - 1)) * 4 + mu) * 6) * 1024u; };
   bf4 fbg[2][6];
 
@@ -342,9 +346,23 @@
     }
   };
 
+  bool pf_next = false;
+  float cb0 = 0.f, cb1 = 0.f, cb2 = 0.f, cb3 = 0.f;
   auto epilogue = [&]() {
     const int t = threadIdx.x, lane = t & 63, l31 = lane & 31, half = lane >> 5;
     __syncthreads();
+    if constexpr (CH) {
+      asm volatile("" : "+v"(cb0), "+v"(cb1), "+v"(cb2), "+v"(cb3));
+      if (pf_next) {
+        rsg = 0; rc0 = 0;
+        if (aNseg > 1) raw_setup_seg_of(aS0ptr, aS0stride, aS0C, aS0boff, aS0bmod);
+        raw_issue(0);
+      }
+      const unsigned so = (unsigned)((((ct + (pf_next ? 1 : 0)) * nkc) * 4 + mu) * 6) * 1024u;
+#pragma unroll
+      for (int j = 0; j < 6; ++j) fbg[0][j] = conv_buf_load(brsrc, bvoff, so + (unsigned)j * 1024u);
+      __builtin_amdgcn_sched_barrier(0);
+    }
     if constexpr ((FLAGS & W2D_DBG_TIME) != 0) tmE1 = __builtin_readcyclecounter();
     float o[4][16];
   #pragma unroll
@@ -356,17 +374,18 @@
       o[2][r] = __builtin_fmaf(4.f, s34, s12);
       o[3][r] = d12 + __builtin_fmaf(8.f, d34, m5);
     }
-    bf4* const xb = reinterpret_cast<bf4*>(smem);
     constexpr int XB4 = NG * 4 * 256;
-    static_assert(2 * XB4 <= NS * STAGE4, "exchange buffers");
+    bf4* const xb = reinterpret_cast<bf4*>(smem) + (CH ? STAGE4 : 0);
+    static_assert(CH || 2 * XB4 <= NS * STAGE4, "exchange buffers");
     const int widx = (ng * 4 + mu) * 256 + l31 * 8;
     const int rng = t >> 8, run = (t >> 3) & 31, rcg = t & 7;
     const int ridx = rng * 1024 + run * 8 + (rcg ^ (run & 7));
     const int nrd = n0 + rng * 32 + rcg * 4;
     const bool rawsum = XE && ksp > 1;
-    const bool has_pw = XE && p.pw_out != nullptr;
+    const bool has_pw = XE && !CH && p.pw_out != nullptr;
     float b0 = 0.f, b1 = 0.f, b2 = 0.f, b3 = 0.f;
-    if (!rawsum) { const float* const bp = p.bias + nrd; b0 = bp[0]; b1 = bp[1]; b2 = bp[2]; b3 = bp[3]; }
+    if constexpr (CH) { b0 = cb0; b1 = cb1; b2 = cb2; b3 = cb3; }
+    else if (!rawsum) { const float* const bp = p.bias + nrd; b0 = bp[0]; b1 = bp[1]; b2 = bp[2]; b3 = bp[3]; }
     const int oy = y0 + 2 * (run / QW), ox = x0 + 4 * (run % QW);
     const int ostr = rawsum ? p.Cout : p.ostride;
     const float slope = (p.leaky && !rawsum) ? 0.2f : 1.f;
@@ -461,19 +480,39 @@
     }
   };
   if constexpr ((FLAGS & W2D_DBG_TIME) != 0) tm1 = __builtin_readcyclecounter();
-  for (int tile = 0; tile < 1; ++tile) {
+  const int nblk = CH ? aChain : 1;
+  for (int tile = 0; tile < nblk; ++tile) {
+    if constexpr (CH) pf_next = tile + 1 < nblk;
     chunk(kc0, C0{}, C1{}, C0{});
     chunk(kc0 + 1, C1{}, C0{}, C0{});
     for (int kc = kc0 + 2; kc < kc1 - 2; kc += 2) {
       chunk(kc, C0{}, C0{}, C0{});
       chunk(kc + 1, C1{}, C0{}, C0{});
     }
+    if constexpr (CH) {
+      const float* const bp = p.bias + (n0 + (t & 7) * 4);
+      cb0 = bp[0]; cb1 = bp[1]; cb2 = bp[2]; cb3 = bp[3];
+    }
     if (nsc > 1) {
       chunk(kc1 - 2, C0{}, C0{}, C1{});
       chunk(kc1 - 1, C1{}, C0{}, C1{});
     }
     if constexpr ((FLAGS & W2D_DBG_TIME) != 0) tm2 = __builtin_readcyclecounter();
     epilogue();
+    if constexpr (CH) {
+      n0 += pf_next ? 32 : 0; ct += pf_next ? 1 : 0;
+      __builtin_amdgcn_sched_barrier(0);
+      asm volatile("s_waitcnt vmcnt(6)" ::: "memory");
+      __syncthreads();
+#pragma unroll
+      for (int j = 0; j < 6; ++j) fbg[1][j] = conv_buf_load(brsrc, bvoff, slab(kc0 + 1) + (unsigned)j * 1024u);
+      __builtin_amdgcn_sched_barrier(0);
+      if (!pf_next) break;
+      st_s = 0; st_n = 1; st_dma = 0; dma_on = false; gs = 0;
+      if (nsc > 1) raw_issue(1);
+      if constexpr (NS > 2) { if (nsc > 2) raw_issue(2); }
+      prepare(A[0], 0, C0{});
+    }
   }
   if constexpr ((FLAGS & W2D_DBG_TIME) != 0) {
     const unsigned long long tm3 = __builtin_readcyclecounter();
@@ -490,7 +529,10 @@
 template <int BN, int FLAGS, int NS = 3>
 hipError_t conv_wino2d_launch(const ConvParams& p, hipStream_t s) {
   if (!(FLAGS & W2D_F_XEPI) && (p.ksplit > 1 || p.pool_out || p.pw_out)) return hipErrorInvalidValue;
-  const size_t lds = p.pw_out ? (size_t)2 * (BN / 32) * 16 * 1024 + 256 * 68 * 4 + 1024 : (size_t)NS * 24 * 1024;
+  constexpr bool CH = (FLAGS & W2D_F_CHAIN) != 0;
+  if (CH && (p.chain < 1 || p.Cout % (BN * p.chain) || p.ksplit > 1 || p.pw_out)) return hipErrorInvalidValue;
+  const int chain = CH ? p.chain : 1;
+  const size_t lds = p.pw_out ? (size_t)2 * (BN / 32) * 16 * 1024 + 256 * 68 * 4 + 1024 : std::max<size_t>((size_t)NS * 24 * 1024, CH ? 56 * 1024 : 0);
   constexpr int NT = 4 * (BN / 32) * 64;
   if (p.ksize != 3 || p.Ctot % 16 || p.Cout % BN) return hipErrorInvalidValue;
   if (p.ksplit > 1 && (!p.part || (reinterpret_cast<uintptr_t>(p.part) & 15) || p.Cout % 4 || p.pool_out || p.pw_out || p.ksplit > p.Ctot / 16)) return hipErrorInvalidValue;
@@ -510,8 +552,9 @@
   constexpr bool SQ = (FLAGS & W2D_F_SQ) != 0;
   const int ntx = SQ ? (p.W + 15) / 16 : (p.W + 31) / 32, nty = SQ ? (p.H + 15) / 16 : (p.H + 7) / 8;
   const int ntiles = p.NB * ntx * nty;
-  dim3 grid((unsigned)ntiles, p.Cout / BN, (unsigned)(p.ksplit > 1 ? p.ksplit : 1));
+  dim3 grid((unsigned)ntiles, p.Cout / (BN * chain), (unsigned)(p.ksplit > 1 ? p.ksplit : 1));
   ConvParams q = p;
+  q.chain = chain;
   bool exact = true;
   q.mg_nby = conv_magic(grid.y, (unsigned long long)grid.x * grid.y, exact);
   q.mg_tpi = conv_magic((unsigned long long)ntx * nty, (unsigned long long)ntiles + 1, exact);
diff --git a/frame-interpolation_amd/csrc/film_engine.cpp b/frame-interpolation_amd/csrc/film_engine.cpp
--- a/frame-interpolation_amd/csrc/film_engine.cpp
+++ b/frame-interpolation_amd/csrc/film_engine.cpp
@@ -65,6 +65,7 @@
     {"w2d_min_px", &film_t::opt_w2d_min_px, AS_IS, true, 1, 1 << 30, "w2d_min_px: pixels per image"},
     {"w2d_splitk", &film_t::opt_w2d_splitk, AS_IS, true, 0, 16, "w2d_splitk: 0 (off), 1 (default rule) or 2..16 (A/B: the cap on levels of <= 1024 pixels)"},
     {"w2d_shape", &film_t::opt_w2d_shape, AS_IS, true, -1, W2D_SHAPES - 1, "w2d_shape: -1 (autotuned) or a Wino2dTile shape index"},
+    {"w2d_chain", &film_t::opt_w2d_chain, AS_IS, true, 0, 2, "w2d_chain: 0 (never), 1 (offered to the autotuner: the default) or 2 (every op that can, for tests)"},
     {"fold4_shape", &film_t::opt_fold4_shape, AS_IS, true, -1, F4_4x32, "fold4_shape: -1 (autotuned) or a Fold4Tile shape index"},
     {"w43_shape", &film_t::opt_w43_shape, AS_IS, true, -1, 31, "w43_shape: -1 (autotuned) or a Wino43Tile shape index"},
     {"precision", &film_t::opt_precision, AS_IS, true, 0, 2, "precision: 0 (f32), 1 (bf16x6) or 2 (bf16x3)", FAM_SPLIT6, 1, 2,
diff --git a/frame-interpolation_amd/csrc/film_exec.cpp b/frame-interpolation_amd/csrc/film_exec.cpp
--- a/frame-interpolation_amd/csrc/film_exec.cpp
+++ b/frame-interpolation_amd/csrc/film_exec.cpp
@@ -25,6 +25,7 @@
       p.M = op.NB * op.H * op.W;
       p.fold = op.fold; p.py = op.py; p.px = op.px; p.ftaps = op.ftaps;
       p.ksplit = op.ksplit; p.part = op.ksplit > 1 ? arena + op.part_off : nullptr;
+      p.chain = op.chain;
       if (op.out2.buf >= 0) { p.pool_out = mptr(arena, op.out2); p.pool_ostride = op.out2.stride; }
       if (op.pw_out.buf >= 0) {
         p.pw_w = wts + op.w2_off; p.pw_bias = wts + op.b2_off; p.pw_out = mptr(arena, op.pw_out); p.pw_ostride = op.pw_out.stride; p.pw_cout = op.pw_cout;
diff --git a/frame-interpolation_amd/csrc/film_internal.h b/frame-interpolation_amd/csrc/film_internal.h
--- a/frame-interpolation_amd/csrc/film_internal.h
+++ b/frame-interpolation_amd/csrc/film_internal.h
@@ -59,6 +59,7 @@
   int64_t b_off = 0;
   int64_t w2_off = 0, b2_off = 0;
   int ksplit = 1;
+  int chain = 1;
   int64_t part_off = 0;
   int fold = 0, py = 0, px = 0;
   int ftaps = 0; int tdy[4] = {0, 0, 0, 0}, tdx[4] = {0, 0, 0, 0};
@@ -192,6 +193,7 @@
   int opt_w2d_small_px = 256;
   int opt_w2d_splitk = 1;
   int opt_w2d_shape = -1;
+  int opt_w2d_chain = 1;
   int opt_fold4_shape = -1;
   int opt_w43_shape = -1;
   std::string profile_json;
diff --git a/frame-interpolation_amd/csrc/film_kernels.h b/frame-interpolation_amd/csrc/film_kernels.h
--- a/frame-interpolation_amd/csrc/film_kernels.h
+++ b/frame-interpolation_amd/csrc/film_kernels.h
@@ -32,7 +32,7 @@
   long long fold_woff[4];
   int ksplit;
   float* part;
-  int unused_chain;
+  int chain;
   unsigned mg_tpi, mg_ntx, mg_nby;
   int tl_ntx, tl_tpi;
   float* pool_out;
@@ -169,9 +169,18 @@
   return sh == W43_Q16_4x64_T21_P2 || sh == W43_Q16_4x32_T11_P2 || sh == W43_Q16_4x64_N1_P2 || sh == W43_Q8_8x64_T21_P2 || sh == W43_Q8_8x64_N1_P2 ||
          sh == W43_Q8_8x32_T11_BG || sh == W43_Q8_8x32_T11_P2;
 }
-enum Wino2dTile { W2D_8x64 = 0, W2D_8x32 = 1, W2D_8x32_S2 = 2, W2D_16x64 = 3, W2D_16x32 = 4, W2D_16x32_S2 = 5, W2D_SHAPES = 6 };
-inline bool film_w2d_square(int shape) { return shape >= W2D_16x64 && shape <= W2D_16x32_S2; }
+enum Wino2dTile { W2D_8x64 = 0, W2D_8x32 = 1, W2D_8x32_S2 = 2, W2D_16x64 = 3, W2D_16x32 = 4, W2D_16x32_S2 = 5, W2D_SHAPES = 6,
+                  W2D_8x32_S2_C = 6, W2D_16x32_S2_C = 7, W2D_TILES = 8 };
+inline bool film_w2d_square(int shape) { return (shape >= W2D_16x64 && shape <= W2D_16x32_S2) || shape == W2D_16x32_S2_C; }
 inline bool film_w2d_64(int shape) { return shape == W2D_8x64 || shape == W2D_16x64; }
+inline bool film_w2d_chained(int shape) { return shape == W2D_8x32_S2_C || shape == W2D_16x32_S2_C; }
+inline int film_w2d_chain(int mode, int NB, int H, int W, int Cout) {
+  if (mode <= 0 || Cout % 32) return 1;
+  const long long tiles = (long long)NB * ((W + 31) / 32) * ((H + 7) / 8);
+  for (int c = 4; c >= 2; c -= 2)
+    if ((Cout / 32) % c == 0 && (mode >= 2 || tiles * (Cout / (32 * c)) >= 2048)) return c;
+  return 1;
+}
 enum Fold4Tile { F4_4x64 = 0, F4_4x32 = 1 };
 enum FoldX3Tile { FX3_4x64 = 0 , FX3_8x64 = 1 , FX3_4x128 = 2  };
 enum WinoX3Tile { WX3_4x128_T22 = 0, WX3_4x64_T12 = 1, WX3_4x64_T21 = 3, WX3_4x32_T11 = 4 };
diff --git a/frame-interpolation_amd/csrc/film_planner.cpp b/frame-interpolation_amd/csrc/film_planner.cpp
--- a/frame-interpolation_amd/csrc/film_planner.cpp
+++ b/frame-interpolation_amd/csrc/film_planner.cpp
@@ -191,6 +191,7 @@
     }
     const int S = conv_ksplit(op.family, s, *h);
     if (S > 1) split_k(op, S);
+    if (op.family == FAM_W2D && op.ksplit <= 1) op.chain = film_w2d_chain(h->opt_w2d_chain, NB, op.H, op.W, op.Cout);
     const double out_px = (double)NB * H * W;
     op.flops = 2.0 * out_px * L.cout * L.kh * L.kw * L.cin;
     op.bytes = 4.0 * out_px * ((folded ? L.cin / 4.0 : L.cin) + L.cout);
@@ -443,7 +444,7 @@
     if ((h->opt_fuse & FUSE_RGB_HEAD) && last.kind == OP_CONV && kConvFamily[last.family].fused_shape >= 0 && last.Cout == 64 && last.ksplit <= 1 &&
         last.out2.buf < 0 && LO.cout <= 4 && LO.cin == 64) {
       last.tag += "+output_conv";
-      last.pw_out = view(out_buf, 0, 0, 3); last.pw_cout = LO.cout;
+      last.pw_out = view(out_buf, 0, 0, 3); last.pw_cout = LO.cout; last.chain = 1;
       last.w2_off = LO.w_off; last.b2_off = LO.b_off;
       last.tile = conv_tile(last.family, kConvFamily[last.family].fused_shape, true);
       last.flops += 2.0 * (double)B * H0 * W0 * LO.cout * LO.cin;
@@ -587,7 +588,7 @@
   j.num("w_off", op.w_off); j.num("b_off", op.b_off); j.num("wf4_off", op.wf4_off);
   j.num("wh_off", op.wh_off); j.num("halo", fc.halo); j.num("ws_off", op.ws_off); j.num("split", fc.split);
   j.num("ww_off", op.ww_off); j.num("wx_off", op.wx_off); j.num("wfx_off", op.wfx_off); j.num("w43_off", op.w43_off); j.num("w2d_off", op.w2d_off);
-  j.num("wino", fc.wino); j.num("fold", op.fold); j.num("ksplit", op.ksplit);
+  j.num("wino", fc.wino); j.num("fold", op.fold); j.num("ksplit", op.ksplit); j.num("chain", op.chain);
   j.num("py", op.py); j.num("px", op.px); j.num("ftaps", op.ftaps); j.ints("tdy", op.tdy, 4); j.ints("tdx", op.tdx, 4);
   j.ints("fold_woff", op.fold_woff, 4); j.num("lane", op.lane); j.ints("xdeps", op.xdeps.data(), op.xdeps.size());
   j.num("w2_off", op.w2_off); j.num("b2_off", op.b2_off); j.num("c3", fc.c3);
diff --git a/frame-interpolation_amd/csrc/film_plans.cpp b/frame-interpolation_amd/csrc/film_plans.cpp
--- a/frame-interpolation_amd/csrc/film_plans.cpp
+++ b/frame-interpolation_amd/csrc/film_plans.cpp
@@ -116,6 +116,16 @@
       }
     }
   }
+  if (h->opt_w2d_chain == 2)
+    for (Plan* R : {P.get(), P->twin.get()}) {
+      if (!R) continue;
+      for (OpDesc& op : R->ops) {
+        if (op.kind != OP_CONV || op.family != FAM_W2D || op.chain <= 1) continue;
+        const std::vector<int> cands = conv_candidates(op);
+        const int want = conv_tile(FAM_W2D, film_w2d_square(conv_tile_shape(op.tile)) ? W2D_16x32_S2_C : W2D_8x32_S2_C, (op.tile & CONV_TILE_XCD) != 0);
+        if (std::find(cands.begin(), cands.end(), want) != cands.end()) op.tile = want;
+      }
+    }
   P->last_use = ++h->tick;
   *out = P.get();
   h->plans.push_back(std::move(P));
diff --git a/frame-interpolation_amd/csrc/film_tune.cpp b/frame-interpolation_amd/csrc/film_tune.cpp
--- a/frame-interpolation_amd/csrc/film_tune.cpp
+++ b/frame-interpolation_amd/csrc/film_tune.cpp
@@ -11,7 +11,7 @@
 std::string conv_signature(const OpDesc& op) {
   std::ostringstream o;
   const FamilyCodes fc = family_codes(op.family);
-  o << op.NB << 'x' << op.H << 'x' << op.W << ':' << op.Cout << ':' << op.ksize << ':' << op.out.stride << ':' << fc.c3 << ':' << fc.halo << ':' << fc.split << ':' << fc.wino << ':' << op.fold << ':' << op.ksplit << ':' << (op.out2.buf >= 0) << ':' << op.pw_cout;
+  o << op.NB << 'x' << op.H << 'x' << op.W << ':' << op.Cout << ':' << op.ksize << ':' << op.out.stride << ':' << fc.c3 << ':' << fc.halo << ':' << fc.split << ':' << fc.wino << ':' << op.fold << ':' << op.ksplit << ':' << (op.out2.buf >= 0) << ':' << op.pw_cout << ':' << op.chain;
   for (int i = 0; i < op.nseg; ++i)
     o << '|' << op.seg[i].v.C << ',' << op.seg[i].v.stride << ',' << op.seg[i].up << ',' << op.seg[i].bmod;
   return o.str();
@@ -68,6 +68,10 @@
   if (!pw) {
     shapes.push_back(W2D_8x32); shapes.push_back(W2D_8x32_S2);
     if (sq) { shapes.push_back(W2D_16x32); shapes.push_back(W2D_16x32_S2); }
+    if (op.chain > 1 && op.ksplit <= 1) {
+      shapes.push_back(W2D_8x32_S2_C);
+      if (sq) shapes.push_back(W2D_16x32_S2_C);
+    }
   }
   return both_maps(FAM_W2D, shapes);
 }
@@ -159,6 +163,13 @@
           if (film_w2d_64(timed[c].second & 15) && timed[c].first < ms64) { ms64 = timed[c].first; t64 = timed[c].second; }
         if (t64 >= 0 && ms64 <= best_ms * 1.02f) best = t64;
       }
+      if (op.family == FAM_W2D && !film_w2d_64(best & 15) && !film_w2d_chained(best & 15)) {
+        float msc = 1e30f;
+        int tc = -1;
+        for (size_t c = 0; c < std::max<size_t>(nfin, 1) && c < timed.size(); ++c)
+          if (film_w2d_chained(timed[c].second & 15) && timed[c].first < msc) { msc = timed[c].first; tc = timed[c].second; }
+        if (tc >= 0 && msc <= best_ms * 1.02f) best = tc;
+      }
       h->tune_cache[sig] = best;
     }
     (void)hipEventDestroy(e0);
```
